# CompVis/behavior-driven-video-synthesis

Hardware: AMD Instinct MI355X
Metric: frames/sec VUnet 256x256 bs=16 fwd+bwd (higher is better)
Workload: dtype f32 (operands scaled by a power of two and split into 2 fp16 terms, 3 partial products on fp16 MFMA, fp32 accumulate; weight gradients and uncovered layers: 3 bf16 terms / 6 products, fp32-input MFMA, fp32 VALU); 1 GPU; Human3.6m shape_and_pose_net VunetAlter 256x256 per-GPU bs=16 fwd+bwd, VGG19 perceptual + KL loss, fused Adam, dropout 0.05, regressor side loop off, seeded-synthetic VGG19 weights, rasterised synthetic stickmen; global_batch=16, parallelism=dp1, conv_precision=h2, hip_streams=4, hip_graph=True, graph_settle_steps=7, rccl_world_size=1, dp_backend=none

## Files before the change

behavior_driven_video_synthesis_amd/csrc/common.h:

```cpp
#pragma once
#include <hip/hip_runtime.h>
#include <stdint.h>
#include <stdlib.h>

typedef float f32x16 __attribute__((ext_vector_type(16)));
typedef float f32x4 __attribute__((ext_vector_type(4)));

#include "../../include/vunet_hip.h"

enum { ACT_NONE = 0, ACT_ELU = 1, ACT_RELU = 2, ACT_SIGMOID = 3, ACT_LRELU = 4 };

__host__ __device__ __forceinline__ uint32_t vunet_hash_u32(uint32_t x) {
  x ^= x >> 16;
  x *= 0x7feb352dU;
  x ^= x >> 15;
  x *= 0x846ca68bU;
  x ^= x >> 16;
  return x;
}

__device__ __forceinline__ float elu_f(float x) { return x > 0.f ? x : (__expf(x) - 1.f); }
__device__ __forceinline__ float elu_grad_f(float x) { return x > 0.f ? 1.f : __expf(x); }
__device__ __forceinline__ float sigmoid_f(float x) { return 1.f / (1.f + expf(-x)); }
__device__ __forceinline__ float4 add4(float4 a, float4 b) { return make_float4(a.x + b.x, a.y + b.y, a.z + b.z, a.w + b.w); }

struct InAct {
  int act;
  uint32_t thresh;
  uint32_t seed;
  float keep_scale;
  float slope;
  const uint32_t* step;
};

#define VUNET_DROP_STEP_MUL 0x9E3779B1u

__device__ __forceinline__ uint32_t inact_seed(const InAct& a) {
  return a.step ? a.seed + (*a.step) * VUNET_DROP_STEP_MUL : a.seed;
}

__device__ __forceinline__ void inact_resolve(InAct& a) {
  a.seed = inact_seed(a);
  a.step = nullptr;
}

__device__ __forceinline__ float apply_in_act(const InAct& a, float v, uint32_t idx) {
  if (a.act == ACT_ELU) v = elu_f(v);
  else if (a.act == ACT_RELU) v = v > 0.f ? v : 0.f;
  else if (a.act == ACT_LRELU) v = v > 0.f ? v : v * a.slope;
  if (a.thresh) v = (vunet_hash_u32(idx + inact_seed(a)) >= a.thresh) ? v * a.keep_scale : 0.f;
  return v;
}

template <int FORM>
__device__ __forceinline__ float in_act_form(const InAct& a, float v, uint32_t idx) {
  if constexpr (FORM == 0) return v;
  else if constexpr (FORM == 1) return elu_f(v);
  else if constexpr (FORM == 2) {
    v = elu_f(v);
    return (vunet_hash_u32(idx + a.seed) >= a.thresh) ? v * a.keep_scale : 0.f;
  } else return apply_in_act(a, v, idx);
}
__device__ __forceinline__ int in_act_form_of(const InAct& a) {
  if (a.thresh) return a.act == ACT_ELU ? 2 : 3;
  return a.act == ACT_NONE ? 0 : (a.act == ACT_ELU ? 1 : 3);
}

__device__ __forceinline__ float in_act_grad(const InAct& a, float v, uint32_t idx) {
  float g = 1.f;
  if (a.act == ACT_ELU) g = elu_grad_f(v);
  else if (a.act == ACT_RELU) g = v > 0.f ? 1.f : 0.f;
  else if (a.act == ACT_LRELU) g = v > 0.f ? 1.f : a.slope;
  if (a.thresh) g = (vunet_hash_u32(idx + inact_seed(a)) >= a.thresh) ? g * a.keep_scale : 0.f;
  return g;
}

__device__ __forceinline__ float wave_sum(float v) {
#pragma unroll
  for (int o = 32; o > 0; o >>= 1) v += __shfl_xor(v, o, 64);
  return v;
}

__device__ __forceinline__ float wave_max(float v) {
#pragma unroll
  for (int o = 32; o > 0; o >>= 1) v = fmaxf(v, __shfl_xor(v, o, 64));
  return v;
}

__device__ __forceinline__ unsigned xcd_remap(unsigned bid, unsigned nblk) {
  const unsigned q = nblk >> 3, r = nblk & 7u, xcd = bid & 7u, idx = bid >> 3;
  const unsigned start = xcd < r ? xcd * (q + 1) : r * (q + 1) + (xcd - r) * q;
  return start + idx;
}

extern const uint32_t* g_vunet_drop_step;

static inline InAct make_inact(int act, float slope, float p, uint32_t seed) {
  InAct a;
  a.act = act;
  a.slope = slope;
  a.seed = seed;
  a.step = p > 0.f ? g_vunet_drop_step : nullptr;
  if (p > 0.f) {
    double t = (double)p * 4294967296.0;
    a.thresh = t >= 4294967295.0 ? 4294967295u : (uint32_t)t;
    if (a.thresh == 0) a.thresh = 1;
    a.keep_scale = 1.f / (1.f - p);
  } else {
    a.thresh = 0;
    a.keep_scale = 1.f;
  }
  return a;
}

#define VUNET_ENV_FLAG(fn, name)                              \
  static inline bool fn() {                                   \
    static const bool on = getenv(name) != nullptr;           \
    return on;                                                \
  }

extern int g_vunet_tune[16];

static inline int vunet_check_launch() {
  hipError_t e = hipGetLastError();
  return e == hipSuccess ? VUNET_OK : VUNET_ERR_LAUNCH;
}

#define VUNET_LAUNCH(...)          \
  do {                             \
    (void)hipGetLastError();       \
    hipLaunchKernelGGL(__VA_ARGS__); \
  } while (0)
```

behavior_driven_video_synthesis_amd/csrc/conv_h2_kernel.h:

```cpp
#pragma once
#include <type_traits>

#include "conv_common.h"

#include "split_h2.h"

__device__ __forceinline__ void h2_dma_wait() { asm volatile("s_waitcnt vmcnt(0)" ::: "memory"); }

union H2Unit {
  uint4 u;
  h2_f16x8 b;
};

#ifdef H2_TSTAMP
static __device__ unsigned long long h2_ts[8192 * 8];
#define H2_STAMP(k_)                                                                                              \
  do {                                                                                                            \
    if (threadIdx.x == 0 && blockIdx.x < 8192) h2_ts[blockIdx.x * 8 + (k_)] = __builtin_amdgcn_s_memrealtime();   \
  } while (0)
extern "C" int H2_TSTAMP(unsigned long long* out, int nblocks) {
  return hipMemcpyFromSymbol(out, HIP_SYMBOL(h2_ts), sizeof(unsigned long long) * 8 * (size_t)nblocks) == hipSuccess ? 0 : -1;
}
#else
#define H2_STAMP(k_)
#endif

template <int MT, int NT, int MODE, int PRO, int PHW = -1, int NWV = 4, int TW = 32>
__global__ __launch_bounds__(64 * NWV, (NWV == 8 || MT * NT >= 8) ? 1 : 2) void conv_h2_kernel(const GatherArgs a_in,
                                                                             const uint4* __restrict__ wx, int mtiles_pad,
                                                                             const float* __restrict__ amax) {
  GatherArgs a = a_in;
  H2_STAMP(0);
  inact_resolve(a.in1);
  inact_resolve(a.in2);
  inact_resolve(a.auxa);
  static_assert(PHW < 0 || MODE == 1, "parity phases exist for the data gradient only");
  constexpr bool ALLP = PHW == 4;
  static_assert(!ALLP || (NT == 1 && TW == 32 && NWV == 4 && PRO == 0), "fused parities: one dy row per wave");
  constexpr int NQ = ALLP ? 4 : NT;
  constexpr bool PIPE = TW == 16 && PHW < 0;
  constexpr int PH = (PHW >= 0 && !ALLP) ? (PHW >> 1) : 0, PW = (PHW >= 0 && !ALLP) ? (PHW & 1) : 0;
  constexpr int NKH = (PHW < 0 || ALLP) ? 3 : (PH ? 2 : 1);
  constexpr int NTHR = 64 * NWV;
  static_assert(TW == 32 || TW == 16, "tile width");
  constexpr int RPQ = 32 / TW;
  constexpr int TH = NWV * NT * RPQ, IH = TH + 2, CW = TW + 2, IW = TW == 32 ? CW : 32, PIX = IH * IW, MB = 32 * MT;
  constexpr int XU = 2 * IH * CW;
  constexpr int NX = (XU + NTHR - 1) / NTHR;
  constexpr int WU = H2_SLAB * MT;
  constexpr int GS = NWV == 8 ? NKH : 1;
  constexpr int WUS = WU * GS;
  extern __shared__ __attribute__((aligned(16))) uint4 smem4[];
  uint4* const xL = smem4;
  uint4* const wL = smem4 + 8 * PIX;

  const vunet_conv_desc& d = a.d;
  const int tid = threadIdx.x, lane = tid & 63, wave = tid >> 6;
  const int j = lane & 31, h = lane >> 5;
  const int jr = j / TW, jc = j % TW;
  const int H = d.Hs, W = d.Ws, HW = a.HsWs;

  const unsigned bid = xcd_remap(blockIdx.x, gridDim.x);
  const int mblocks = (d.M + MB - 1) / MB;
  const int mb = bid % mblocks;
  int t = bid / mblocks;
  const int tiles_w = W / TW, tiles_h = H / TH;
  const int tx = t % tiles_w;
  t /= tiles_w;
  const int ty = t % tiles_h;
  const int n = t / tiles_h;
  const int row0 = ty * TH, col0 = tx * TW, m0 = mb * MB;

  float sx, descale, descale2;

  unsigned rel[NX];
  int lds_x[NX];
  uint32_t vbits = 0;
#pragma unroll
  for (int i = 0; i < NX; ++i) {
    int u = tid + NTHR * i;
    if (u >= XU) u -= XU;
    const int c8 = u / (IH * CW);
    const int rem = u - c8 * (IH * CW);
    const int r = rem / CW, col = rem - r * CW;
    const int ih = row0 - 1 + r, iw = col0 - 1 + col;
    const bool ok = (unsigned)ih < (unsigned)H && (unsigned)iw < (unsigned)W;
    rel[i] = ok ? (unsigned)(8 * c8 * HW + ih * W + iw) : 0u;
    lds_x[i] = c8 * PIX + r * IW + col;
    vbits |= (ok ? 1u : 0u) << i;
  }

  f32x16 acc[MT][NQ], acx[MT][NQ];
#pragma unroll
  for (int mt = 0; mt < MT; ++mt)
#pragma unroll
    for (int q = 0; q < NQ; ++q)
#pragma unroll
      for (int r = 0; r < 16; ++r) acc[mt][q][r] = acx[mt][q][r] = 0.f;

  const int nch1 = d.C1 / 16, nch = nch1 + d.C2 / 16;
  float xv[NX][8];
  float mk[1][8];
  const int mt0 = (d.m_off + m0) >> 5;

  auto issue_x = [&](int ch, int i) {
    const bool second = ch >= nch1;
    const int cs = second ? (ch - nch1) * 16 : ch * 16;
    const int C = second ? d.C2 : d.C1;
    const float* __restrict__ xs = (second ? a.x2 : a.x1) + (size_t)(n * C + cs) * HW;
#pragma unroll
    for (int k = 0; k < 8; ++k)
      xv[i][k] = *reinterpret_cast<const float*>(reinterpret_cast<const char*>(xs) +
                                                 4u * (rel[i] + (((vbits >> i) & 1u) ? (unsigned)(k * HW) : 0u)));
  };
  auto issue_mask = [&](int ch, int i) {
    if constexpr (PRO == 4) {
      const float* __restrict__ ms = a.mask + (size_t)(n * d.C1 + ch * 16) * HW;
#pragma unroll
      for (int k = 0; k < 8; ++k)
        mk[0][k] = *reinterpret_cast<const float*>(reinterpret_cast<const char*>(ms) +
                                                   4u * (rel[i] + (((vbits >> i) & 1u) ? (unsigned)(k * HW) : 0u)));
    }
  };
  auto write_x = [&](int ch, int i) {
    const bool second = ch >= nch1;
    const int cs = second ? (ch - nch1) * 16 : ch * 16;
    const int C = second ? d.C2 : d.C1;
    InAct ia = a.in1;
    ia.seed = second ? a.in2.seed : a.in1.seed;
    const int gbase = (n * C + cs) * HW;
    const bool ok = (vbits >> i) & 1u;
    float v[8];
#pragma unroll
    for (int k = 0; k < 8; ++k) {
      float t_ = ok ? xv[i][k] : 0.f;
      if constexpr (PRO == 4) t_ = mk[0][k] > 0.f ? t_ : 0.f;
      else if constexpr (PRO != 0) t_ = prologue<PRO>(ia, t_, (uint32_t)gbase + rel[i] + (uint32_t)(k * HW));
      v[k] = t_ * sx;
    }
    uint4 ph, pl;
    h2_split2(v[0], v[1], ph.x, pl.x);
    h2_split2(v[2], v[3], ph.y, pl.y);
    h2_split2(v[4], v[5], ph.z, pl.z);
    h2_split2(v[6], v[7], ph.w, pl.w);
    uint4* const xb = xL + (ch & 1) * 4 * PIX;
    xb[lds_x[i]] = ph;
    xb[2 * PIX + lds_x[i]] = pl;
  };
  constexpr int WPS = WU / 64;
  constexpr int NWI = (GS * WPS + NWV - 1) / NWV;
  const int wave_u = __builtin_amdgcn_readfirstlane(wave);
  const uint32_t wL_addr = (uint32_t)(uintptr_t)(__attribute__((address_space(3))) void*)wL;
  auto slab_of = [&](int step) {
    if constexpr (PHW < 0 || ALLP) return step;
    else if constexpr (PH == 0) return step * 3 + 1;
    else return (step >> 1) * 3 + ((step & 1) ? 2 : 0);
  };
  auto issue_w = [&](int stage, int buf) {
#pragma unroll
    for (int i = 0; i < NWI; ++i) {
      int wi = wave_u + NWV * i;
      if (wi >= GS * WPS) wi -= GS * WPS;
      const int g = wi / WPS, r = wi - g * WPS;
      const char* wp = reinterpret_cast<const char*>(wx) + 16 +
                       ((size_t)slab_of(stage * GS + g) * mtiles_pad + mt0) * (H2_SLAB * 16);
      h2_dma16(wp + (size_t)(r * 64 + lane) * 16, wL_addr + (uint32_t)(buf * WUS + g * WU + r * 64) * 16u);
    }
  };

  issue_w(0, 0);
#pragma unroll
  for (int i = 0; i < NX; ++i) issue_x(0, i);
  {
    const float4 pm = h2_amax4(amax, a.amax2, tid & 255);
    float m_ = fmaxf(fmaxf(pm.x, pm.y), fmaxf(pm.z, pm.w));
    m_ = wave_max(m_);
    float* const redm = reinterpret_cast<float*>(smem4);
    if (lane == 0) redm[wave] = m_;
    __syncthreads();
    m_ = fmaxf(fmaxf(redm[0], redm[1]), fmaxf(redm[2], redm[3]));
    __syncthreads();
    if (a.in1.thresh) m_ *= a.in1.keep_scale;
    const int ex = h2_scale_exp(m_);
    const int ew = reinterpret_cast<const int*>(wx)[0];
    sx = h2_pow2(ex);
    h2_pow2_pair(-(ex + ew), descale, descale2);
  }
  H2_STAMP(1);

#pragma unroll
  for (int i = 0; i < NX; ++i) {
    issue_mask(0, i);
    write_x(0, i);
  }
  h2_dma_wait();
  __syncthreads();
  H2_STAMP(2);

  const uint4* const xB0 = xL + h * PIX + (wave * NT * RPQ + jr) * IW + jc;
  const uint4* const wA = wL + h * 32 + j;
  auto chunk = [&](int ch, auto last_c) {
    constexpr bool LAST = decltype(last_c)::value;
#pragma unroll
    for (int ki = 0; ki < NKH; ++ki) {
      const int kh = (PHW < 0 || ALLP) ? ki : (PH ? 2 * ki : 1);
      const int ph_t = ALLP ? ((kh + 1) & 1) : PH;
      const int phase = ch * NKH + ki;
      const int stage = phase / GS, g = phase - stage * GS;
      const int buf = stage & 1;
      const bool stage_begin = g == 0, stage_end = g == GS - 1;
      const bool more_w = !(LAST && ki == NKH - 1);
      const uint4* const xB = xB0 + (ch & 1) * 4 * PIX;
      if constexpr (!LAST) {
#pragma unroll
        for (int i = 0; i < NX; ++i)
          if (i * NKH / NX == ki) issue_x(ch + 1, i);
      }
      if (stage_begin && !(LAST && GS == NKH) && (GS == NKH || more_w)) issue_w(stage + 1, buf ^ 1);
      const int dr = PHW >= 0 ? (ph_t + 1 - kh) / 2 + 1 : (MODE == 0 ? kh : 2 - kh);
      if constexpr (PIPE) {
        H2Unit fa[2][2][MT], fb[2][2][NT];
        auto rd = [&](int kw, H2Unit (&av)[2][MT], H2Unit (&bv)[2][NT]) {
          const int dc = MODE == 0 ? kw : 2 - kw;
#pragma unroll
          for (int p = 0; p < 2; ++p) {
#pragma unroll
            for (int mt = 0; mt < MT; ++mt) av[p][mt].u = wA[buf * WUS + g * WU + ((mt * 3 + kw) * 2 + p) * 64];
#pragma unroll
            for (int q = 0; q < NT; ++q) bv[p][q].u = xB[p * 2 * PIX + (q * RPQ + dr) * IW + dc];
          }
        };
        rd(0, fa[0], fb[0]);
#pragma unroll
        for (int kw = 0; kw < 3; ++kw) {
          __builtin_amdgcn_sched_barrier(0);
          if (kw + 1 < 3) rd(kw + 1, fa[(kw + 1) & 1], fb[(kw + 1) & 1]);
          __builtin_amdgcn_sched_barrier(0);
#pragma unroll
          for (int mt = 0; mt < MT; ++mt)
#pragma unroll
            for (int q = 0; q < NT; ++q) {
              f32x16 cx = acx[mt][q];
              cx = __builtin_amdgcn_mfma_f32_32x32x16_f16(fa[kw & 1][1][mt].b, fb[kw & 1][0][q].b, cx, 0, 0, 0);
              cx = __builtin_amdgcn_mfma_f32_32x32x16_f16(fa[kw & 1][0][mt].b, fb[kw & 1][1][q].b, cx, 0, 0, 0);
              acx[mt][q] = cx;
              acc[mt][q] = __builtin_amdgcn_mfma_f32_32x32x16_f16(fa[kw & 1][0][mt].b, fb[kw & 1][0][q].b, acc[mt][q], 0, 0, 0);
            }
        }
      } else
#pragma unroll
      for (int kw = 0; kw < 3; ++kw) {
        if (PHW >= 0 && !ALLP && ((kw + PW) & 1) == 0) continue;
        const int pw_t = ALLP ? ((kw + 1) & 1) : PW;
        const int par = ph_t * 2 + pw_t;
        if constexpr (MT * NT < 8) __builtin_amdgcn_sched_barrier(0);
        const int dc = PHW >= 0 ? (pw_t + 1 - kw) / 2 + 1 : (MODE == 0 ? kw : 2 - kw);
        H2Unit av[2][MT], bv[2][NT];
#pragma unroll
        for (int p = 0; p < 2; ++p) {
#pragma unroll
          for (int mt = 0; mt < MT; ++mt) av[p][mt].u = wA[buf * WUS + g * WU + ((mt * 3 + kw) * 2 + p) * 64];
#pragma unroll
          for (int q = 0; q < NT; ++q) bv[p][q].u = xB[p * 2 * PIX + (q * RPQ + dr) * IW + dc];
        }
#pragma unroll
        for (int mt = 0; mt < MT; ++mt)
#pragma unroll
          for (int q = 0; q < NT; ++q) {
            const int qa = ALLP ? par : q;
            f32x16 cx = acx[mt][qa];
            cx = __builtin_amdgcn_mfma_f32_32x32x16_f16(av[1][mt].b, bv[0][q].b, cx, 0, 0, 0);
            cx = __builtin_amdgcn_mfma_f32_32x32x16_f16(av[0][mt].b, bv[1][q].b, cx, 0, 0, 0);
            acx[mt][qa] = cx;
            acc[mt][qa] = __builtin_amdgcn_mfma_f32_32x32x16_f16(av[0][mt].b, bv[0][q].b, acc[mt][qa], 0, 0, 0);
          }
      }
      __builtin_amdgcn_sched_barrier(0);
      if constexpr (!LAST) {
#pragma unroll
        for (int i = 0; i < NX; ++i)
          if (i * NKH / NX == ki) {
            issue_mask(ch + 1, i);
            write_x(ch + 1, i);
          }
      }
      if (stage_end && more_w) {
        h2_dma_wait();
        __syncthreads();
      }
    }
  };
  for (int ch = 0; ch + 1 < nch; ++ch) {
    chunk(ch, std::false_type{});
#ifdef H2_TSTAMP
    if (ch == 0) H2_STAMP(6);
#endif
  }
  chunk(nch - 1, std::true_type{});
  H2_STAMP(3);

  auto geo = [&](int q) {
    PixGeo g;
    g.n = n;
    const int orow = row0 + (wave * NT + q) * RPQ + jr, ocol = col0 + jc;
    g.oh = PHW >= 0 ? 2 * orow + PH : orow;
    g.ow = PHW >= 0 ? 2 * ocol + PW : ocol;
    g.valid = true;
    return g;
  };
  auto combined = [&](auto tc) {
    constexpr int t = decltype(tc)::value, q = t / MT, mt = t % MT;
    f32x16 c;
#pragma unroll
    for (int r = 0; r < 16; ++r) c[r] = (acc[mt][q][r] + acx[mt][q][r] * (1.f / 2048.f)) * descale * descale2;
    return c;
  };
  float ymax = 0.f;
  auto publish = [&]() {
    if (a.amax_out) {
      const float m_ = wave_max(ymax);
      if (lane == 0) atomicMax(reinterpret_cast<unsigned*>(a.amax_out) + ((blockIdx.x * 4u + wave) & 511u), __float_as_uint(m_));
    }
  };
  if constexpr (ALLP) {
    const int orow = row0 + wave + jr, ocol = col0 + jc;
#pragma unroll
    for (int mt = 0; mt < MT; ++mt)
#pragma unroll
      for (int ph = 0; ph < 2; ++ph) {
        f32x16 c0, c1;
#pragma unroll
        for (int r = 0; r < 16; ++r) {
          c0[r] = (acc[mt][2 * ph][r] + acx[mt][2 * ph][r] * (1.f / 2048.f)) * descale * descale2;
          c1[r] = (acc[mt][2 * ph + 1][r] + acx[mt][2 * ph + 1][r] * (1.f / 2048.f)) * descale * descale2;
        }
        ymax = fmaxf(ymax, store_tile_pair(a, n, 2 * orow + ph, 2 * ocol, m0 + 32 * mt, h, c0, c1));
      }
    publish();
    return;
  }
  if (PHW < 0 && a.wide) {
    const int k = lane & 3;
    TileSide4 side[2];
    auto tile = [&](auto tc, auto form_c) {
      constexpr int t = decltype(tc)::value, q = t / MT, mt = t % MT, FORM = decltype(form_c)::value;
      if constexpr (t == 0) load_tile_side4<MODE, FORM>(a, geo(0), m0, h, k, side[0]);
      if constexpr (t + 1 < MT * NT)
        load_tile_side4<MODE, FORM>(a, geo((t + 1) / MT), m0 + 32 * ((t + 1) % MT), h, k, side[(t + 1) & 1]);
      ymax = fmaxf(ymax, store_tile_side4<MODE, FORM>(a, geo(q), m0 + 32 * mt, h, k, combined(tc), side[t & 1]));
    };
    auto tiles = [&](auto form_c) {
      tile(std::integral_constant<int, 0>{}, form_c);
      if constexpr (MT * NT > 1) tile(std::integral_constant<int, 1>{}, form_c);
      if constexpr (MT * NT > 2) {
        tile(std::integral_constant<int, 2>{}, form_c);
        tile(std::integral_constant<int, 3>{}, form_c);
      }
      if constexpr (MT * NT > 4) {
        tile(std::integral_constant<int, 4>{}, form_c);
        tile(std::integral_constant<int, 5>{}, form_c);
        tile(std::integral_constant<int, 6>{}, form_c);
        tile(std::integral_constant<int, 7>{}, form_c);
      }
    };
    const int form = side4_form<MODE>(a);
    if (form == 1) tiles(std::integral_constant<int, 1>{});
    else if (MODE == 1 && form == 2) tiles(std::integral_constant<int, MODE == 1 ? 2 : 0>{});
    else if (MODE == 1 && form == 3) tiles(std::integral_constant<int, MODE == 1 ? 3 : 0>{});
    else tiles(std::integral_constant<int, 0>{});
    static_assert(MT * NT <= 8, "epilogue tiles are named at compile time");
    publish();
#ifdef H2_TSTAMP
    H2_STAMP(4);
    asm volatile("s_waitcnt vmcnt(0)" ::: "memory");
    H2_STAMP(5);
#endif
    return;
  }
  TileSide side[2];
  load_tile_side(a, geo(0), m0, h, side[0]);
  auto tile = [&](auto tc) {
    constexpr int t = decltype(tc)::value, q = t / MT, mt = t % MT;
    if constexpr (t + 1 < MT * NT) load_tile_side(a, geo((t + 1) / MT), m0 + 32 * ((t + 1) % MT), h, side[(t + 1) & 1]);
    ymax = fmaxf(ymax, store_tile_side(a, geo(q), m0 + 32 * mt, h, combined(tc), side[t & 1]));
  };
  tile(std::integral_constant<int, 0>{});
  if constexpr (MT * NT > 1) tile(std::integral_constant<int, 1>{});
  if constexpr (MT * NT > 2) {
    tile(std::integral_constant<int, 2>{});
    tile(std::integral_constant<int, 3>{});
  }
  if constexpr (MT * NT > 4) {
    tile(std::integral_constant<int, 4>{});
    tile(std::integral_constant<int, 5>{});
    tile(std::integral_constant<int, 6>{});
    tile(std::integral_constant<int, 7>{});
  }
  publish();
}

template <int MT, int NT, int MODE, int PRO, int PHW, int NWV, int TW = 32>
static int launch_h2_one(const GatherArgs& ga, const void* wx, int mtiles_pad, const float* amax, hipStream_t st) {
  constexpr int RPQ = 32 / TW;
  constexpr int PIX = (NWV * NT * RPQ + 2) * (TW == 32 ? 34 : 32);
  constexpr int NKH = (PHW < 0 || PHW == 4) ? 3 : ((PHW >> 1) ? 2 : 1);
  constexpr size_t lds = (size_t)(8 * PIX + 2 * H2_SLAB * MT * (NWV == 8 ? NKH : 1)) * 16;
  const vunet_conv_desc& d = ga.d;
  const int blocks = d.N * (d.Hs / (NWV * NT * RPQ)) * (d.Ws / TW) * ((d.M + 32 * MT - 1) / (32 * MT));
  auto kern = conv_h2_kernel<MT, NT, MODE, PRO, PHW, NWV, TW>;
  if (lds > 64 * 1024 &&
      hipFuncSetAttribute((const void*)kern, hipFuncAttributeMaxDynamicSharedMemorySize, (int)lds) != hipSuccess)
    return VUNET_ERR_LAUNCH;
  VUNET_LAUNCH(kern, dim3((unsigned)blocks), dim3(64 * NWV), lds, st, ga, (const uint4*)wx, mtiles_pad, amax);
  return vunet_check_launch();
}

template <int MT>
static int launch_h2_w16(const GatherArgs& ga, const void* wx, int mtiles_pad, const float* amax, int pro, hipStream_t st) {
  if (ga.d.mode == 1) {
    if (ga.d.stride != 1) return VUNET_ERR_UNSUPPORTED;
    if (pro == 4) return launch_h2_one<MT, 1, 1, 4, -1, 4, 16>(ga, wx, mtiles_pad, amax, st);
    if (pro == 0) return launch_h2_one<MT, 1, 1, 0, -1, 4, 16>(ga, wx, mtiles_pad, amax, st);
    return VUNET_ERR_UNSUPPORTED;
  }
  switch (pro) {
    case 0: return launch_h2_one<MT, 1, 0, 0, -1, 4, 16>(ga, wx, mtiles_pad, amax, st);
    case 1: return launch_h2_one<MT, 1, 0, 1, -1, 4, 16>(ga, wx, mtiles_pad, amax, st);
    case 2: return launch_h2_one<MT, 1, 0, 2, -1, 4, 16>(ga, wx, mtiles_pad, amax, st);
    default: return VUNET_ERR_UNSUPPORTED;
  }
}

template <int MT, int NT, int NWV = 4>
static int launch_h2(const GatherArgs& ga, const void* wx, int mtiles_pad, const float* amax, int pro, hipStream_t st) {
  if (ga.d.mode == 1 && ga.d.stride == 2) {
    if (pro != 0) return VUNET_ERR_UNSUPPORTED;
    int rc = launch_h2_one<MT, NT, 1, 0, 0, NWV>(ga, wx, mtiles_pad, amax, st);
    if (rc == VUNET_OK) rc = launch_h2_one<MT, NT, 1, 0, 1, NWV>(ga, wx, mtiles_pad, amax, st);
    if (rc == VUNET_OK) rc = launch_h2_one<MT, NT, 1, 0, 2, NWV>(ga, wx, mtiles_pad, amax, st);
    if (rc == VUNET_OK) rc = launch_h2_one<MT, NT, 1, 0, 3, NWV>(ga, wx, mtiles_pad, amax, st);
    return rc;
  }
  if (ga.d.mode == 1) {
    if (pro == 4) return launch_h2_one<MT, NT, 1, 4, -1, NWV>(ga, wx, mtiles_pad, amax, st);
    if (pro == 0) return launch_h2_one<MT, NT, 1, 0, -1, NWV>(ga, wx, mtiles_pad, amax, st);
    return VUNET_ERR_UNSUPPORTED;
  }
  switch (pro) {
    case 0: return launch_h2_one<MT, NT, 0, 0, -1, NWV>(ga, wx, mtiles_pad, amax, st);
    case 1: return launch_h2_one<MT, NT, 0, 1, -1, NWV>(ga, wx, mtiles_pad, amax, st);
    case 2: return launch_h2_one<MT, NT, 0, 2, -1, NWV>(ga, wx, mtiles_pad, amax, st);
    default: return VUNET_ERR_UNSUPPORTED;
  }
}
```

behavior_driven_video_synthesis_amd/csrc/conv_h2_mt2.hip:

```cpp
#include "conv_h2_kernel.h"

int vunet_conv_h2_launch_mt2(const GatherArgs& ga, const void* wx, int mtiles_pad, const float* amax, int pro, int NT,
                             hipStream_t st) {
  if (NT == 2) return launch_h2<2, 2>(ga, wx, mtiles_pad, amax, pro, st);
  return launch_h2<2, 1>(ga, wx, mtiles_pad, amax, pro, st);
}
```

behavior_driven_video_synthesis_amd/csrc/conv_h2_w16.hip:

```cpp
#include "conv_h2_kernel.h"

int vunet_conv_h2_launch_w16(const GatherArgs& ga, const void* wx, int mtiles_pad, const float* amax, int pro, int MT,
                             hipStream_t st) {
  return MT == 1 ? launch_h2_w16<1>(ga, wx, mtiles_pad, amax, pro, st) : launch_h2_w16<2>(ga, wx, mtiles_pad, amax, pro, st);
}
```

behavior_driven_video_synthesis_amd/csrc/conv_p2.hip:

```cpp
#include <stdio.h>

#include <type_traits>

#include "common.h"
#include "split_h2.h"

namespace {

constexpr int P2_META = 128, P2_AMAX0 = 16, P2_NSLOT = 64;

struct P2Args {
  const uint4* x;
  const int* xmeta;
  const uint4* w;
  const float* wk;
  const float* shift;
  const uint4* mask;
  uint4* y;
  int* ymeta;
  int N, C, H, W, M;
  int relu;
};

__device__ __forceinline__ void p2_dma(uint32_t voff, const void* sbase, uint32_t lds_addr) {
  uint32_t keep;
  asm volatile("s_mov_b32 %0, m0\n\ts_mov_b32 m0, %3\n\ts_nop 0\n\tglobal_load_lds_dwordx4 %1, %2\n\ts_mov_b32 m0, %0"
               : "=&s"(keep)
               : "v"(voff), "s"(sbase), "s"(lds_addr)
               : "memory");
}
template <int N>
__device__ __forceinline__ void p2_dma_wait() {
  static_assert(N == 0 || N == 1 || N == 2 || N == 4, "counts in use");
  if constexpr (N == 0) asm volatile("s_waitcnt vmcnt(0)" ::: "memory");
  else if constexpr (N == 1) asm volatile("s_waitcnt vmcnt(1)" ::: "memory");
  else if constexpr (N == 2) asm volatile("s_waitcnt vmcnt(2)" ::: "memory");
  else asm volatile("s_waitcnt vmcnt(4)" ::: "memory");
}
__device__ __forceinline__ const void* p2_uniform_ptr(const void* p) {
  const uint64_t v = (uint64_t)p;
  const uint32_t lo = __builtin_amdgcn_readfirstlane((uint32_t)v), hi = __builtin_amdgcn_readfirstlane((uint32_t)(v >> 32));
  return (const void*)(((uint64_t)hi << 32) | lo);
}

union P2Unit {
  uint4 u;
  h2_f16x8 b;
};

__device__ __forceinline__ float p2_meta_amax(const int* meta, int lane) {
  return wave_max(__int_as_float(meta[P2_AMAX0 + (lane & (P2_NSLOT - 1))]));
}

__device__ __forceinline__ void p2_swap16(uint32_t& a, uint32_t& b) {
  const auto r = __builtin_amdgcn_permlane16_swap(a, b, false, false);
  a = r[0];
  b = r[1];
}

__device__ __forceinline__ uint32_t p2_nonzero_halves(uint32_t t) {
  typedef unsigned short u16x2 __attribute__((ext_vector_type(2)));
  u16x2 v = __builtin_bit_cast(u16x2, t);
  const u16x2 one = {1, 1}, all = {0xFFFF, 0xFFFF};
  v = __builtin_elementwise_min(v, one) * all;
  return __builtin_bit_cast(uint32_t, v);
}

#define P2_TERMS 2
#include "conv_p2_kernel.h"
#undef P2_TERMS
#define P2_TERMS 1
#include "conv_p2_kernel.h"
#undef P2_TERMS

template <int CT, int TERMS>
int p2a_launch(const P2Args& a, hipStream_t st) {
  constexpr int XU = 4 * TERMS * 10 * (CT + 2), XS = (XU + 63) / 64 * 64, WU = 128 * 4 * TERMS;
  constexpr size_t lds = (size_t)(2 * XS + 2 * WU) * 16;
  const int blocks = a.N * (a.H / 8) * (a.W / CT) * (a.M / 128);
  void (*kern)(const P2Args);
  if constexpr (TERMS == 2) kern = conv_p2a_kernel<CT>;
  else kern = conv_p2a_kernel<CT, 1>;
  if (hipFuncSetAttribute((const void*)kern, hipFuncAttributeMaxDynamicSharedMemorySize, (int)lds) != hipSuccess) return VUNET_ERR_LAUNCH;
  VUNET_LAUNCH(kern, dim3((unsigned)blocks), dim3(512), lds, st, a);
  return vunet_check_launch();
}

template <int NW, int CT, int XBUF, int TERMS>
int p2_launch(const P2Args& a, hipStream_t st) {
  constexpr int XU = 4 * TERMS * 10 * (CT + 2), XS = (XU + 63) / 64 * 64, WU = 16 * NW * 4 * TERMS;
  constexpr size_t lds = (size_t)(XBUF * XS + 2 * WU) * 16;
  const int blocks = a.N * (a.H / 8) * (a.W / CT) * (a.M / (16 * NW));
  void (*kern)(const P2Args);
  if constexpr (TERMS == 2) kern = conv_p2_kernel<NW, CT, XBUF>;
  else kern = conv_p2_kernel<NW, CT, XBUF, 1>;
  if (lds > 64 * 1024 && hipFuncSetAttribute((const void*)kern, hipFuncAttributeMaxDynamicSharedMemorySize, (int)lds) != hipSuccess)
    return VUNET_ERR_LAUNCH;
  VUNET_LAUNCH(kern, dim3((unsigned)blocks), dim3(64 * NW), lds, st, a);
  return vunet_check_launch();
}

}

static bool p2_shape_ok(const vunet_p2_desc* d) {
  if (!d || d->N < 1 || d->C < 32 || d->C % 32 || d->M < 64 || d->M % 64 || d->H < 8 || d->H % 8) return false;
  if (!(d->W == 16 || (d->W >= 32 && d->W % 32 == 0))) return false;
  const double plane_bytes = (double)d->N * (d->C / 8) * (d->H + 2) * (d->W + 2) * 16.0;
  return plane_bytes * 2.0 < 4.0e9;
}

extern "C" int vunet_p2_conv_supported(const vunet_p2_desc* d) { return p2_shape_ok(d) ? 1 : 0; }

static int p2_form(const vunet_p2_desc* d) {
  const long px_tiles = (long)d->N * (d->H / 8) * (d->W / (d->W == 16 ? 16 : 32));
  const int force = g_vunet_tune[VUNET_TUNE_P2_FORM];
  const bool wide = d->M % 128 == 0 && (force == 2 || force == 3 || (force != 1 && px_tiles * (d->M / 128) >= 256));
  return wide ? 8 : 4;
}

static bool p2_one_term() { return g_vunet_tune[VUNET_TUNE_P2_TERMS] == 1; }

extern "C" int vunet_p2_conv(const vunet_p2_desc* d, const void* x, const int32_t* xmeta, const void* w_image, const float* wk,
                             const float* shift, const void* mask, void* y, int32_t* ymeta, void* stream) {
  if (!d || !x || !xmeta || !w_image || !wk || !y || !ymeta) return VUNET_ERR_ARG;
  if (!p2_shape_ok(d)) return VUNET_ERR_UNSUPPORTED;
  if (((uintptr_t)x | (uintptr_t)w_image | (uintptr_t)y | (uintptr_t)mask | (uintptr_t)shift) & 15) return VUNET_ERR_ARG;
  P2Args a;
  a.x = (const uint4*)x; a.xmeta = xmeta; a.w = (const uint4*)w_image; a.wk = wk; a.shift = shift; a.mask = (const uint4*)mask;
  a.y = (uint4*)y; a.ymeta = ymeta;
  a.N = d->N; a.C = d->C; a.H = d->H; a.W = d->W; a.M = d->M; a.relu = d->relu;
  hipStream_t st = (hipStream_t)stream;
  const int form = p2_form(d);
  if (!p2_one_term()) {
    const bool lockstep = g_vunet_tune[VUNET_TUNE_P2_FORM] == 3;
    if (d->W == 16) return form == 8 ? (lockstep ? p2_launch<8, 16, 2, 2>(a, st) : p2a_launch<16, 2>(a, st)) : p2_launch<4, 16, 1, 2>(a, st);
    return form == 8 ? (lockstep ? p2_launch<8, 32, 2, 2>(a, st) : p2a_launch<32, 2>(a, st)) : p2_launch<4, 32, 1, 2>(a, st);
  }
  if (d->W == 16) return form == 8 ? p2a_launch<16, 1>(a, st) : p2_launch<4, 16, 1, 1>(a, st);
  return form == 8 ? p2a_launch<32, 1>(a, st) : p2_launch<4, 32, 1, 1>(a, st);
}

extern "C" int vunet_p2_conv_variant(const vunet_p2_desc* d, char* name, int32_t len) {
  if (!d || !name || len < 32) return VUNET_ERR_ARG;
  if (!p2_shape_ok(d)) return VUNET_ERR_UNSUPPORTED;
  const int form = p2_form(d);
  if (p2_one_term()) {
    if (form == 8) snprintf(name, (size_t)len, "conv_p2a_kernel<%d, 1>", d->W == 16 ? 16 : 32);
    else snprintf(name, (size_t)len, "conv_p2_kernel<4, %d, 1, 1>", d->W == 16 ? 16 : 32);
    return VUNET_OK;
  }
  if (form == 8 && g_vunet_tune[VUNET_TUNE_P2_FORM] != 3) snprintf(name, (size_t)len, "conv_p2a_kernel<%d>", d->W == 16 ? 16 : 32);
  else snprintf(name, (size_t)len, "conv_p2_kernel<%d, %d, %d>", form, d->W == 16 ? 16 : 32, form == 8 ? 2 : 1);
  return VUNET_OK;
}

namespace {
__global__ __launch_bounds__(256) void p2_wstat_kernel(const float* __restrict__ w, int Cout, int Cin, int dgrad,
                                                       float* __restrict__ rows) {
  __shared__ float red[8];
  const int r = blockIdx.x;
  float s = 0.f, m = 0.f;
  const int K = dgrad ? Cout : Cin;
  for (int i = threadIdx.x; i < K * 9; i += 256) {
    const int k = i / 9, t = i - 9 * k;
    const float v = fabsf(dgrad ? w[((size_t)k * Cin + r) * 9 + t] : w[((size_t)r * Cin + k) * 9 + t]);
    s += v;
    m = fmaxf(m, v);
  }
  s = wave_sum(s);
  m = wave_max(m);
  if ((threadIdx.x & 63) == 0) {
    red[threadIdx.x >> 6] = s;
    red[4 + (threadIdx.x >> 6)] = m;
  }
  __syncthreads();
  if (threadIdx.x == 0) {
    rows[2 * r] = (red[0] + red[1]) + (red[2] + red[3]);
    rows[2 * r + 1] = fmaxf(fmaxf(red[4], red[5]), fmaxf(red[6], red[7]));
  }
}
__global__ __launch_bounds__(256) void p2_wk_kernel(const float* __restrict__ rows, int R, const float* __restrict__ shift,
                                                    int nshift, float* __restrict__ wk) {
  __shared__ float red[12];
  float s = 0.f, m = 0.f, b = 0.f;
  for (int i = threadIdx.x; i < R; i += 256) {
    s = fmaxf(s, rows[2 * i]);
    m = fmaxf(m, rows[2 * i + 1]);
  }
  for (int i = threadIdx.x; i < nshift; i += 256) b = fmaxf(b, fabsf(shift[i]));
  s = wave_max(s);
  m = wave_max(m);
  b = wave_max(b);
  if ((threadIdx.x & 63) == 0) {
    red[threadIdx.x >> 6] = s;
    red[4 + (threadIdx.x >> 6)] = m;
    red[8 + (threadIdx.x >> 6)] = b;
  }
  __syncthreads();
  if (threadIdx.x == 0) {
    const float mx = fmaxf(fmaxf(red[4], red[5]), fmaxf(red[6], red[7]));
    wk[0] = fmaxf(fmaxf(red[0], red[1]), fmaxf(red[2], red[3])) * (1.f + 1e-6f);
    wk[1] = fmaxf(fmaxf(red[8], red[9]), fmaxf(red[10], red[11]));
    wk[2] = (float)h2_scale_exp(mx);
    wk[3] = mx;
  }
}
__global__ __launch_bounds__(256) void p2_wpack_kernel(const float* __restrict__ w, int Cout, int Cin, int dgrad,
                                                       const float* __restrict__ wk, uint4* __restrict__ img) {
  const int R = dgrad ? Cin : Cout, K = dgrad ? Cout : Cin;
  const int MT = R / 16;
  const size_t units = (size_t)(K / 32) * 9 * MT * 2 * 64;
  const float sw = h2_pow2((int)wk[2]);
  for (size_t u = (size_t)blockIdx.x * 256 + threadIdx.x; u < units; u += (size_t)gridDim.x * 256) {
    size_t v = u;
    const int l = (int)(v & 63);
    v >>= 6;
    const int p = (int)(v & 1);
    v >>= 1;
    const int mt = (int)(v % MT);
    v /= MT;
    const int tap = (int)(v % 9);
    const int ch = (int)(v / 9);
    const int row = mt * 16 + (l & 15), k0 = ch * 32 + (l >> 4) * 8;
    const int kh = tap / 3, kw = tap - 3 * kh;
    float e[8];
#pragma unroll
    for (int j = 0; j < 8; ++j) {
      const int k = k0 + j;
      const float x = dgrad ? w[(((size_t)k * Cin + row) * 3 + (2 - kh)) * 3 + (2 - kw)] : w[(((size_t)row * Cin + k) * 3 + kh) * 3 + kw];
      e[j] = x * sw;
    }
    uint32_t h[4], lo[4];
#pragma unroll
    for (int j = 0; j < 4; ++j) h2_split2(e[2 * j], e[2 * j + 1], h[j], lo[j]);
    img[u] = p ? make_uint4(lo[0], lo[1], lo[2], lo[3]) : make_uint4(h[0], h[1], h[2], h[3]);
  }
}
}

extern "C" int vunet_p2_weight_image_bytes(int32_t Cout, int32_t Cin, int32_t dgrad) {
  const int R = dgrad ? Cin : Cout, K = dgrad ? Cout : Cin;
  if (R < 16 || R % 16 || K < 32 || K % 32 || (int64_t)R * K > (1 << 22)) return 0;
  return (K / 32) * 9 * (R / 16) * 2 * 64 * 16;
}

extern "C" int vunet_p2_pack_weights(const float* w, const float* shift, int32_t Cout, int32_t Cin, int32_t dgrad, void* image,
                                     float* wk, float* workspace, void* stream) {
  if (!w || !image || !wk || !workspace) return VUNET_ERR_ARG;
  if (vunet_p2_weight_image_bytes(Cout, Cin, dgrad) == 0) return VUNET_ERR_UNSUPPORTED;
  const int R = dgrad ? Cin : Cout;
  hipStream_t st = (hipStream_t)stream;
  VUNET_LAUNCH(p2_wstat_kernel, dim3((unsigned)R), dim3(256), 0, st, w, (int)Cout, (int)Cin, (int)dgrad, workspace);
  VUNET_LAUNCH(p2_wk_kernel, dim3(1), dim3(256), 0, st, (const float*)workspace, R, dgrad ? nullptr : shift,
               (dgrad || !shift) ? 0 : (int)Cout, wk);
  const size_t units = (size_t)vunet_p2_weight_image_bytes(Cout, Cin, dgrad) / 16;
  size_t nb = (units + 255) / 256;
  if (nb > 2048) nb = 2048;
  VUNET_LAUNCH(p2_wpack_kernel, dim3((unsigned)nb), dim3(256), 0, st, w, (int)Cout, (int)Cin, (int)dgrad, (const float*)wk,
               (uint4*)image);
  return vunet_check_launch();
}

extern "C" int vunet_p2_weight_bound(const float* w, const float* shift, int32_t Cout, int32_t Cin, float* wk, float* workspace,
                                     void* stream) {
  if (!w || !wk || !workspace || Cout < 1 || Cin < 1) return VUNET_ERR_ARG;
  hipStream_t st = (hipStream_t)stream;
  VUNET_LAUNCH(p2_wstat_kernel, dim3((unsigned)Cout), dim3(256), 0, st, w, (int)Cout, (int)Cin, 0, workspace);
  VUNET_LAUNCH(p2_wk_kernel, dim3(1), dim3(256), 0, st, (const float*)workspace, (int)Cout, shift, shift ? (int)Cout : 0, wk);
  return vunet_check_launch();
}

namespace {
__global__ __launch_bounds__(256) void p2_from_nchw_kernel(const float* __restrict__ x, const float* __restrict__ amax, int n_amax,
                                                           int relu, uint4* __restrict__ y, int* __restrict__ ymeta, int N, int C,
                                                           int H, int W) {
  __shared__ float red[4];
  float m = 0.f;
  for (int i = threadIdx.x; i < n_amax; i += 256) m = fmaxf(m, amax[i]);
  m = wave_max(m);
  if ((threadIdx.x & 63) == 0) red[threadIdx.x >> 6] = m;
  __syncthreads();
  m = fmaxf(fmaxf(red[0], red[1]), fmaxf(red[2], red[3]));
  const int e = h2_scale_exp(m);
  const float s = h2_pow2(e);
  if (blockIdx.x == 0 && threadIdx.x == 0) {
    ymeta[0] = e;
    ymeta[P2_AMAX0] = __float_as_int(m);
  }
  const int CB = C >> 3, Hp = H + 2, Wp = W + 2;
  const size_t HW = (size_t)H * W, total = (size_t)N * CB * HW, plane = (size_t)N * CB * Hp * Wp;
  for (size_t i = (size_t)blockIdx.x * 256 + threadIdx.x; i < total; i += (size_t)gridDim.x * 256) {
    const int xw = (int)(i % W);
    size_t t = i / W;
    const int yh = (int)(t % H);
    t /= H;
    const float* src = x + (t * 8) * HW + (size_t)yh * W + xw;
    float v[8];
#pragma unroll
    for (int j = 0; j < 8; ++j) {
      float f = src[j * HW];
      if (relu) f = f > 0.f ? f : 0.f;
      v[j] = f * s;
    }
    uint4 h, l;
    h2_split2(v[0], v[1], h.x, l.x);
    h2_split2(v[2], v[3], h.y, l.y);
    h2_split2(v[4], v[5], h.z, l.z);
    h2_split2(v[6], v[7], h.w, l.w);
    const size_t o = (t * Hp + (yh + 1)) * Wp + (xw + 1);
    y[o] = h;
    y[plane + o] = l;
  }
}
__device__ __forceinline__ void p2_unpack(const uint4& h, const uint4& l, float inv, float* v) {
  const uint32_t hs[4] = {h.x, h.y, h.z, h.w}, ls[4] = {l.x, l.y, l.z, l.w};
#pragma unroll
  for (int j = 0; j < 4; ++j) {
    const h2_f16x2 a = __builtin_bit_cast(h2_f16x2, hs[j]), b = __builtin_bit_cast(h2_f16x2, ls[j]);
    v[2 * j] = ((float)a[0] + (float)b[0] * (1.f / 2048.f)) * inv;
    v[2 * j + 1] = ((float)a[1] + (float)b[1] * (1.f / 2048.f)) * inv;
  }
}
__global__ __launch_bounds__(256) void p2_to_nchw_kernel(const uint4* __restrict__ x, const int* __restrict__ xmeta,
                                                         float* __restrict__ y, int N, int C, int H, int W) {
  const int CB = C >> 3, Hp = H + 2, Wp = W + 2;
  const float inv = h2_pow2(-xmeta[0]);
  const size_t HW = (size_t)H * W, total = (size_t)N * CB * HW, plane = (size_t)N * CB * Hp * Wp;
  for (size_t i = (size_t)blockIdx.x * 256 + threadIdx.x; i < total; i += (size_t)gridDim.x * 256) {
    const int xw = (int)(i % W);
    size_t t = i / W;
    const int yh = (int)(t % H);
    t /= H;
    const size_t o = (t * Hp + (yh + 1)) * Wp + (xw + 1);
    float v[8];
    p2_unpack(x[o], x[plane + o], inv, v);
    float* dst = y + (t * 8) * HW + (size_t)yh * W + xw;
#pragma unroll
    for (int j = 0; j < 8; ++j) dst[j * HW] = v[j];
  }
}
}

extern "C" int vunet_p2_from_nchw(const float* x, const float* amax, int32_t n_amax, int32_t relu, void* y, int32_t* ymeta,
                                  int32_t N, int32_t C, int32_t H, int32_t W, void* stream) {
  if (!x || !amax || n_amax < 1 || !y || !ymeta || C % 8 || N < 1) return VUNET_ERR_ARG;
  const size_t total = (size_t)N * (C / 8) * H * W;
  size_t nb = (total + 255) / 256;
  if (nb > 4096) nb = 4096;
  VUNET_LAUNCH(p2_from_nchw_kernel, dim3((unsigned)nb), dim3(256), 0, (hipStream_t)stream, x, amax, (int)n_amax, (int)relu, (uint4*)y,
               (int*)ymeta, (int)N, (int)C, (int)H, (int)W);
  return vunet_check_launch();
}

extern "C" int vunet_p2_to_nchw(const void* x, const int32_t* xmeta, float* y, int32_t N, int32_t C, int32_t H, int32_t W,
                                void* stream) {
  if (!x || !xmeta || !y || C % 8 || N < 1) return VUNET_ERR_ARG;
  const size_t total = (size_t)N * (C / 8) * H * W;
  size_t nb = (total + 255) / 256;
  if (nb > 4096) nb = 4096;
  VUNET_LAUNCH(p2_to_nchw_kernel, dim3((unsigned)nb), dim3(256), 0, (hipStream_t)stream, (const uint4*)x, (const int*)xmeta, y, (int)N,
               (int)C, (int)H, (int)W);
  return vunet_check_launch();
}
```

behavior_driven_video_synthesis_amd/csrc/conv_p2_kernel.h:

```cpp
#if P2_TERMS == 2
template <int NW, int CT, int XBUF>
#else
template <int NW, int CT, int XBUF, int ONE>
#endif
__global__ __launch_bounds__(64 * NW, NW == 8 ? 1 : 2) void conv_p2_kernel(const P2Args a) {
  constexpr int TERMS = P2_TERMS;
  static_assert(NW == 4 || NW == 8, "waves");
  static_assert(CT == 32 || CT == 16, "tile width");
  static_assert(TERMS == 1 || TERMS == 2, "terms per operand");
  constexpr int MW = 16 * NW;
  constexpr int RT = 8, IH = RT + 2, CW = CT + 2, XPIX = IH * CW, XU = 4 * TERMS * XPIX;
  constexpr int NXI = (XU + 63) / 64, XS = NXI * 64;
  constexpr int NXW = (NXI + NW - 1) / NW;
  constexpr int WU = MW * 4 * TERMS;
  constexpr int NWI = WU / 64 / NW;
  constexpr int WSRC = TERMS == 2 ? 1024 : 2048;
  constexpr int PTR = CT / 16, NPT = 2 * PTR;
  static_assert(XBUF == 1 || NXW <= 8, "the next chunk's pieces ride on the first taps");
  extern __shared__ __attribute__((aligned(16))) uint4 smem[];
  uint4* const xL = smem;
  uint4* const wL = smem + XBUF * XS;

  const int tid = threadIdx.x, lane = tid & 63;
  const int wave = __builtin_amdgcn_readfirstlane(tid >> 6);
// ... 117 lines not shown
          for (int q = 0; q < NPT; ++q)
            acx[mt][q] = __builtin_amdgcn_mfma_f32_16x16x32_f16(av[0][mt].b, bv[TERMS - 1][q].b, acx[mt][q], 0, 0, 0);
      }
#pragma unroll
      for (int mt = 0; mt < 4; ++mt)
#pragma unroll
        for (int q = 0; q < NPT; ++q)
          acc[mt][q] = __builtin_amdgcn_mfma_f32_16x16x32_f16(av[0][mt].b, bv[0][q].b, acc[mt][q], 0, 0, 0);
      __builtin_amdgcn_sched_barrier(0);
      if (more_w) {
        if (xpiece) p2_dma_wait<1>();
        else p2_dma_wait<0>();
        __syncthreads();
        if (XBUF == 1 && tap == 8) {
#pragma unroll
          for (int i = 0; i < NXW; ++i) issue_x(ch + 1, i);
          p2_dma_wait<0>();
          __syncthreads();
        }
      }
    }
  };
  for (int ch = 0; ch + 1 < nch; ++ch) chunk(ch, std::false_type{});
  chunk(nch - 1, std::true_type{});

  const bool relu = a.relu != 0;
  const size_t plane = (size_t)a.N * MB * Hp * Wp;
  float ymax = 0.f;
#pragma unroll
  for (int mt = 0; mt < 4; ++mt) {
    const int co = m0 + 64 * mg + 16 * mt + 4 * cg;
    float sh[4] = {0.f, 0.f, 0.f, 0.f};
    if (a.shift) {
      const float4 s4 = *reinterpret_cast<const float4*>(a.shift + co);
      sh[0] = s4.x; sh[1] = s4.y; sh[2] = s4.z; sh[3] = s4.w;
    }
#pragma unroll
    for (int qp = 0; qp < NPT; qp += 2) {
      uint32_t hh[2][2], ll[2][2];
#pragma unroll
      for (int s = 0; s < 2; ++s) {
        float v[4];
#pragma unroll
        for (int r = 0; r < 4; ++r) {
          float c;
          if constexpr (TERMS == 2) c = (acc[mt][qp + s][r] + acx[mt][qp + s][r] * (1.f / 2048.f)) * descale * descale2 + sh[r];
          else c = acc[mt][qp + s][r] * descale * descale2 + sh[r];
          c = (relu && !(c > 0.f)) ? 0.f : c;
          ymax = fmaxf(ymax, fabsf(c));
          v[r] = c * sy;
        }
        h2_split2(v[0], v[1], hh[s][0], ll[s][0]);
        h2_split2(v[2], v[3], hh[s][1], ll[s][1]);
      }
      p2_swap16(hh[0][0], hh[1][0]);
      p2_swap16(hh[0][1], hh[1][1]);
      p2_swap16(ll[0][0], ll[1][0]);
      p2_swap16(ll[0][1], ll[1][1]);
      uint4 uh = make_uint4(hh[0][0], hh[0][1], hh[1][0], hh[1][1]);
      uint4 ul = make_uint4(ll[0][0], ll[0][1], ll[1][0], ll[1][1]);
      const int q = qp + (cg & 1);
      const int orow = row0 + 2 * rg + q / PTR, ocol = col0 + (q % PTR) * 16 + px;
      const int cb = ((m0 + 64 * mg + 16 * mt) >> 3) + (cg >> 1);
      const size_t o = (((size_t)n * MB + cb) * Hp + (orow + 1)) * Wp + (ocol + 1);
      if (a.mask) {
        const uint4 mh = a.mask[o], ml = a.mask[plane + o];
        const uint32_t k0 = p2_nonzero_halves((mh.x | ml.x) & 0x7FFF7FFFu), k1 = p2_nonzero_halves((mh.y | ml.y) & 0x7FFF7FFFu);
        const uint32_t k2 = p2_nonzero_halves((mh.z | ml.z) & 0x7FFF7FFFu), k3 = p2_nonzero_halves((mh.w | ml.w) & 0x7FFF7FFFu);
        uh.x &= k0; uh.y &= k1; uh.z &= k2; uh.w &= k3;
        ul.x &= k0; ul.y &= k1; ul.z &= k2; ul.w &= k3;
      }
      a.y[o] = uh;
      a.y[plane + o] = ul;
    }
  }
  {
    const float m_ = wave_max(ymax);
    if (lane == 0)
      atomicMax(reinterpret_cast<unsigned*>(a.ymeta) + P2_AMAX0 + ((blockIdx.x * NW + wave) & (P2_NSLOT - 1)), __float_as_uint(m_));
  }
}

#if P2_TERMS == 2
template <int CT>
#else
template <int CT, int ONE>
#endif
__global__ __launch_bounds__(512, 1) void conv_p2a_kernel(const P2Args a) {
  constexpr int TERMS = P2_TERMS;
  static_assert(TERMS == 1 || TERMS == 2, "terms per operand");
  constexpr int NW = 8, MW = 128;
  constexpr int RT = 8, IH = RT + 2, CW = CT + 2, XPIX = IH * CW, XU = 4 * TERMS * XPIX;
  constexpr int NXI = (XU + 63) / 64, XS = NXI * 64;
  constexpr int NXG = (NXI + 3) / 4;
  constexpr int XPT = 2, NXT = (NXG + XPT - 1) / XPT;
  constexpr int WU = MW * 4 * TERMS;
  constexpr int WSRC = TERMS == 2 ? 1024 : 2048;
  constexpr int PTR = CT / 16, NPT = 2 * PTR;
  static_assert(NXT <= 8, "the next chunk's pieces must be visible before its first tap");
  extern __shared__ __attribute__((aligned(16))) uint4 smem[];
  uint4* const xL = smem;
  uint4* const wL = smem + 2 * XS;

  const int tid = threadIdx.x, lane = tid & 63;
  const int wave = __builtin_amdgcn_readfirstlane(tid >> 6);
  const int mg = wave >> 2, rg = wave & 3;
  const int px = lane & 15, cg = lane >> 4;
  const int Hp = a.H + 2, Wp = a.W + 2, CB = a.C >> 3, MB = a.M >> 3;

  const unsigned bid = xcd_remap(blockIdx.x, gridDim.x);
  const int mblocks = a.M / MW;
  const int mb = bid % mblocks;
  int t = bid / mblocks;
  const int tiles_w = a.W / CT, tiles_h = a.H / RT;
  const int tx = t % tiles_w;
  t /= tiles_w;
  const int ty = t % tiles_h;
  const int n = t / tiles_h;
  const int row0 = ty * RT, col0 = tx * CT, m0 = mb * MW;

  uint32_t xoff[NXG];
#pragma unroll
  for (int i = 0; i < NXG; ++i) {
    int j = rg + 4 * i;
    if (j >= NXI) j = NXI - 1;
    int u = 64 * j + lane;
    if (u >= XU) u = XU - 1;
    const int p = u / (4 * XPIX);
    int rem = u - p * 4 * XPIX;
    const int kq = rem / XPIX;
    rem -= kq * XPIX;
    const int r = rem / CW, c = rem - r * CW;
    xoff[i] = (uint32_t)((((size_t)p * a.N * CB + kq) * Hp + (row0 + r)) * Wp + col0 + c) * 16u;
  }
  const uint32_t xL_addr = (uint32_t)(uintptr_t)(__attribute__((address_space(3))) void*)xL;
  const uint32_t wL_addr = (uint32_t)(uintptr_t)(__attribute__((address_space(3))) void*)wL;
  const char* const xsrc0 = reinterpret_cast<const char*>(a.x) + (size_t)n * CB * Hp * Wp * 16;
  const size_t xchunk = (size_t)4 * Hp * Wp * 16;
  const char* const wsrc0 = reinterpret_cast<const char*>(a.w) + (size_t)mb * (MW / 16) * 128 * 16;
  const size_t wslab = (size_t)(a.M / 16) * 128 * 16;
  const uint32_t lane16 = (uint32_t)lane * 16u;

  auto issue_x = [&](int ch, int i) {
    int j = rg + 4 * i;
    if (j >= NXI) j = NXI - 1;
    if constexpr (TERMS == 1) j = __builtin_amdgcn_readfirstlane(j);
    p2_dma(xoff[i], p2_uniform_ptr(xsrc0 + (size_t)ch * xchunk), xL_addr + (uint32_t)((ch & 1) * XS + 64 * j) * 16u);
  };
  auto issue_w = [&](int g, int buf) {
    const char* src = wsrc0 + (size_t)g * wslab;
#pragma unroll
    for (int i = 0; i < 2 * TERMS; ++i) {
      const int part = rg * (2 * TERMS) + i;
      p2_dma(lane16, p2_uniform_ptr(src + (size_t)part * WSRC), wL_addr + (uint32_t)(buf * WU + part * 64) * 16u);
    }
  };

  if (mg == 0) issue_w(0, 0);
  else {
#pragma unroll
    for (int i = 0; i < NXG; ++i) issue_x(0, i);
  }
  float descale, descale2, sy;
  {
    const int ex = a.xmeta[0];
    const float amax_x = p2_meta_amax(a.xmeta, lane);
    const int ew = (int)a.wk[2];
    h2_pow2_pair(-(ex + ew), descale, descale2);
    const float bound = a.wk[0] * amax_x + a.wk[1];
    const int ey = h2_scale_exp(bound);
    sy = h2_pow2(ey);
    if (blockIdx.x == 0 && tid == 0) a.ymeta[0] = ey;
  }
  f32x4 acc[4][NPT], acx[4][NPT];
#pragma unroll
  for (int mt = 0; mt < 4; ++mt)
#pragma unroll
    for (int q = 0; q < NPT; ++q)
#pragma unroll
      for (int r = 0; r < 4; ++r) acc[mt][q][r] = acx[mt][q][r] = 0.f;
  p2_dma_wait<0>();
  __syncthreads();
  if (mg == 1) __builtin_amdgcn_s_barrier();

  const int nch = a.C >> 5;
  const uint4* const wA0 = wL + (mg * 4) * (64 * TERMS) + lane;
  const uint4* const xB0 = xL + cg * XPIX + px + (2 * rg) * CW;

  auto chunk = [&](int ch, auto last_c) {
    constexpr bool LAST = decltype(last_c)::value;
    const uint4* const xB = xB0 + (ch & 1) * XS;
    const int wpar = (ch * 9) & 1;
#pragma unroll
    for (int tap = 0; tap < 9; ++tap) {
      const int kh = tap / 3, kw = tap - 3 * kh;
      const int g = ch * 9 + tap;
      const int buf = wpar ^ (tap & 1);
      const bool more_w = !(LAST && tap == 8);
      if (mg == 0) {
        if (more_w) issue_w(g + 1, buf ^ 1);
      } else if (!LAST && tap < NXT) {
#pragma unroll
        for (int i = 0; i < XPT; ++i)
          if (tap * XPT + i < NXG) issue_x(ch + 1, tap * XPT + i);
      }
      const uint4* const wA = wA0 + buf * WU;
      P2Unit av[TERMS][4], bv[TERMS][NPT];
#pragma unroll
      for (int p = 0; p < TERMS; ++p) {
#pragma unroll
        for (int mt = 0; mt < 4; ++mt) av[p][mt].u = wA[(mt * TERMS + p) * 64];
#pragma unroll
        for (int q = 0; q < NPT; ++q) bv[p][q].u = xB[p * 4 * XPIX + (q / PTR + kh) * CW + (q % PTR) * 16 + kw];
      }
      asm volatile("s_waitcnt lgkmcnt(0)" ::: "memory");
      __builtin_amdgcn_sched_barrier(0);
      __builtin_amdgcn_s_barrier();
      __builtin_amdgcn_sched_barrier(0);
      __builtin_amdgcn_s_setprio(1);
      if constexpr (TERMS == 2) {
#pragma unroll
        for (int mt = 0; mt < 4; ++mt)
#pragma unroll
          for (int q = 0; q < NPT; ++q)
            acx[mt][q] = __builtin_amdgcn_mfma_f32_16x16x32_f16(av[TERMS - 1][mt].b, bv[0][q].b, acx[mt][q], 0, 0, 0);
#pragma unroll
        for (int mt = 0; mt < 4; ++mt)
#pragma unroll
          for (int q = 0; q < NPT; ++q)
            acx[mt][q] = __builtin_amdgcn_mfma_f32_16x16x32_f16(av[0][mt].b, bv[TERMS - 1][q].b, acx[mt][q], 0, 0, 0);
      }
#pragma unroll
      for (int mt = 0; mt < 4; ++mt)
#pragma unroll
        for (int q = 0; q < NPT; ++q)
          acc[mt][q] = __builtin_amdgcn_mfma_f32_16x16x32_f16(av[0][mt].b, bv[0][q].b, acc[mt][q], 0, 0, 0);
      __builtin_amdgcn_s_setprio(0);
      __builtin_amdgcn_sched_barrier(0);
      p2_dma_wait<0>();
      __builtin_amdgcn_s_barrier();
      __builtin_amdgcn_sched_barrier(0);
    }
  };
  for (int ch = 0; ch + 1 < nch; ++ch) chunk(ch, std::false_type{});
  chunk(nch - 1, std::true_type{});
  if (mg == 0) __builtin_amdgcn_s_barrier();

  const bool relu = a.relu != 0;
  const size_t plane = (size_t)a.N * MB * Hp * Wp;
  float ymax = 0.f;
#pragma unroll
  for (int mt = 0; mt < 4; ++mt) {
    const int co = m0 + 64 * mg + 16 * mt + 4 * cg;
    float sh[4] = {0.f, 0.f, 0.f, 0.f};
    if (a.shift) {
      const float4 s4 = *reinterpret_cast<const float4*>(a.shift + co);
      sh[0] = s4.x; sh[1] = s4.y; sh[2] = s4.z; sh[3] = s4.w;
    }
#pragma unroll
    for (int qp = 0; qp < NPT; qp += 2) {
      uint32_t hh[2][2], ll[2][2];
#pragma unroll
      for (int s = 0; s < 2; ++s) {
        float v[4];
#pragma unroll
        for (int r = 0; r < 4; ++r) {
          float c;
          if constexpr (TERMS == 2) c = (acc[mt][qp + s][r] + acx[mt][qp + s][r] * (1.f / 2048.f)) * descale * descale2 + sh[r];
          else c = acc[mt][qp + s][r] * descale * descale2 + sh[r];
          c = (relu && !(c > 0.f)) ? 0.f : c;
          ymax = fmaxf(ymax, fabsf(c));
          v[r] = c * sy;
        }
        h2_split2(v[0], v[1], hh[s][0], ll[s][0]);
        h2_split2(v[2], v[3], hh[s][1], ll[s][1]);
      }
      p2_swap16(hh[0][0], hh[1][0]);
      p2_swap16(hh[0][1], hh[1][1]);
      p2_swap16(ll[0][0], ll[1][0]);
      p2_swap16(ll[0][1], ll[1][1]);
      uint4 uh = make_uint4(hh[0][0], hh[0][1], hh[1][0], hh[1][1]);
      uint4 ul = make_uint4(ll[0][0], ll[0][1], ll[1][0], ll[1][1]);
      const int q = qp + (cg & 1);
      const int orow = row0 + 2 * rg + q / PTR, ocol = col0 + (q % PTR) * 16 + px;
      const int cb = ((m0 + 64 * mg + 16 * mt) >> 3) + (cg >> 1);
      const size_t o = (((size_t)n * MB + cb) * Hp + (orow + 1)) * Wp + (ocol + 1);
      if (a.mask) {
        const uint4 mh = a.mask[o], ml = a.mask[plane + o];
        const uint32_t k0 = p2_nonzero_halves((mh.x | ml.x) & 0x7FFF7FFFu), k1 = p2_nonzero_halves((mh.y | ml.y) & 0x7FFF7FFFu);
        const uint32_t k2 = p2_nonzero_halves((mh.z | ml.z) & 0x7FFF7FFFu), k3 = p2_nonzero_halves((mh.w | ml.w) & 0x7FFF7FFFu);
        uh.x &= k0; uh.y &= k1; uh.z &= k2; uh.w &= k3;
        ul.x &= k0; ul.y &= k1; ul.z &= k2; ul.w &= k3;
      }
      a.y[o] = uh;
      a.y[plane + o] = ul;
    }
  }
  {
    const float m_ = wave_max(ymax);
    if (lane == 0)
      atomicMax(reinterpret_cast<unsigned*>(a.ymeta) + P2_AMAX0 + ((blockIdx.x * NW + wave) & (P2_NSLOT - 1)), __float_as_uint(m_));
  }
}
```

behavior_driven_video_synthesis_amd/csrc/conv_route.h:

```cpp
#pragma once
#include "conv_common.h"

enum ConvFamily {
  CONV_UNSUPPORTED = 0,
  CONV_PHASE,
  CONV_THIN,
  CONV_1X1,
  CONV_TILED,
  CONV_GATHER,
  CONV_SPLITK,
  CONV_H2_S2,
  CONV_H2_SMALL,
  CONV_H2_W16,
  CONV_H2_PAR,
  CONV_H2,
  CONV_X6,
};

struct ConvRoute {
  int family;
  int pro;
  int MT, NT, TW;
  int form;
  bool publishes;
};

static inline bool conv_route_is_split(const ConvRoute& r) { return r.family >= CONV_H2_S2; }

ConvRoute conv_route(const vunet_conv_desc* d, int scheme, bool has_aux, bool has_res, bool has_mask, long min_blocks, bool query);
bool conv_route_tiled(const vunet_conv_desc* d, int pro, bool has_aux, ConvRoute* r);
int conv_route_gather_form(const vunet_conv_desc* d, long NP, int* MT, int* NT);
int conv_route_name(const ConvRoute& r, const vunet_conv_desc* d, char* name, int len);

int vunet_conv_thin_kind(const vunet_conv_desc* d, int pro, bool has_aux, bool has_res);
bool vunet_conv_thin_strips(const vunet_conv_desc* d);
int vunet_conv_thin_launch(const ConvRoute& r, const GatherArgs& ga, hipStream_t st);
bool vunet_conv_1x1_applicable(const vunet_conv_desc* d, int pro);
int vunet_conv_1x1_mt(const vunet_conv_desc* d);
int vunet_conv_1x1_launch(const ConvRoute& r, const GatherArgs& ga, hipStream_t st);
bool vunet_conv_tiled_applicable(const vunet_conv_desc* d);
int vunet_conv_tiled_pick(const vunet_conv_desc* d, int* MT, bool valu_heavy);
int vunet_conv_tiled_width(const vunet_conv_desc* d);
int vunet_conv_tiled_launch(const ConvRoute& r, const GatherArgs& ga, hipStream_t st);
int vunet_conv2d_gather_amax(const vunet_conv_desc* d, const float* x1, const float* x2, const float* wt, const float* shift,
                             const float* res, const float* aux, float* y, float* amax_out, void* stream,
                             const ConvRoute* route = nullptr);
bool vunet_conv_h2_s2_ok(const vunet_conv_desc* d, int pro);
int vunet_conv_h2_s2_mt(const vunet_conv_desc* d);
int vunet_conv_h2_s2_launch(const ConvRoute& r, const GatherArgs& ga, const void* wx, int mtiles_pad, const float* amax, hipStream_t st);
bool vunet_conv_h2_small_ok(const vunet_conv_desc* d, int pro);
bool vunet_conv_h2_small_wanted(const vunet_conv_desc* d, int pro);
int vunet_conv_h2_small_nr(const vunet_conv_desc* d);
int vunet_conv_h2_small_launch(const ConvRoute& r, const GatherArgs& ga, const void* wx, int mtiles_pad, const float* amax, hipStream_t st);
int vunet_conv_x6_launch_mt1(const GatherArgs& ga, const void* wx, int mtiles_pad, int pro, int NT, hipStream_t st);
int vunet_conv_x6_launch_mt2(const GatherArgs& ga, const void* wx, int mtiles_pad, int pro, int NT, hipStream_t st);
int vunet_conv_h2_launch_mt1(const GatherArgs& ga, const void* wx, int mtiles_pad, const float* amax, int pro, int NT, hipStream_t st);
int vunet_conv_h2_launch_mt2(const GatherArgs& ga, const void* wx, int mtiles_pad, const float* amax, int pro, int NT, hipStream_t st);
int vunet_conv_h2_launch_par(const GatherArgs& ga, const void* wx, int mtiles_pad, const float* amax, hipStream_t st);
int vunet_conv_h2_launch_w16(const GatherArgs& ga, const void* wx, int mtiles_pad, const float* amax, int pro, int MT, hipStream_t st);
```

behavior_driven_video_synthesis_amd/csrc/conv_x6.hip:

```cpp
#include "conv_route.h"

extern "C" int vunet_x6_mtiles(int32_t M);

static bool x6_enabled() {
  static const bool on = [] {
    const char* e = getenv("VUNET_CONV_PRECISION");
    return !(e && (e[0] == 'f' || e[0] == 'F'));
  }();
  return on;
}

static int prologue_code(const vunet_conv_desc* d, bool has_mask) {
  if (has_mask) return (d->in_act == ACT_NONE && d->drop_p <= 0.f) ? 4 : 3;
  if (d->in_act == ACT_NONE && d->drop_p <= 0.f) return 0;
  if (d->in_act == ACT_ELU && d->drop_p <= 0.f) return 1;
  if (d->in_act == ACT_ELU) return 2;
  return 3;
}

static bool h2_w16(const vunet_conv_desc* d) { return d->Ws % 32 != 0 && d->Ws % 16 == 0 && d->Hs % 8 == 0 && d->stride == 1; }

static bool x6_geometry_ok(const vunet_conv_desc* d, int pro, bool h2 = false) {
  if (d->KH != 3 || d->KW != 3 || d->pad != 1) return false;
  if (d->C1 <= 0 || d->C1 % 16 || d->C2 % 16 || d->Hs % 4) return false;
  if (d->Ws % 32 && !(h2 && h2_w16(d))) return false;
  if (d->M % 32 || d->m_off % 32) return false;
  if (d->stride == 2)
    return d->mode == 1 && pro == 0 && d->C2 == 0 && d->Ho == 2 * d->Hs && d->Wo == 2 * d->Ws;
  if (d->stride != 1 || d->Hs != d->Ho || d->Ws != d->Wo) return false;
  return d->mode == 0 ? (pro == 0 || pro == 1 || pro == 2) : (pro == 0 || pro == 4);
}

static long x6_blocks(const vunet_conv_desc* d, int MT, int NT) {
  if (d->Ws % 32) return NT == 1 ? (long)d->N * (d->Hs / 8) * (d->Ws / 16) * ((d->M + 32 * MT - 1) / (32 * MT)) : 0;
  if (d->Hs % (4 * NT)) return 0;
  return (long)d->N * (d->Hs / (4 * NT)) * (d->Ws / 32) * ((d->M + 32 * MT - 1) / (32 * MT));
}

static int x6_pick(const vunet_conv_desc* d, int* MT, long min_blocks, bool h2 = false) {
  *MT = d->M <= 32 ? 1 : 2;
  const int top = h2 ? (*MT == 1 ? 1 : 2) : (*MT == 1 ? 4 : 2);
  if (int NT = g_vunet_tune[VUNET_TUNE_SPLIT_FORCE_NT]) {
    if (NT > top) NT = (h2 && *MT == 1 && NT == 2) ? 2 : top;
    if ((NT == 1 || NT == 2 || NT == 4) && x6_blocks(d, *MT, NT) > 0) return NT;
  }
  for (int NT = top; NT >= 2; NT >>= 1)
    if (x6_blocks(d, *MT, NT) >= 512) return NT;
  return x6_blocks(d, *MT, 1) >= min_blocks ? 1 : 0;
}

VUNET_ENV_FLAG(env_no_tiled, "VUNET_NO_TILED")
VUNET_ENV_FLAG(env_no_phase, "VUNET_NO_PHASE")

static bool want_splitk(const vunet_conv_desc* d, long NP, int taps) {
  const long tiles = ((NP + 31) / 32) * ((d->M + 31) / 32);
  const int kpairs = ((d->C1 + 1) >> 1) + ((d->C2 + 1) >> 1);
  return (tiles <= 768 && kpairs >= 32) || (tiles <= 2048 && (long)kpairs * taps >= 288);
}

int conv_route_gather_form(const vunet_conv_desc* d, long NP, int* MT, int* NT) {
  *MT = *NT = 1;
  if (want_splitk(d, NP, d->KH * d->KW)) return CONV_SPLITK;
  if (d->M <= 32) *NT = 4;
  else *MT = *NT = 2;
  return CONV_GATHER;
}

bool conv_route_tiled(const vunet_conv_desc* d, int pro, bool has_aux, ConvRoute* r) {
  if (env_no_tiled() || !vunet_conv_tiled_applicable(d) ||
      !(d->mode == 0 ? pro != 4 : (pro == 0 || (pro == 4 && d->stride == 1))) || pro == 3)
    return false;
  if (vunet_conv_tiled_pick(d, &r->MT, true) <= 0) return false;
  r->family = CONV_TILED, r->pro = pro, r->form = 0;
  r->NT = vunet_conv_tiled_pick(d, &r->MT, (pro != 0 && pro != 4) || (d->mode == 1 && has_aux));
  r->TW = vunet_conv_tiled_width(d);
  r->publishes = !d->d2s;
  return true;
}

static ConvRoute gather_route(const vunet_conv_desc* d, bool has_aux, bool has_res) {
  ConvRoute r = {CONV_UNSUPPORTED, prologue_code(d, false), 1, 1, 32, 0, false};
  const long NP = (long)d->N * d->Ho * d->Wo;
  if (d->mode == 1 && d->stride > 1 && !env_no_phase()) {
    r.family = CONV_PHASE;
  } else if (const int thin = vunet_conv_thin_kind(d, r.pro, has_aux, has_res)) {
    r.family = CONV_THIN, r.form = thin;
    r.NT = vunet_conv_thin_strips(d) ? 1 : 0;
    r.publishes = thin == 2;
  } else if (vunet_conv_1x1_applicable(d, r.pro) && !want_splitk(d, NP, 1)) {
    r.family = CONV_1X1, r.MT = vunet_conv_1x1_mt(d);
    r.publishes = !d->d2s;
  } else if (!conv_route_tiled(d, r.pro, has_aux, &r)) {
    r.family = conv_route_gather_form(d, NP, &r.MT, &r.NT);
    r.form = (d->KH == 3 && d->KW == 3) ? 3 : ((d->KH == 1 && d->KW == 1) ? 1 : 0);
    r.publishes = r.family == CONV_SPLITK && !d->d2s;
  }
  return r;
}

static ConvRoute split_route(const vunet_conv_desc* d, bool h2, bool has_aux, bool has_res, bool has_mask, long min_blocks,
                             bool query) {
  ConvRoute r = {CONV_UNSUPPORTED, prologue_code(d, has_mask), 0, 0, 32, 0, h2};
  const int pro = r.pro;
  if (h2 && !has_mask && !has_aux && !has_res && !g_vunet_tune[VUNET_TUNE_S2_FWD_F32] && vunet_conv_h2_s2_ok(d, pro)) {
    r.family = CONV_H2_S2, r.MT = vunet_conv_h2_s2_mt(d);
    return r;
  }
  r.NT = x6_geometry_ok(d, pro, h2) ? x6_pick(d, &r.MT, min_blocks, h2) : 0;
  if (!query && g_vunet_tune[VUNET_TUNE_FORCE_SMALL] && h2 && !has_mask && vunet_conv_h2_small_ok(d, pro)) r.NT = 0;
  if (r.NT == 0) {
    if (!h2 || has_mask || !(min_blocks <= 1 ? vunet_conv_h2_small_ok(d, pro) : vunet_conv_h2_small_wanted(d, pro))) return r;
    r.family = CONV_H2_SMALL, r.form = vunet_conv_h2_small_nr(d);
  } else if (!h2) {
    r.family = CONV_X6;
  } else if (d->Ws % 32) {
    r.family = CONV_H2_W16, r.TW = 16;
  } else if (d->stride == 2 && !g_vunet_tune[VUNET_TUNE_PARITY_LAUNCHES]) {
    r.family = CONV_H2_PAR;
  } else {
    r.family = CONV_H2;
  }
  return r;
}

ConvRoute conv_route(const vunet_conv_desc* d, int scheme, bool has_aux, bool has_res, bool has_mask, long min_blocks, bool query) {
  if (scheme != 0 && x6_enabled()) {
    const int pro = prologue_code(d, has_mask);
    if (vunet_conv_thin_kind(d, pro == 4 ? 0 : pro, has_aux, has_res) == 0) {
      const ConvRoute r = split_route(d, scheme == 2, has_aux, has_res, has_mask, min_blocks, query);
      if (r.family != CONV_UNSUPPORTED) return r;
      if (!query && g_vunet_tune[VUNET_TUNE_FORCE_SMALL] &&
          split_route(d, scheme == 2, has_aux, has_res, has_mask, min_blocks, true).family != CONV_UNSUPPORTED)
        return r;
    }
  }
  return gather_route(d, has_aux, has_res);
}

int conv_route_name(const ConvRoute& r, const vunet_conv_desc* d, char* name, int len) {
  switch (r.family) {
    case CONV_PHASE: snprintf(name, len, "conv_gather_kernel<phase x%d>", d->stride * d->stride); break;
    case CONV_THIN:
      if (r.form == 1 && r.NT == 1) snprintf(name, len, "conv_thin_mv_kernel<%d, 4>", d->mode);
      else if (r.form == 1) snprintf(name, len, "conv_thin_m_kernel<%d>", d->mode);
      else if (r.NT == 1) snprintf(name, len, "conv_thin_kv_kernel<3, 4>");
      else snprintf(name, len, "conv_thin_k_kernel<%d, 3>", d->KH);
      break;
    case CONV_1X1: snprintf(name, len, "conv_1x1_kernel<%d, %d, %d>", r.MT, d->mode, d->mode == 1 ? 0 : r.pro); break;
    case CONV_TILED: {
      const int nt = r.TW == 16 ? 1 : r.NT;
      snprintf(name, len, "conv_tiled_kernel<%d, %d, %d, %d, %d, %d, %d>", r.MT, d->stride == 2 ? 1 : nt,
               (r.MT == 2 && nt == 4) ? 4 : 8, d->mode, d->mode == 1 ? (r.pro == 4 ? 4 : 0) : r.pro, r.TW, d->stride);
      break;
    }
    case CONV_GATHER: snprintf(name, len, "conv_gather_kernel<%d, %d, %d, %d>", r.MT, r.NT, r.pro, r.form); break;
    case CONV_SPLITK: snprintf(name, len, "conv_gather_splitk_kernel<16, %d, %d>", r.pro, r.form); break;
    case CONV_H2_S2: snprintf(name, len, "conv_h2_s2_kernel<%d>", r.MT); break;
    case CONV_H2_SMALL:
      if (r.form == 0) return VUNET_ERR_UNSUPPORTED;
      snprintf(name, len, "conv_h2_small_kernel<%d, %d>", r.pro, r.form); break;
    case CONV_H2_W16: snprintf(name, len, "conv_h2_kernel<%d, 1, %d, %d, -1, 4, 16>", r.MT, d->mode, r.pro); break;
    case CONV_H2_PAR: snprintf(name, len, "conv_h2_kernel<1, 1, 1, 0, 4, 4, 32>"); break;
    case CONV_H2:
      if (d->stride == 2) snprintf(name, len, "conv_h2_kernel<%d, %d, 1, 0, parity x4, 4, 32>", r.MT, r.NT);
      else snprintf(name, len, "conv_h2_kernel<%d, %d, %d, %d, -1, 4, 32>", r.MT, r.NT, d->mode, r.pro);
      break;
    case CONV_X6:
      if (d->stride == 2) snprintf(name, len, "conv_x6_kernel<%d, %d, 1, 0, parity x4>", r.MT, r.NT);
      else snprintf(name, len, "conv_x6_kernel<%d, %d, %d, %d, -1>", r.MT, r.NT, d->mode, r.pro);
      break;
    default: return VUNET_ERR_UNSUPPORTED;
  }
  return VUNET_OK;
}

static int split_launch(const ConvRoute& r, const vunet_conv_desc* d, const float* x1, const float* x2, const void* wx,
                        const float* shift, const float* res, const float* aux, const float* mask, float* y, const float* amax,
                        float* amax_out, void* stream, const float* amax2 = nullptr, const float* res2 = nullptr) {
  if (res2 && (d->mode != 1 || !amax)) return VUNET_ERR_UNSUPPORTED;
  if (r.family == CONV_UNSUPPORTED) return VUNET_ERR_UNSUPPORTED;
  GatherArgs ga;
  fill_gather_args(ga, d, x1, x2, nullptr, shift, res, aux, mask, y, d->stride == 1 && d->Wo % 4 == 0);
  ga.amax2 = amax2;
  if (r.publishes) ga.amax_out = amax_out;
  hipStream_t st = (hipStream_t)stream;
  const int mtp = vunet_x6_mtiles(d->Mpad);
  if (r.family == CONV_H2_S2) return vunet_conv_h2_s2_launch(r, ga, wx, mtp, amax, st);
  ga.res2 = res2;
  ga.wide = ga.wide && (reinterpret_cast<uintptr_t>(res2) & 15) == 0;
  switch (r.family) {
    case CONV_H2_SMALL: return vunet_conv_h2_small_launch(r, ga, wx, mtp, amax, st);
    case CONV_H2_W16: return vunet_conv_h2_launch_w16(ga, wx, mtp, amax, r.pro, r.MT, st);
    case CONV_H2_PAR: return vunet_conv_h2_launch_par(ga, wx, mtp, amax, st);
    case CONV_H2:
      return r.MT == 1 ? vunet_conv_h2_launch_mt1(ga, wx, mtp, amax, r.pro, r.NT, st)
                       : vunet_conv_h2_launch_mt2(ga, wx, mtp, amax, r.pro, r.NT, st);
    default:
      return r.MT == 1 ? vunet_conv_x6_launch_mt1(ga, wx, mtp, r.pro, r.NT, st)
                       : vunet_conv_x6_launch_mt2(ga, wx, mtp, r.pro, r.NT, st);
  }
}

extern "C" int vunet_conv2d_x6(const vunet_conv_desc* d, const float* x1, const float* x2, const void* wx,
                               const float* shift, const float* res, const float* aux, const float* mask, float* y,
                               const float* amax, float* amax_out, void* stream) {
  if (!d || !x1 || !wx || !y || (d->C2 > 0 && !x2) || d->Mpad % 32 != 0) return VUNET_ERR_ARG;
  if (mask && (d->mode != 1 || d->C2 != 0)) return VUNET_ERR_ARG;
  if (d->d2s && (d->M % 4 != 0 || d->mode != 0)) return VUNET_ERR_ARG;
  const ConvRoute r = split_route(d, amax != nullptr, aux != nullptr, res != nullptr, mask != nullptr, 1, false);
  return split_launch(r, d, x1, x2, wx, shift, res, aux, mask, y, amax, amax_out, stream);
}

extern "C" int vunet_conv2d_a2(const vunet_conv_desc* d, const float* x1, const float* x2, const float* wt, const void* wx,
                               const float* shift, const float* res, const float* res2, const float* aux, float* y,
                               const float* amax, const float* amax2, float* amax_out, void* stream) {
  if (!d) return VUNET_ERR_ARG;
  if (amax2 && (!amax || d->C2 <= 0)) return VUNET_ERR_ARG;
  if (res2 && (!res || d->mode != 1)) return VUNET_ERR_ARG;
  if (!wx) {
    if (res2) return VUNET_ERR_UNSUPPORTED;
    return vunet_conv2d_gather_amax(d, x1, x2, wt, shift, res, aux, y, amax_out, stream);
  }
  const ConvRoute r = conv_route(d, amax ? 2 : 1, aux != nullptr, res != nullptr, false, 128, false);
  if (conv_route_is_split(r) || r.family == CONV_UNSUPPORTED) {
    if (!x1 || !y || (d->C2 > 0 && !x2) || d->Mpad % 32 != 0) return VUNET_ERR_ARG;
    return split_launch(r, d, x1, x2, wx, shift, res, aux, nullptr, y, amax, amax_out, stream, amax2, res2);
  }
  if (res2) return VUNET_ERR_UNSUPPORTED;
  return vunet_conv2d_gather_amax(d, x1, x2, wt, shift, res, aux, y, amax_out, stream, &r);
}

extern "C" int vunet_conv2d(const vunet_conv_desc* d, const float* x1, const float* x2, const float* wt, const void* wx,
                            const float* shift, const float* res, const float* aux, float* y, const float* amax,
                            float* amax_out, void* stream) {
  return vunet_conv2d_a2(d, x1, x2, wt, wx, shift, res, nullptr, aux, y, amax, nullptr, amax_out, stream);
}

extern "C" int vunet_conv2d_dgrad_relu_x6(const vunet_conv_desc* d, const float* dy, const float* y, const void* wx,
                                          const float* res, float* dx, const float* amax, float* amax_out, void* stream) {
  if (!d || !dy || !y || !wx || !dx || d->mode != 1 || d->C2 != 0 || d->Mpad % 32 != 0) return VUNET_ERR_ARG;
  if (d->aux_act != ACT_NONE || d->aux_drop_p > 0.f) return VUNET_ERR_UNSUPPORTED;
  const ConvRoute r = conv_route(d, amax ? 2 : 1, false, res != nullptr, true, 128, false);
  if (!conv_route_is_split(r)) return VUNET_ERR_UNSUPPORTED;
  return split_launch(r, d, dy, nullptr, wx, nullptr, res, nullptr, y, dx, amax, amax_out, stream);
}

extern "C" int vunet_conv2d_x6_supported(const vunet_conv_desc* d, int32_t has_mask) {
  return d && x6_geometry_ok(d, prologue_code(d, has_mask != 0)) ? 1 : 0;
}

extern "C" int vunet_conv2d_wants_split(const vunet_conv_desc* d, int32_t has_aux, int32_t has_res, int32_t has_mask, int32_t split) {
  return d && conv_route_is_split(conv_route(d, split == 2 ? 2 : 1, has_aux != 0, has_res != 0, has_mask != 0, 128, true)) ? 1 : 0;
}

extern "C" int vunet_conv2d_publishes_amax(const vunet_conv_desc* d, int32_t has_aux, int32_t has_res, int32_t split) {
  if (!d) return 0;
  return conv_route(d, split == 0 ? 0 : (split == 2 ? 2 : 1), has_aux != 0, has_res != 0, false, 128, true).publishes ? 1 : 0;
}

extern "C" int vunet_conv2d_gather_variant(const vunet_conv_desc* d, int32_t has_aux, char* name, int32_t len) {
  if (!d || !name || len < 8) return VUNET_ERR_ARG;
  return conv_route_name(gather_route(d, has_aux != 0, false), d, name, len);
}

extern "C" int vunet_conv2d_variant(const vunet_conv_desc* d, int32_t has_aux, int32_t has_wx, int32_t has_mask,
                                    char* name, int32_t len) {
  if (!d || !name || len < 8) return VUNET_ERR_ARG;
  return conv_route_name(conv_route(d, has_wx == 2 ? 2 : (has_wx ? 1 : 0), has_aux != 0, false, has_mask != 0, 128, true), d,
                         name, len);
}
```

behavior_driven_video_synthesis_amd/ops.py:

```python
from __future__ import annotations

import contextlib
import ctypes
import os
from dataclasses import dataclass
from typing import Optional, Tuple

import torch

from . import _lib

ACT_NONE, ACT_ELU, ACT_RELU, ACT_SIGMOID, ACT_LRELU = 0, 1, 2, 3, 4
SEED2_OFFSET = 0x9E3779B9


class ConvDesc(ctypes.Structure):
    _fields_ = [("N", ctypes.c_int32), ("C1", ctypes.c_int32), ("C2", ctypes.c_int32), ("Hs", ctypes.c_int32),
                ("Ws", ctypes.c_int32), ("M", ctypes.c_int32), ("m_off", ctypes.c_int32), ("Mpad", ctypes.c_int32),
                ("Ho", ctypes.c_int32), ("Wo", ctypes.c_int32), ("KH", ctypes.c_int32), ("KW", ctypes.c_int32),
                ("stride", ctypes.c_int32), ("pad", ctypes.c_int32), ("mode", ctypes.c_int32),
                ("in_act", ctypes.c_int32), ("in_slope", ctypes.c_float), ("drop_p", ctypes.c_float),
                ("drop_seed", ctypes.c_uint32), ("out_act", ctypes.c_int32), ("d2s", ctypes.c_int32),
                ("aux_act", ctypes.c_int32), ("aux_slope", ctypes.c_float), ("aux_drop_p", ctypes.c_float),
                ("aux_drop_seed", ctypes.c_uint32)]


class WgradDesc(ctypes.Structure):
    _fields_ = [("N", ctypes.c_int32), ("C1", ctypes.c_int32), ("C2", ctypes.c_int32), ("Hs", ctypes.c_int32),
                ("Ws", ctypes.c_int32), ("Cout", ctypes.c_int32), ("Ho", ctypes.c_int32), ("Wo", ctypes.c_int32),
                ("KH", ctypes.c_int32), ("KW", ctypes.c_int32), ("stride", ctypes.c_int32), ("pad", ctypes.c_int32),
                ("in_act", ctypes.c_int32), ("in_slope", ctypes.c_float), ("drop_p", ctypes.c_float),
                ("drop_seed", ctypes.c_uint32), ("nsplit", ctypes.c_int32), ("flags", ctypes.c_int32)]


class WgradItem(ctypes.Structure):
    _fields_ = [("d", WgradDesc)] + [(n, ctypes.c_void_p) for n in ("x1", "x2", "dy", "slabs", "dshift", "amax_x", "amax_x2",
                                                                   "amax_dy")]


class WnDesc(ctypes.Structure):
    _fields_ = [("Cout", ctypes.c_int32), ("C1", ctypes.c_int32), ("C2", ctypes.c_int32), ("KH", ctypes.c_int32),
                ("KW", ctypes.c_int32), ("kind", ctypes.c_int32), ("split", ctypes.c_int32)]


class WnBwdItem(ctypes.Structure):
    _fields_ = ([(n, ctypes.c_void_p) for n in ("slabs", "dshift", "v", "g", "bias", "gamma", "invnorm", "dv", "dg", "dbias",
                                                "dgamma", "dbeta", "workspace")] +
                [("d", WnDesc), ("nsplit", ctypes.c_int32), ("accumulate", ctypes.c_int32)])


def _p(t: Optional[torch.Tensor]):
    return None if t is None else ctypes.c_void_p(t.data_ptr())


_raw_stream = getattr(torch._C, "_cuda_getCurrentRawStream", None)


def _stream():
    if _raw_stream is not None:
        return ctypes.c_void_p(_raw_stream(torch.cuda.current_device()))
    return ctypes.c_void_p(torch.cuda.current_stream().cuda_stream)


def _dev(*ts):
    for t in ts:
        if t is not None and not t.is_cuda:
            raise RuntimeError("vunet HIP path needs device tensors (hand-written gfx950 kernels; no CPU fallback)")
        if t is not None and t.dtype != torch.float32:
            raise RuntimeError(f"vunet HIP path computes in fp32, got {t.dtype}")


def _call(name: str, *args):
    rc = getattr(_lib.lib(), name)(*args)
    if rc != 0:
        raise RuntimeError(f"{name} failed with code {rc}")


def _c(t: Optional[torch.Tensor]) -> Optional[torch.Tensor]:
    return None if t is None else (t if t.is_contiguous() else t.contiguous())


def _r2(x: int) -> int:
    return (x + 1) // 2 * 2


def _r32(x: int) -> int:
    return (x + 31) // 32 * 32


_drop_state = {"base": None, "ctr": 0, "step": None, "host_step": 0}


def set_dropout_seed(seed: int):
    _drop_state["base"] = int(seed) & 0xFFFFFFFF
    _drop_state["ctr"] = 0


def set_dropout_host_step(step: int):
    _drop_state["host_step"] = int(step) & 0xFFFFFFFF


def reset_dropout_counter():
    if _drop_state["base"] is None:
        set_dropout_seed(torch.initial_seed())
    _drop_state["ctr"] = 0


def set_dropout_step(counter: Optional[torch.Tensor]):
    if counter is not None and not (counter.is_cuda and counter.dtype == torch.int32 and counter.numel() == 1):
        raise RuntimeError("dropout step counter: one int32 element on the GPU")
    _drop_state["step"] = counter
    _call("vunet_set_dropout_step", _p(counter))


def dropout_step_counter() -> Optional[torch.Tensor]:
    return _drop_state["step"]


def next_dropout_seed() -> int:
    if _drop_state["base"] is None:
        set_dropout_seed(torch.initial_seed())
    _drop_state["ctr"] += 1
    x = (_drop_state["base"] * 0x9E3779B1 + _drop_state["ctr"] * 0x85EBCA77) & 0xFFFFFFFF
    x ^= x >> 15
    return ((x * 0x2C1B3C6D) + _drop_state["host_step"] * 0x9E3779B1) & 0xFFFFFFFF


@dataclass
class ConvCfg:
    kind: int = 0
    k: int = 3
    stride: int = 1
    pad: int = 0
    in_act: int = ACT_NONE
    in_slope: float = 0.0
    drop_p: float = 0.0
    drop_seed: int = 0
    out_act: int = ACT_NONE
    d2s: bool = False
    res_is_x1: bool = False
    owner: object = None
    bf16: bool = False
    passthrough: bool = False


def conv_out_size(h: int, k: int, stride: int, pad: int) -> int:
    return (h + 2 * pad - k) // stride + 1


_SCHEMES = {"f32": 0, "x6": 1, "h2": 2}
_conv_precision = {"mode": os.environ.get("VUNET_CONV_SCHEME", "h2")}


def set_conv_precision(mode: str):
    if mode not in _SCHEMES:
        raise ValueError(f"unknown conv precision {mode!r} (h2 | x6 | f32)")
    _conv_precision["mode"] = mode


def conv_precision() -> str:
    return _conv_precision["mode"]


def _scheme() -> int:
    return _SCHEMES[_conv_precision["mode"]]


_wants_split_cache = {}
_TUNING_KEYS = {"split_force_nt": 0, "tiled_force_nt": 1, "force_small": 2, "blk_force_nt": 3, "parity_launches": 4, "blk_ws": 5, "wgrad_rowsplit": 6, "s2_fwd_f32": 7, "p2_form": 8,
                "p2_terms": 9}
_tuning_values = {}


def set_tuning(key: str, value: int):
    _call("vunet_set_tuning", _TUNING_KEYS[key], int(value))
    _tuning_values[key] = int(value)
    _wants_split_cache.clear()


def tuning(key: str) -> int:
    _TUNING_KEYS[key]
    return _tuning_values.get(key, 0)


def apply_env_tuning():
    spec = os.environ.get("VUNET_TUNING", "")
    for kv in filter(None, (t.strip() for t in spec.split(","))):
        k, _, v = kv.partition("=")
        set_tuning(k.strip(), int(v))


def absmax_partials(x1, x2=None):
    out = torch.empty(1024, device=x1.device, dtype=torch.float32)
    _call("vunet_absmax_partials", _p(x1), x1.numel(), _p(x2), 0 if x2 is None else x2.numel(), _p(out), _stream())
    return out


_amax_arena = {}


def _new_amax_out(dev):
    idx = dev.index if dev.index is not None else torch.cuda.current_device()
    key = (idx, _raw_stream(idx) if _raw_stream is not None else 0)
    a = _amax_arena.get(key)
    if a is None or a[1] >= a[0].shape[0]:
        a = _amax_arena[key] = [torch.zeros(128, 1024, device=dev, dtype=torch.float32), 0]
    a[1] += 1
    return a[0][a[1] - 1]


def _zero_scalar(dev, shape=(1,)):
    idx = dev.index if dev.index is not None else torch.cuda.current_device()
    key = (idx, _raw_stream(idx) if _raw_stream is not None else 0)
    z = _zero_rows.get(key)
    if z is None or z[1] + 16 > z[0].numel():
        z = _zero_rows[key] = [_new_amax_out(dev), 0]
    z[1] += 16
    return z[0][z[1] - 16:z[1] - 15].view(shape)


_zero_rows = {}
_amax_retired = []


def _reset_amax_arena():
    _amax_retired[:] = [list(_amax_arena.values())]
    _amax_arena.clear()
    _zero_rows.clear()


def _tag_amax(t, buf):
    t._vunet_amax = (buf, t._version)


def _tagged_amax(t):
    rec = getattr(t, "_vunet_amax", None)
    return rec[0] if rec is not None and rec[1] == t._version else None


def carry_amax_tag(src, dst):
    tag = _tagged_amax(src)
    if tag is not None:
        _tag_amax(dst, tag)
    if _is_relu_out(src):
        _tag_relu_out(dst)


_relu_premask = os.environ.get("VUNET_RELU_PREMASK", "1") != "0"


def enable_relu_premask(on: bool = True):
    global _relu_premask
    _relu_premask = bool(on)


def _tag_relu_out(t):
    t._vunet_relu_out = t._version


def _is_relu_out(t) -> bool:
    return t is not None and getattr(t, "_vunet_relu_out", None) == t._version


def _tag_masked(g, by):
    g._vunet_masked = (by.data_ptr(), g._version)


def _is_masked_by(g, y) -> bool:
    rec = getattr(g, "_vunet_masked", None)
    return rec is not None and y is not None and rec[0] == y.data_ptr() and rec[1] == g._version


def _amax_for(x1, x2=None):
    t1 = _tagged_amax(x1)
    if x2 is None:
        return t1 if t1 is not None else absmax_partials(x1)
    t2 = _tagged_amax(x2)
    if t1 is None and t2 is None:
        return absmax_partials(x1, x2)
    return (t1 if t1 is not None else absmax_partials(x1), t2 if t2 is not None else absmax_partials(x2))


def _amax_pair(amax):
    return amax if isinstance(amax, tuple) else (amax, None)


def _publishes_amax(desc, has_aux: bool, has_res: bool, has_wx: bool) -> bool:
    key = ("p", desc.N, desc.C1, desc.C2, desc.Hs, desc.Ws, desc.M, desc.m_off, desc.Mpad, desc.Ho, desc.Wo, desc.KH,
           desc.stride, desc.pad, desc.mode, desc.in_act, desc.drop_p > 0, desc.out_act, desc.d2s, desc.aux_act,
           desc.aux_drop_p > 0, has_aux, has_res, has_wx)
    r = _wants_split_cache.get(key)
    if r is None:
        r = _wants_split_cache[key] = _lib.lib().vunet_conv2d_publishes_amax(ctypes.byref(desc), int(has_aux),
                                                                             int(has_res), 2 if has_wx else 0) == 1
    return r


def _wgrad_wants_split(wd) -> bool:
    key = ("w", wd.N, wd.C1, wd.C2, wd.Hs, wd.Ws, wd.Cout, wd.Ho, wd.Wo, wd.KH, wd.stride, wd.pad, wd.flags & 1)
    r = _wants_split_cache.get(key)
    if r is None:
        r = _wants_split_cache[key] = _lib.lib().vunet_conv2d_wgrad_wants_split(ctypes.byref(wd)) == 1
    return r


def _wants_split(desc, has_aux: bool, has_res: bool, has_mask: bool = False) -> bool:
    key = (desc.N, desc.C1, desc.C2, desc.Hs, desc.Ws, desc.M, desc.m_off, desc.Mpad, desc.Ho, desc.Wo, desc.KH, desc.stride,
           desc.pad, desc.mode, desc.in_act, desc.drop_p > 0, desc.out_act, desc.d2s, desc.aux_act, desc.aux_drop_p > 0,
           has_aux, has_res, has_mask, _scheme())
    r = _wants_split_cache.get(key)
    if r is None:
        r = _wants_split_cache[key] = _lib.lib().vunet_conv2d_wants_split(ctypes.byref(desc), int(has_aux), int(has_res),
                                                                          int(has_mask), _scheme()) == 1
    return r


def x6_mtiles(m: int) -> int:
    return (((m + 31) // 32 + 1) + 1) & ~1


def x6_image_units(cout: int, c1: int, c2: int, k: int, dgrad: bool, split: int = 1) -> int:
    if k != 3:
        return 0
    slab, hdr = (384, 1) if split == 2 else (576, 0)
    if dgrad:
        return (cout // 16) * 3 * x6_mtiles(c1 + c2) * slab + hdr if cout % 16 == 0 else 0
    return ((c1 + c2) // 16) * 3 * x6_mtiles(cout) * slab + hdr if (c1 % 16 == 0 and c2 % 16 == 0) else 0


def _alloc_x6(cout, c1, c2, k, dgrad, dev):
    if _scheme() == 0:
        return None
    n = x6_image_units(cout, c1, c2, k, dgrad, _scheme())
    return torch.zeros(n * 4, device=dev, dtype=torch.int32) if n else None


def pack_weights(v, g, bias, gamma, beta, c1: int, c2: int, kind: int, need_dgrad: bool):
    cout, ctot, kh, kw = v.shape
    assert ctot == c1 + c2
    t = kh * kw
    dev = v.device
    wt_f = torch.empty(t * (_r2(c1) + _r2(c2)), _r32(cout), device=dev, dtype=torch.float32)
    wt_d = torch.empty(t * _r2(cout), _r32(ctot), device=dev, dtype=torch.float32) if need_dgrad else None
    wx_f = _alloc_x6(cout, c1, c2, kh, False, dev) if kh == kw else None
    wx_d = _alloc_x6(cout, c1, c2, kh, True, dev) if (need_dgrad and kh == kw) else None
    small = torch.empty(4, cout, device=dev, dtype=torch.float32)
    d = WnDesc(cout, c1, c2, kh, kw, kind, _scheme())
    _call("vunet_weightnorm_fwd", ctypes.byref(d), _p(v), _p(g), _p(bias), _p(gamma), _p(beta), _p(wt_f), _p(wt_d),
          _p(wx_f), _p(wx_d), _p(small[0]), _p(small[1]), _p(small[2]), _p(small[3]), _stream())
    return wt_f, wt_d, small[0], small[1], small[2], wx_f, wx_d


_prof = {"on": False, "recs": []}
_NO_TIMER = contextlib.nullcontext()


def profile_start():
    _prof["on"], _prof["recs"] = True, []


def profile_stop(detail: bool = False, by_kernel: bool = False):
    _prof["on"] = False
    if _prof["recs"]:
        torch.cuda.synchronize()
    fam = {}
    for name, flop, e0, e1 in _prof["recs"]:
        if by_kernel:
            name = name[-1]
        elif not detail:
            name = name[0]
        f = fam.setdefault(name, {"ms": 0.0, "flop": 0.0, "n": 0})
        f["ms"] += e0.elapsed_time(e1)
        f["flop"] += flop
        f["n"] += 1
    _prof["recs"] = []
    return fam


class _Timed:
    def __init__(self, name, flop):
        self.name, self.flop = name, flop

    def __enter__(self):
        if _prof["on"]:
            self.e0 = torch.cuda.Event(enable_timing=True)
            self.e1 = torch.cuda.Event(enable_timing=True)
            self.e0.record()

    def __exit__(self, *a):
        if _prof["on"]:
            self.e1.record()
            _prof["recs"].append((self.name, self.flop, self.e0, self.e1))


def _conv_gather(desc: ConvDesc, x1, x2, wt, shift, res, aux, y, wx=None, amax=None, res2=None):
    t = desc.KH * desc.KW
    scheme = _scheme() if wx is not None else 0
    amax_out = None
    if scheme == 2:
        if _wants_split(desc, aux is not None, res is not None):
            if amax is None:
                amax = _amax_for(x1, x2)
        else:
            wx = amax = None
    else:
        amax = None
    if _scheme() == 2 and _publishes_amax(desc, aux is not None, res is not None, wx is not None):
        amax_out = _new_amax_out(y.device)
    if desc.mode == 0:
        name, flop = "conv_gather_fwd", 2.0 * desc.N * desc.Ho * desc.Wo * desc.M * (desc.C1 + desc.C2) * t
    else:
        name, flop = "conv_gather_dgrad", 2.0 * desc.N * desc.Hs * desc.Ws * desc.C1 * desc.M * t
    kname = ""
    if _prof["on"]:
        buf = ctypes.create_string_buffer(96)
        _call("vunet_conv2d_variant", ctypes.byref(desc), 0 if aux is None else 1, 0 if wx is None else scheme, 0, buf, 96)
        kname = buf.value.decode()
    with (_Timed((name, desc.N, desc.C1, desc.C2, desc.Hs, desc.Ws, desc.M, desc.KH, desc.stride, desc.in_act, kname),
                flop) if _prof["on"] else _NO_TIMER):
        a1, a2 = _amax_pair(amax)
        rc = _lib.lib().vunet_conv2d_a2(ctypes.byref(desc), _p(x1), _p(x2), _p(wt), _p(wx), _p(shift), _p(res), _p(res2),
                                        _p(aux), _p(y), _p(a1), _p(a2), _p(amax_out), _stream())
        if rc == -3 and res2 is not None:
            _call("vunet_conv2d_a2", ctypes.byref(desc), _p(x1), _p(x2), _p(wt), _p(wx), _p(shift), _p(res), None, _p(aux),
                  _p(y), _p(a1), _p(a2), None, _stream())
            y.add_(res2)
            amax_out = None
        elif rc != 0:
            raise RuntimeError(f"vunet_conv2d_a2 failed with code {rc}")
    if amax_out is not None:
        _tag_amax(y, amax_out)
    return amax


def _plain_pack(w, need_dgrad):
    cout, cin = w.shape[0], w.shape[1]
    return pack_weights(w.contiguous(), None, None, None, None, cin, 0, 1, need_dgrad)


def _plain_desc(n, cin, hs, ws, m, ho, wo, k, stride, pad, mode, mpad):
    return ConvDesc(N=n, C1=cin, C2=0, Hs=hs, Ws=ws, M=m, m_off=0, Mpad=mpad, Ho=ho, Wo=wo, KH=k, KW=k,
                    stride=stride, pad=pad, mode=mode, in_act=ACT_NONE, in_slope=0.0, drop_p=0.0, drop_seed=0,
                    out_act=ACT_NONE, d2s=0, aux_act=ACT_NONE, aux_slope=0.0, aux_drop_p=0.0, aux_drop_seed=0)


class ConvPlainFwd(torch.autograd.Function):

    @staticmethod
    def forward(ctx, x, w, stride, pad):
        _dev(x, w)
        x, w = _c(x), _c(w)
        n, cin, hs, ws = x.shape
        cout, _, k, _ = w.shape
        ho, wo = conv_out_size(hs, k, stride, pad), conv_out_size(ws, k, stride, pad)
        pk = _plain_pack(w, False)
        wt_f = pk[0]
        y = torch.empty(n, cout, ho, wo, device=x.device, dtype=torch.float32)
        _conv_gather(_plain_desc(n, cin, hs, ws, cout, ho, wo, k, stride, pad, 0, wt_f.shape[1]), x, None, wt_f, None,
                     None, None, y, pk[5])
        ctx.save_for_backward(x, w)
        ctx.geo = (stride, pad)
        return y

    @staticmethod
    def backward(ctx, gy):
        x, w = ctx.saved_tensors
        stride, pad = ctx.geo
        gx = ConvPlainDgrad.apply(gy, w, x.shape[2], x.shape[3], stride, pad) if ctx.needs_input_grad[0] else None
        gw = ConvPlainWgrad.apply(x, gy, w.shape[2], stride, pad) if ctx.needs_input_grad[1] else None
        return gx, gw, None, None


class ConvPlainDgrad(torch.autograd.Function):

    @staticmethod
    def forward(ctx, dy, w, hs, ws, stride, pad):
        _dev(dy, w)
        dy, w = _c(dy), _c(w)
        n, cout, ho, wo = dy.shape
        cin, k = w.shape[1], w.shape[2]
        pk = _plain_pack(w, True)
        wt_d = pk[1]
        dx = torch.empty(n, cin, hs, ws, device=dy.device, dtype=torch.float32)
        _conv_gather(_plain_desc(n, cout, ho, wo, cin, hs, ws, k, stride, pad, 1, wt_d.shape[1]), dy, None, wt_d, None,
                     None, None, dx, pk[6])
        ctx.save_for_backward(dy, w)
        ctx.geo = (stride, pad)
        return dx

    @staticmethod
    def backward(ctx, gdx):
        dy, w = ctx.saved_tensors
# ... 1256 lines not shown
```

include/vunet_hip.h:

```cpp
#ifndef VUNET_HIP_H
#define VUNET_HIP_H
#include <stddef.h>
#include <stdint.h>

#ifdef __cplusplus
extern "C" {
#endif

#define VUNET_OK 0
#define VUNET_ERR_ARG (-1)
#define VUNET_ERR_LAUNCH (-2)
#define VUNET_ERR_UNSUPPORTED (-3)

#define VUNET_ACT_NONE 0
#define VUNET_ACT_ELU 1
#define VUNET_ACT_RELU 2
#define VUNET_ACT_SIGMOID 3
#define VUNET_ACT_LRELU 4

int vunet_abi_version(void);

typedef struct vunet_conv_desc {
  int32_t N;
  int32_t C1, C2;
  int32_t Hs, Ws;
  int32_t M;
  int32_t m_off;
  int32_t Mpad;
  int32_t Ho, Wo;
  int32_t KH, KW, stride, pad;
  int32_t mode;
  int32_t in_act;
  float in_slope;
  float drop_p;
  uint32_t drop_seed;
  int32_t out_act;
  int32_t d2s;
  int32_t aux_act;
  float aux_slope;
  float aux_drop_p;
  uint32_t aux_drop_seed;
} vunet_conv_desc;

int vunet_conv2d_gather(const vunet_conv_desc* d, const float* x1, const float* x2, const float* wt,
                        const float* shift, const float* res, const float* aux, float* y, void* stream);

int vunet_conv2d_dgrad_relu(const vunet_conv_desc* d, const float* dy, const float* y, const float* wt,
                            const float* res, float* dx, void* stream);

int vunet_conv2d_gather_variant(const vunet_conv_desc* d, int32_t has_aux, char* name, int32_t len);

int vunet_conv2d(const vunet_conv_desc* d, const float* x1, const float* x2, const float* wt, const void* wx,
                 const float* shift, const float* res, const float* aux, float* y, const float* amax, float* amax_out,
                 void* stream);
int vunet_conv2d_a2(const vunet_conv_desc* d, const float* x1, const float* x2, const float* wt, const void* wx,
                    const float* shift, const float* res, const float* res2, const float* aux, float* y, const float* amax,
                    const float* amax2, float* amax_out, void* stream);
int vunet_conv2d_x6(const vunet_conv_desc* d, const float* x1, const float* x2, const void* wx, const float* shift,
                    const float* res, const float* aux, const float* mask, float* y, const float* amax, float* amax_out,
                    void* stream);
int vunet_conv2d_x6_supported(const vunet_conv_desc* d, int32_t has_mask);
int vunet_conv2d_wants_split(const vunet_conv_desc* d, int32_t has_aux, int32_t has_res, int32_t has_mask, int32_t split);
int vunet_conv2d_dgrad_relu_x6(const vunet_conv_desc* d, const float* dy, const float* y, const void* wx,
                               const float* res, float* dx, const float* amax, float* amax_out, void* stream);
int vunet_conv2d_publishes_amax(const vunet_conv_desc* d, int32_t has_aux, int32_t has_res, int32_t split);
int vunet_absmax_partials(const float* x1, int64_t n1, const float* x2, int64_t n2, float* out, void* stream);
int vunet_conv2d_variant(const vunet_conv_desc* d, int32_t has_aux, int32_t has_wx, int32_t has_mask, char* name,
                         int32_t len);

int vunet_conv2d_bf16_supported(const vunet_conv_desc* d);
int vunet_pack_bf16(const float* wt_f, void* wb, int32_t C1, int32_t C2, int32_t Mpad, void* stream);
int vunet_conv2d_bf16(const vunet_conv_desc* d, const float* x1, const float* x2, const void* wb,
                      const float* shift, const float* res, float* y, void* stream);

int vunet_conv2d_blk(const vunet_conv_desc* d, const void* x1, const void* x2, const void* wb, const float* shift,
                     const void* res, void* y, int32_t y_fp32_nchw, void* stream);
int vunet_conv2d_blk_rnb_supported(const vunet_conv_desc* d);
int vunet_conv2d_blk_rnb(const vunet_conv_desc* d, const void* x, const void* skip, const void* wb_nin, const float* shift_nin,
                         int32_t Mpad_nin, const void* wb, const float* shift, const void* res, void* y, void* stream);
int vunet_conv2d_blk_tiled(const vunet_conv_desc* d);
int vunet_pack_bf16_taps(const float* wt_f, void* wb, int32_t C1, int32_t C2, int32_t Mpad, int32_t taps, void* stream);
int vunet_nchw_to_blk(const float* x, void* y, int32_t N, int32_t C, int32_t H, int32_t W, void* stream);
int vunet_blk_to_nchw(const void* x, float* y, int32_t N, int32_t C, int32_t H, int32_t W, void* stream);
int vunet_conv1x1_few_to_blk(const float* x, const float* wt_f, const float* shift, void* y, int32_t N, int32_t C,
                             int32_t H, int32_t W, int32_t M, int32_t Mpad, void* stream);

typedef struct vunet_wgrad_desc {
  int32_t N, C1, C2, Hs, Ws;
  int32_t Cout, Ho, Wo;
  int32_t KH, KW, stride, pad;
  int32_t in_act;
  float in_slope;
  float drop_p;
  uint32_t drop_seed;
  int32_t nsplit;
  int32_t flags;
} vunet_wgrad_desc;

int vunet_conv2d_wgrad(const vunet_wgrad_desc* d, const float* x1, const float* x2, const float* dy,
                       float* slabs, float* dshift, const float* amax_x, const float* amax_dy, void* stream);
int vunet_conv2d_wgrad_a2(const vunet_wgrad_desc* d, const float* x1, const float* x2, const float* dy,
                          float* slabs, float* dshift, const float* amax_x, const float* amax_x2, const float* amax_dy,
                          void* stream);
typedef struct vunet_wgrad_item {
  vunet_wgrad_desc d;
  const float* x1;
  const float* x2;
  const float* dy;
  float* slabs;
  float* dshift;
  const float* amax_x;
  const float* amax_x2;
  const float* amax_dy;
} vunet_wgrad_item;
int vunet_conv2d_wgrad_multi(const vunet_wgrad_item* items, int32_t n, void* stream);
int vunet_conv2d_wgrad_batchable(const vunet_wgrad_desc* d);
int vunet_conv2d_wgrad_wants_split(const vunet_wgrad_desc* d);
int vunet_conv2d_wgrad_variant(const vunet_wgrad_desc* d, char* name, int32_t len);
int vunet_conv2d_wgrad_nsplit(const vunet_wgrad_desc* d);

typedef struct vunet_wn_desc {
  int32_t Cout, C1, C2, KH, KW;
  int32_t kind;
  int32_t split;
} vunet_wn_desc;

int vunet_weightnorm_fwd(const vunet_wn_desc* d, const float* v, const float* g, const float* bias,
                         const float* gamma, const float* beta, float* wt_f, float* wt_d, void* wx_f, void* wx_d,
                         float* scale, float* shift, float* invnorm, float* wmax, void* stream);

typedef struct vunet_wn_item {
  const float *v, *g, *bias, *gamma, *beta;
  float *wt_f, *wt_d, *scale, *shift, *invnorm;
  void *wx_f, *wx_d;
  float* wmax;
  vunet_wn_desc d;
} vunet_wn_item;
int vunet_weightnorm_fwd_multi(const vunet_wn_item* items_dev, int32_t n_items, int32_t max_cout, void* stream);
int vunet_x6_image_bytes(const vunet_wn_desc* d, int32_t dgrad);
int vunet_x6_mtiles(int32_t M);

int vunet_weightnorm_bwd(const vunet_wn_desc* d, const float* slabs, const float* dshift, int32_t nsplit,
                         const float* v, const float* g, const float* bias, const float* gamma,
                         const float* invnorm, float* dv, float* dg, float* dbias, float* dgamma,
                         float* dbeta, float* workspace, int32_t accumulate, void* stream);

typedef struct vunet_wn_bwd_item {
  const float *slabs, *dshift, *v, *g, *bias, *gamma, *invnorm;
  float *dv, *dg, *dbias, *dgamma, *dbeta;
  float* workspace;
  vunet_wn_desc d;
  int32_t nsplit, accumulate;
} vunet_wn_bwd_item;
int vunet_weightnorm_bwd_multi(const vunet_wn_bwd_item* items_dev, int32_t n_items, int32_t max_cout,
                               int32_t max_reduce_blocks, void* stream);

int vunet_depth_to_space(const float* x, float* y, int32_t N, int32_t C, int32_t H, int32_t W, void* stream);
int vunet_space_to_depth(const float* x, float* y, int32_t N, int32_t C, int32_t H, int32_t W, void* stream);

int vunet_upsample_bilinear2x_fwd(const float* x, float* y, int64_t NC, int32_t H, int32_t W, void* stream);
int vunet_upsample_bilinear2x_bwd(const float* dy, float* dx, int64_t NC, int32_t H, int32_t W, void* stream);

int vunet_axpby(const float* x, const float* y_in, float* y, float a, float b, int64_t n, void* stream);
int vunet_act_bwd_from_out(const float* y, const float* dy, float* dx, int32_t act, float slope, int64_t n,
                           void* stream);
int vunet_act_fwd(const float* x, float* y, int32_t act, float slope, int64_t n, void* stream);

int vunet_reparam_fwd(const float* mu, const float* logstd, const float* eps, float* z, int64_t n, void* stream);
int vunet_reparam_bwd(const float* dz, const float* logstd, const float* eps, float* dmu, float* dlogstd,
                      int64_t n, void* stream);

int vunet_l1_mean_fwd(const float* a, const float* b, float* partial, float* out, float weight, int64_t n,
                      void* stream);
int vunet_l1_mean_bwd(const float* a, const float* b, const float* add, float* db, float gscale,
                      const float* gout, int64_t n, void* stream);
int vunet_l1_mean_bwd_amax(const float* a, const float* b, const float* add, float* db, float gscale,
                           const float* gout, int64_t n, float* amax_out, int32_t relu_mask, void* stream);

int vunet_kl_fwd(const float* mu, const float* logstd, float* partial, float* out, float weight, int32_t N, int64_t D,
                 void* stream);
int vunet_kl_bwd(const float* mu, const float* logstd, float* dmu, float* dlogstd, float gscale,
                 const float* gout, int64_t n, void* stream);
int vunet_sqdiff_fwd(const float* p, const float* q, float* partial, float* out, float weight, int32_t N, int64_t D,
                     void* stream);
int vunet_sqdiff_bwd(const float* p, const float* q, float* dp, float* dq, float gscale, const float* gout,
                     int64_t n, void* stream);

int vunet_vgg_preprocess(const float* x, float* y, int32_t N, int32_t H, int32_t W, void* stream);
int vunet_vgg_preprocess_bwd(const float* dy, const float* add, float* dx, int32_t N, int32_t H, int32_t W,
                             void* stream);
int vunet_maxpool2_fwd(const float* x, float* y, int32_t NC, int32_t H, int32_t W, void* stream);
int vunet_l1_pool_fwd(const float* a, const float* b, float* partial, float* out, float* y, float weight, int32_t NC,
                      int32_t H, int32_t W, void* stream);
int vunet_l1_pool_bwd(const float* a, const float* b, const float* dy_pool, float* db, float gscale, const float* gout,
                      int32_t NC, int32_t H, int32_t W, float* amax_out, int32_t relu_mask, void* stream);
int vunet_maxpool2_bwd_relu(const float* x, const float* y, const float* dy, float* dx, int32_t NC, int32_t H, int32_t W,
                            void* stream);
int vunet_maxpool2_bwd(const float* x, const float* y, const float* dy, float* dx, int32_t NC, int32_t H,
                       int32_t W, void* stream);

int vunet_instnorm_fwd(const float* x, float* y, float* stats, int32_t NC, int32_t HW, float eps, void* stream);
int vunet_instnorm_bwd(const float* y, const float* dy, const float* stats, float* dx, int32_t NC, int32_t HW,
                       void* stream);

int vunet_adam_step(float* param, const float* grad, float* exp_avg, float* exp_avg_sq, int64_t n, float lr,
                    float beta1, float beta2, float eps, float weight_decay, int32_t step, float grad_scale,
                    void* stream);

int vunet_adam_step_dev(float* param, const float* grad, float* exp_avg, float* exp_avg_sq, int64_t n,
                        const double* lr_dev, float beta1, float beta2, float eps, float weight_decay,
                        const int64_t* step_dev, float grad_scale, void* stream);

int vunet_set_dropout_step(const uint32_t* step_dev);

#define VUNET_TUNE_SPLIT_FORCE_NT 0
#define VUNET_TUNE_TILED_FORCE_NT 1
#define VUNET_TUNE_FORCE_SMALL 2
#define VUNET_TUNE_BLK_FORCE_NT 3
#define VUNET_TUNE_PARITY_LAUNCHES 4
#define VUNET_TUNE_BLK_WS 5
#define VUNET_TUNE_WGRAD_ROWSPLIT 6
#define VUNET_TUNE_S2_FWD_F32 7
#define VUNET_TUNE_P2_FORM 8
#define VUNET_TUNE_P2_TERMS 9
#define VUNET_TUNE_COUNT 10
int vunet_set_tuning(int32_t key, int32_t value);

int vunet_dropout_mask(float* mask, int64_t n, float p, uint32_t seed, void* stream);

int vunet_stickman_raster(const float* kps, int32_t B, int32_t J, const int32_t* body, int32_t n_body,
                          const int32_t* cmds, int32_t n_cmds, uint8_t* out_u8, float* out_f32, int32_t H, int32_t W,
                          void* stream);
int vunet_stickman_raster_thick(const float* kps, int32_t B, int32_t J, const int32_t* body, int32_t n_body,
                                const int32_t* cmds, int32_t n_cmds, uint8_t* out_u8, float* out_f32, int32_t H, int32_t W,
                                int32_t thickness, void* stream);
int vunet_u8_to_unit(const uint8_t* in, float* out, int64_t n, void* stream);

int vunet_ssim_partial(const float* x, const float* y, int32_t planes, int32_t H, int32_t W, float data_range,
                       const float* window11, float* partial, void* stream);

int vunet_dp_available(void);
int vunet_dp_unique_id(void* id128);
int vunet_dp_init(int32_t world, int32_t rank, const void* id128);
int vunet_dp_world(void);
int vunet_dp_allreduce_bucket(float* buf, int64_t n, int32_t average, void* stream);
int vunet_dp_finalize(void);

int vunet_crop_window(const float* x, float* y, int32_t planes, int32_t H, int32_t W, int32_t P, const int32_t* off,
                      void* stream);
int vunet_crop_window_bwd(const float* dy, float* dx, int32_t planes, int32_t H, int32_t W, int32_t P, const int32_t* off,
                          void* stream);

#define VUNET_LOSS_MAX_TERMS 8
int vunet_total_loss(const float* const* terms, int32_t n, const float* kl, const float* gamma, float gamma_const,
                     float ll_weight, int32_t use_kl, float* loss, float* ll, void* stream);
int vunet_total_loss_bwd(const float* g_loss, const float* g_ll, int32_t n, const float* gamma, float gamma_const,
                         float ll_weight, int32_t use_kl, float* d, void* stream);
int vunet_gamma_update(float* gamma, const float* imax, const float* avg_kl, float gamma_step, void* stream);

int vunet_unit_sample(const float* mu, const float* logstd, float* z, float* eps_out, int64_t n, uint32_t seed, void* stream);

int vunet_set_schedule(double* lr_dev, double lr, float* imax_dev, float imax, int32_t* step_dev, int32_t step, void* stream);

int vunet_sum_amax(const float* const* srcs, int32_t n, float* out, float* amax_out, int64_t numel, void* stream);

typedef struct vunet_p2_desc {
  int32_t N, C, H, W;
  int32_t M;
  int32_t relu;
} vunet_p2_desc;
int vunet_p2_conv_supported(const vunet_p2_desc* d);
int vunet_p2_conv_variant(const vunet_p2_desc* d, char* name, int32_t len);
int vunet_p2_conv(const vunet_p2_desc* d, const void* x, const int32_t* xmeta, const void* w_image, const float* wk,
                  const float* shift, const void* mask, void* y, int32_t* ymeta, void* stream);
int vunet_p2_weight_image_bytes(int32_t Cout, int32_t Cin, int32_t dgrad);
int vunet_p2_pack_weights(const float* w, const float* shift, int32_t Cout, int32_t Cin, int32_t dgrad, void* image, float* wk,
                          float* workspace, void* stream);
int vunet_p2_weight_bound(const float* w, const float* shift, int32_t Cout, int32_t Cin, float* wk, float* workspace, void* stream);
int vunet_p2_conv_first(const float* x, const float* amax_x, int32_t n_amax, const float* wt_f, int32_t Mpad, const float* shift,
                        const float* wk, void* y, int32_t* ymeta, int32_t N, int32_t H, int32_t W, int32_t M, void* stream);
int vunet_p2_from_nchw(const float* x, const float* amax, int32_t n_amax, int32_t relu, void* y, int32_t* ymeta, int32_t N,
                       int32_t C, int32_t H, int32_t W, void* stream);
int vunet_p2_to_nchw(const void* x, const int32_t* xmeta, float* y, int32_t N, int32_t C, int32_t H, int32_t W, void* stream);

int vunet_p2_l1_fwd(const void* t, const int32_t* tmeta, const void* p, const int32_t* pmeta, float* partial, float* out,
                    float weight, int32_t N, int32_t C, int32_t H, int32_t W, void* stream);
int vunet_p2_pool_fwd(const void* t, const int32_t* tmeta, const void* p, const int32_t* pmeta, float* partial, float* out,
                      float weight, void* y, int32_t* ymeta, int32_t N, int32_t C, int32_t H, int32_t W, void* stream);
int vunet_p2_l1_bwd(const void* t, const int32_t* tmeta, const void* p, const int32_t* pmeta, const void* add,
                    const int32_t* addmeta, void* g, int32_t* gmeta, float gscale, const float* gout, int32_t N, int32_t C,
                    int32_t H, int32_t W, void* stream);
int vunet_p2_pool_bwd(const void* t, const int32_t* tmeta, const void* p, const int32_t* pmeta, const void* dy,
                      const int32_t* dymeta, void* g, int32_t* gmeta, float gscale, const float* gout, int32_t N, int32_t C,
                      int32_t H, int32_t W, void* stream);

typedef struct vunet_seq_linear_desc {
  int32_t B, M, K, ldx, act0, act1, nets, shared_in, S;
} vunet_seq_linear_desc;
typedef struct vunet_seq_coupling_desc {
  int32_t B, C, c1, ld_in, ld_out, Mp, reverse, affine_on_src, S;
} vunet_seq_coupling_desc;
typedef struct vunet_seq_lstm_desc {
  int32_t B, H, ldx, hoff, n, ldraw;
  int64_t seq_stride;
} vunet_seq_lstm_desc;
int vunet_seq_linear(const vunet_seq_linear_desc* d, const float* w0, const float* w1, const float* x, const float* bias0,
                     const float* bias1, float* y, void* stream);
int vunet_seq_coupling(const vunet_seq_coupling_desc* d, const float* in, const float* st, const float* bias_s, const float* bias_t,
                       const int32_t* map, const float* scale, const float* loc, float* out, float* logdet, void* stream);
int vunet_seq_start(const float* x0, int64_t x0_stride, const float* h0, const float* c0, float* xraw, int32_t ldraw, float* xh,
                    int32_t ldx, int32_t hoff, float* c, int32_t B, int32_t n, int32_t H, void* stream);
int vunet_seq_lstm_gates(const vunet_seq_lstm_desc* d, const float* w_perm, const float* xh, const float* bias_perm, const float* c_in,
                         float* c_out, float* xh_next, float* h_out, const float* x_next, void* stream);
int vunet_seq_decoder_out(const vunet_seq_lstm_desc* d, float* xh, const float* w_out, const float* b_out, float* xraw, float* xs,
                          float* cs, void* stream);
int vunet_seq_lstm_bias(const float* b_ih, const float* b_hh, const float* fold, int32_t H, float* bias_perm, void* stream);
int vunet_seq_fold_input(const float* w_ih, const float* w_in, const float* b_in, int32_t M, int32_t n, float* w_fold,
                         float* bias_fold, void* stream);
int vunet_seq_bottleneck(const float* heads, int32_t Mp, const float* eps, float* mu, float* logstd, float* b_out, int32_t B,
                         int32_t H, void* stream);
int vunet_seq_pack_rows(const float* src, int32_t M, int32_t K, const float* row_scale, float* dst, int32_t ld_dst, int32_t col_off,
                        int32_t row_off, int32_t row_mul, void* stream);
int vunet_seq_pose_project(const float* x, int32_t n_use, const int32_t* dims_to_use, const double* mean, const double* stdv, int32_t D,
                           int32_t f32_math, const double* cam, float* kps, int32_t T, int32_t J, void* stream);
int vunet_seq_actnorm_init(const float* x, int32_t ld, int32_t B, int32_t C, float* loc, float* scale, void* stream);
int vunet_seq_normlinear_rows(const float* v, const float* g, const float* bias, const float* gamma, const float* beta, int32_t M,
                              int32_t K, float* row_scale, float* bias_eff, void* stream);

int vunet_seq_slerp(const float* b1, const float* b2, int64_t ld_in, int pairs, int h, const double* steps, int n_steps, float* out,
                    void* stream);

#ifdef __cplusplus
}
#endif
#endif
```

Measured before the change: 799.4 frames/s.

## Add intra-block K-split to h2 conv kernels for low-occupancy layers

Moves the h2 conv kernel body into a shared header instantiated with KS=1 and KS=2. The KS=2 variant splits the input-channel chunks between two wave groups, each with its own LDS staging area, so that convs with too few blocks to fill the device get more parallel work per block. A routing heuristic turns the split on for stride-1, NT=1 routes when the block count is at most the CU count, and an env override plus a query API are added. The cost is doubled LDS per block and an extra cross-group reduction of the accumulators.

```diff
diff --git a/behavior_driven_video_synthesis_amd/csrc/common.h b/behavior_driven_video_synthesis_amd/csrc/common.h
--- a/behavior_driven_video_synthesis_amd/csrc/common.h
+++ b/behavior_driven_video_synthesis_amd/csrc/common.h
@@ -120,6 +120,8 @@
   }
 
 extern int g_vunet_tune[16];
+extern int g_vunet_ksplit;
+int vunet_cu_count();
 
 static inline int vunet_check_launch() {
   hipError_t e = hipGetLastError();
diff --git a/behavior_driven_video_synthesis_amd/csrc/conv_h2_kernel.h b/behavior_driven_video_synthesis_amd/csrc/conv_h2_kernel.h
--- a/behavior_driven_video_synthesis_amd/csrc/conv_h2_kernel.h
+++ b/behavior_driven_video_synthesis_amd/csrc/conv_h2_kernel.h
@@ -25,408 +25,68 @@
 #define H2_STAMP(k_)
 #endif
 
-template <int MT, int NT, int MODE, int PRO, int PHW = -1, int NWV = 4, int TW = 32>
-__global__ __launch_bounds__(64 * NWV, (NWV == 8 || MT * NT >= 8) ? 1 : 2) void conv_h2_kernel(const GatherArgs a_in,
-                                                                             const uint4* __restrict__ wx, int mtiles_pad,
-                                                                             const float* __restrict__ amax) {
-  GatherArgs a = a_in;
-  H2_STAMP(0);
-  inact_resolve(a.in1);
-  inact_resolve(a.in2);
-  inact_resolve(a.auxa);
-  static_assert(PHW < 0 || MODE == 1, "parity phases exist for the data gradient only");
-  constexpr bool ALLP = PHW == 4;
-  static_assert(!ALLP || (NT == 1 && TW == 32 && NWV == 4 && PRO == 0), "fused parities: one dy row per wave");
-  constexpr int NQ = ALLP ? 4 : NT;
-  constexpr bool PIPE = TW == 16 && PHW < 0;
-  constexpr int PH = (PHW >= 0 && !ALLP) ? (PHW >> 1) : 0, PW = (PHW >= 0 && !ALLP) ? (PHW & 1) : 0;
-  constexpr int NKH = (PHW < 0 || ALLP) ? 3 : (PH ? 2 : 1);
-  constexpr int NTHR = 64 * NWV;
-  static_assert(TW == 32 || TW == 16, "tile width");
-  constexpr int RPQ = 32 / TW;
-  constexpr int TH = NWV * NT * RPQ, IH = TH + 2, CW = TW + 2, IW = TW == 32 ? CW : 32, PIX = IH * IW, MB = 32 * MT;
-  constexpr int XU = 2 * IH * CW;
-  constexpr int NX = (XU + NTHR - 1) / NTHR;
-  constexpr int WU = H2_SLAB * MT;
-  constexpr int GS = NWV == 8 ? NKH : 1;
-  constexpr int WUS = WU * GS;
-  extern __shared__ __attribute__((aligned(16))) uint4 smem4[];
-  uint4* const xL = smem4;
-  uint4* const wL = smem4 + 8 * PIX;
+#define H2_KS 1
+#include "conv_h2_kernel_body.h"
+#undef H2_KS
+#define H2_KS 2
+#include "conv_h2_kernel_body.h"
+#undef H2_KS
 
-  const vunet_conv_desc& d = a.d;
-  const int tid = threadIdx.x, lane = tid & 63, wave = tid >> 6;
-  const int j = lane & 31, h = lane >> 5;
-  const int jr = j / TW, jc = j % TW;
-  const int H = d.Hs, W = d.Ws, HW = a.HsWs;
-
-  const unsigned bid = xcd_remap(blockIdx.x, gridDim.x);
-  const int mblocks = (d.M + MB - 1) / MB;
-  const int mb = bid % mblocks;
-  int t = bid / mblocks;
-  const int tiles_w = W / TW, tiles_h = H / TH;
-  const int tx = t % tiles_w;
-  t /= tiles_w;
-  const int ty = t % tiles_h;
-  const int n = t / tiles_h;
-  const int row0 = ty * TH, col0 = tx * TW, m0 = mb * MB;
-
-  float sx, descale, descale2;
-
-  unsigned rel[NX];
-  int lds_x[NX];
-  uint32_t vbits = 0;
-#pragma unroll
-  for (int i = 0; i < NX; ++i) {
-    int u = tid + NTHR * i;
-    if (u >= XU) u -= XU;
-    const int c8 = u / (IH * CW);
-    const int rem = u - c8 * (IH * CW);
-    const int r = rem / CW, col = rem - r * CW;
-    const int ih = row0 - 1 + r, iw = col0 - 1 + col;
-    const bool ok = (unsigned)ih < (unsigned)H && (unsigned)iw < (unsigned)W;
-    rel[i] = ok ? (unsigned)(8 * c8 * HW + ih * W + iw) : 0u;
-    lds_x[i] = c8 * PIX + r * IW + col;
-    vbits |= (ok ? 1u : 0u) << i;
-  }
-
-  f32x16 acc[MT][NQ], acx[MT][NQ];
-#pragma unroll
-  for (int mt = 0; mt < MT; ++mt)
-#pragma unroll
-    for (int q = 0; q < NQ; ++q)
-#pragma unroll
-      for (int r = 0; r < 16; ++r) acc[mt][q][r] = acx[mt][q][r] = 0.f;
-
-  const int nch1 = d.C1 / 16, nch = nch1 + d.C2 / 16;
-  float xv[NX][8];
-  float mk[1][8];
-  const int mt0 = (d.m_off + m0) >> 5;
-
-  auto issue_x = [&](int ch, int i) {
-    const bool second = ch >= nch1;
-    const int cs = second ? (ch - nch1) * 16 : ch * 16;
-    const int C = second ? d.C2 : d.C1;
-    const float* __restrict__ xs = (second ? a.x2 : a.x1) + (size_t)(n * C + cs) * HW;
-#pragma unroll
-    for (int k = 0; k < 8; ++k)
-      xv[i][k] = *reinterpret_cast<const float*>(reinterpret_cast<const char*>(xs) +
-                                                 4u * (rel[i] + (((vbits >> i) & 1u) ? (unsigned)(k * HW) : 0u)));
-  };
-  auto issue_mask = [&](int ch, int i) {
-    if constexpr (PRO == 4) {
-      const float* __restrict__ ms = a.mask + (size_t)(n * d.C1 + ch * 16) * HW;
-#pragma unroll
-      for (int k = 0; k < 8; ++k)
-        mk[0][k] = *reinterpret_cast<const float*>(reinterpret_cast<const char*>(ms) +
-                                                   4u * (rel[i] + (((vbits >> i) & 1u) ? (unsigned)(k * HW) : 0u)));
-    }
-  };
-  auto write_x = [&](int ch, int i) {
-    const bool second = ch >= nch1;
-    const int cs = second ? (ch - nch1) * 16 : ch * 16;
-    const int C = second ? d.C2 : d.C1;
-    InAct ia = a.in1;
-    ia.seed = second ? a.in2.seed : a.in1.seed;
-    const int gbase = (n * C + cs) * HW;
-    const bool ok = (vbits >> i) & 1u;
-    float v[8];
-#pragma unroll
-    for (int k = 0; k < 8; ++k) {
-      float t_ = ok ? xv[i][k] : 0.f;
-      if constexpr (PRO == 4) t_ = mk[0][k] > 0.f ? t_ : 0.f;
-      else if constexpr (PRO != 0) t_ = prologue<PRO>(ia, t_, (uint32_t)gbase + rel[i] + (uint32_t)(k * HW));
-      v[k] = t_ * sx;
-    }
-    uint4 ph, pl;
-    h2_split2(v[0], v[1], ph.x, pl.x);
-    h2_split2(v[2], v[3], ph.y, pl.y);
-    h2_split2(v[4], v[5], ph.z, pl.z);
-    h2_split2(v[6], v[7], ph.w, pl.w);
-    uint4* const xb = xL + (ch & 1) * 4 * PIX;
-    xb[lds_x[i]] = ph;
-    xb[2 * PIX + lds_x[i]] = pl;
-  };
-  constexpr int WPS = WU / 64;
-  constexpr int NWI = (GS * WPS + NWV - 1) / NWV;
-  const int wave_u = __builtin_amdgcn_readfirstlane(wave);
-  const uint32_t wL_addr = (uint32_t)(uintptr_t)(__attribute__((address_space(3))) void*)wL;
-  auto slab_of = [&](int step) {
-    if constexpr (PHW < 0 || ALLP) return step;
-    else if constexpr (PH == 0) return step * 3 + 1;
-    else return (step >> 1) * 3 + ((step & 1) ? 2 : 0);
-  };
-  auto issue_w = [&](int stage, int buf) {
-#pragma unroll
-    for (int i = 0; i < NWI; ++i) {
-      int wi = wave_u + NWV * i;
-      if (wi >= GS * WPS) wi -= GS * WPS;
-      const int g = wi / WPS, r = wi - g * WPS;
-      const char* wp = reinterpret_cast<const char*>(wx) + 16 +
-                       ((size_t)slab_of(stage * GS + g) * mtiles_pad + mt0) * (H2_SLAB * 16);
-      h2_dma16(wp + (size_t)(r * 64 + lane) * 16, wL_addr + (uint32_t)(buf * WUS + g * WU + r * 64) * 16u);
-    }
-  };
-
-  issue_w(0, 0);
-#pragma unroll
-  for (int i = 0; i < NX; ++i) issue_x(0, i);
-  {
-    const float4 pm = h2_amax4(amax, a.amax2, tid & 255);
-    float m_ = fmaxf(fmaxf(pm.x, pm.y), fmaxf(pm.z, pm.w));
-    m_ = wave_max(m_);
-    float* const redm = reinterpret_cast<float*>(smem4);
-    if (lane == 0) redm[wave] = m_;
-    __syncthreads();
-    m_ = fmaxf(fmaxf(redm[0], redm[1]), fmaxf(redm[2], redm[3]));
-    __syncthreads();
-    if (a.in1.thresh) m_ *= a.in1.keep_scale;
-    const int ex = h2_scale_exp(m_);
-    const int ew = reinterpret_cast<const int*>(wx)[0];
-    sx = h2_pow2(ex);
-    h2_pow2_pair(-(ex + ew), descale, descale2);
-  }
-  H2_STAMP(1);
-
-#pragma unroll
-  for (int i = 0; i < NX; ++i) {
-    issue_mask(0, i);
-    write_x(0, i);
-  }
-  h2_dma_wait();
-  __syncthreads();
-  H2_STAMP(2);
-
-  const uint4* const xB0 = xL + h * PIX + (wave * NT * RPQ + jr) * IW + jc;
-  const uint4* const wA = wL + h * 32 + j;
-  auto chunk = [&](int ch, auto last_c) {
-    constexpr bool LAST = decltype(last_c)::value;
-#pragma unroll
-    for (int ki = 0; ki < NKH; ++ki) {
-      const int kh = (PHW < 0 || ALLP) ? ki : (PH ? 2 * ki : 1);
-      const int ph_t = ALLP ? ((kh + 1) & 1) : PH;
-      const int phase = ch * NKH + ki;
-      const int stage = phase / GS, g = phase - stage * GS;
-      const int buf = stage & 1;
-      const bool stage_begin = g == 0, stage_end = g == GS - 1;
-      const bool more_w = !(LAST && ki == NKH - 1);
-      const uint4* const xB = xB0 + (ch & 1) * 4 * PIX;
-      if constexpr (!LAST) {
-#pragma unroll
-        for (int i = 0; i < NX; ++i)
-          if (i * NKH / NX == ki) issue_x(ch + 1, i);
-      }
-      if (stage_begin && !(LAST && GS == NKH) && (GS == NKH || more_w)) issue_w(stage + 1, buf ^ 1);
-      const int dr = PHW >= 0 ? (ph_t + 1 - kh) / 2 + 1 : (MODE == 0 ? kh : 2 - kh);
-      if constexpr (PIPE) {
-        H2Unit fa[2][2][MT], fb[2][2][NT];
-        auto rd = [&](int kw, H2Unit (&av)[2][MT], H2Unit (&bv)[2][NT]) {
-          const int dc = MODE == 0 ? kw : 2 - kw;
-#pragma unroll
-          for (int p = 0; p < 2; ++p) {
-#pragma unroll
-            for (int mt = 0; mt < MT; ++mt) av[p][mt].u = wA[buf * WUS + g * WU + ((mt * 3 + kw) * 2 + p) * 64];
-#pragma unroll
-            for (int q = 0; q < NT; ++q) bv[p][q].u = xB[p * 2 * PIX + (q * RPQ + dr) * IW + dc];
-          }
-        };
-        rd(0, fa[0], fb[0]);
-#pragma unroll
-        for (int kw = 0; kw < 3; ++kw) {
-          __builtin_amdgcn_sched_barrier(0);
-          if (kw + 1 < 3) rd(kw + 1, fa[(kw + 1) & 1], fb[(kw + 1) & 1]);
-          __builtin_amdgcn_sched_barrier(0);
-#pragma unroll
-          for (int mt = 0; mt < MT; ++mt)
-#pragma unroll
-            for (int q = 0; q < NT; ++q) {
-              f32x16 cx = acx[mt][q];
-              cx = __builtin_amdgcn_mfma_f32_32x32x16_f16(fa[kw & 1][1][mt].b, fb[kw & 1][0][q].b, cx, 0, 0, 0);
-              cx = __builtin_amdgcn_mfma_f32_32x32x16_f16(fa[kw & 1][0][mt].b, fb[kw & 1][1][q].b, cx, 0, 0, 0);
-              acx[mt][q] = cx;
-              acc[mt][q] = __builtin_amdgcn_mfma_f32_32x32x16_f16(fa[kw & 1][0][mt].b, fb[kw & 1][0][q].b, acc[mt][q], 0, 0, 0);
-            }
-        }
-      } else
-#pragma unroll
-      for (int kw = 0; kw < 3; ++kw) {
-        if (PHW >= 0 && !ALLP && ((kw + PW) & 1) == 0) continue;
-        const int pw_t = ALLP ? ((kw + 1) & 1) : PW;
-        const int par = ph_t * 2 + pw_t;
-        if constexpr (MT * NT < 8) __builtin_amdgcn_sched_barrier(0);
-        const int dc = PHW >= 0 ? (pw_t + 1 - kw) / 2 + 1 : (MODE == 0 ? kw : 2 - kw);
-        H2Unit av[2][MT], bv[2][NT];
-#pragma unroll
-        for (int p = 0; p < 2; ++p) {
-#pragma unroll
-          for (int mt = 0; mt < MT; ++mt) av[p][mt].u = wA[buf * WUS + g * WU + ((mt * 3 + kw) * 2 + p) * 64];
-#pragma unroll
-          for (int q = 0; q < NT; ++q) bv[p][q].u = xB[p * 2 * PIX + (q * RPQ + dr) * IW + dc];
-        }
-#pragma unroll
-        for (int mt = 0; mt < MT; ++mt)
-#pragma unroll
-          for (int q = 0; q < NT; ++q) {
-            const int qa = ALLP ? par : q;
-            f32x16 cx = acx[mt][qa];
-            cx = __builtin_amdgcn_mfma_f32_32x32x16_f16(av[1][mt].b, bv[0][q].b, cx, 0, 0, 0);
-            cx = __builtin_amdgcn_mfma_f32_32x32x16_f16(av[0][mt].b, bv[1][q].b, cx, 0, 0, 0);
-            acx[mt][qa] = cx;
-            acc[mt][qa] = __builtin_amdgcn_mfma_f32_32x32x16_f16(av[0][mt].b, bv[0][q].b, acc[mt][qa], 0, 0, 0);
-          }
-      }
-      __builtin_amdgcn_sched_barrier(0);
-      if constexpr (!LAST) {
-#pragma unroll
-        for (int i = 0; i < NX; ++i)
-          if (i * NKH / NX == ki) {
-            issue_mask(ch + 1, i);
-            write_x(ch + 1, i);
-          }
-      }
-      if (stage_end && more_w) {
-        h2_dma_wait();
-        __syncthreads();
-      }
-    }
-  };
-  for (int ch = 0; ch + 1 < nch; ++ch) {
-    chunk(ch, std::false_type{});
-#ifdef H2_TSTAMP
-    if (ch == 0) H2_STAMP(6);
-#endif
-  }
-  chunk(nch - 1, std::true_type{});
-  H2_STAMP(3);
-
-  auto geo = [&](int q) {
-    PixGeo g;
-    g.n = n;
-    const int orow = row0 + (wave * NT + q) * RPQ + jr, ocol = col0 + jc;
-    g.oh = PHW >= 0 ? 2 * orow + PH : orow;
-    g.ow = PHW >= 0 ? 2 * ocol + PW : ocol;
-    g.valid = true;
-    return g;
-  };
-  auto combined = [&](auto tc) {
-    constexpr int t = decltype(tc)::value, q = t / MT, mt = t % MT;
-    f32x16 c;
-#pragma unroll
-    for (int r = 0; r < 16; ++r) c[r] = (acc[mt][q][r] + acx[mt][q][r] * (1.f / 2048.f)) * descale * descale2;
-    return c;
-  };
-  float ymax = 0.f;
-  auto publish = [&]() {
-    if (a.amax_out) {
-      const float m_ = wave_max(ymax);
-      if (lane == 0) atomicMax(reinterpret_cast<unsigned*>(a.amax_out) + ((blockIdx.x * 4u + wave) & 511u), __float_as_uint(m_));
-    }
-  };
-  if constexpr (ALLP) {
-    const int orow = row0 + wave + jr, ocol = col0 + jc;
-#pragma unroll
-    for (int mt = 0; mt < MT; ++mt)
-#pragma unroll
-      for (int ph = 0; ph < 2; ++ph) {
-        f32x16 c0, c1;
-#pragma unroll
-        for (int r = 0; r < 16; ++r) {
-          c0[r] = (acc[mt][2 * ph][r] + acx[mt][2 * ph][r] * (1.f / 2048.f)) * descale * descale2;
-          c1[r] = (acc[mt][2 * ph + 1][r] + acx[mt][2 * ph + 1][r] * (1.f / 2048.f)) * descale * descale2;
-        }
-        ymax = fmaxf(ymax, store_tile_pair(a, n, 2 * orow + ph, 2 * ocol, m0 + 32 * mt, h, c0, c1));
-      }
-    publish();
-    return;
-  }
-  if (PHW < 0 && a.wide) {
-    const int k = lane & 3;
-    TileSide4 side[2];
-    auto tile = [&](auto tc, auto form_c) {
-      constexpr int t = decltype(tc)::value, q = t / MT, mt = t % MT, FORM = decltype(form_c)::value;
-      if constexpr (t == 0) load_tile_side4<MODE, FORM>(a, geo(0), m0, h, k, side[0]);
-      if constexpr (t + 1 < MT * NT)
-        load_tile_side4<MODE, FORM>(a, geo((t + 1) / MT), m0 + 32 * ((t + 1) % MT), h, k, side[(t + 1) & 1]);
-      ymax = fmaxf(ymax, store_tile_side4<MODE, FORM>(a, geo(q), m0 + 32 * mt, h, k, combined(tc), side[t & 1]));
-    };
-    auto tiles = [&](auto form_c) {
-      tile(std::integral_constant<int, 0>{}, form_c);
-      if constexpr (MT * NT > 1) tile(std::integral_constant<int, 1>{}, form_c);
-      if constexpr (MT * NT > 2) {
-        tile(std::integral_constant<int, 2>{}, form_c);
-        tile(std::integral_constant<int, 3>{}, form_c);
-      }
-      if constexpr (MT * NT > 4) {
-        tile(std::integral_constant<int, 4>{}, form_c);
-        tile(std::integral_constant<int, 5>{}, form_c);
-        tile(std::integral_constant<int, 6>{}, form_c);
-        tile(std::integral_constant<int, 7>{}, form_c);
-      }
-    };
-    const int form = side4_form<MODE>(a);
-    if (form == 1) tiles(std::integral_constant<int, 1>{});
-    else if (MODE == 1 && form == 2) tiles(std::integral_constant<int, MODE == 1 ? 2 : 0>{});
-    else if (MODE == 1 && form == 3) tiles(std::integral_constant<int, MODE == 1 ? 3 : 0>{});
-    else tiles(std::integral_constant<int, 0>{});
-    static_assert(MT * NT <= 8, "epilogue tiles are named at compile time");
-    publish();
-#ifdef H2_TSTAMP
-    H2_STAMP(4);
-    asm volatile("s_waitcnt vmcnt(0)" ::: "memory");
-    H2_STAMP(5);
-#endif
-    return;
-  }
-  TileSide side[2];
-  load_tile_side(a, geo(0), m0, h, side[0]);
-  auto tile = [&](auto tc) {
-    constexpr int t = decltype(tc)::value, q = t / MT, mt = t % MT;
-    if constexpr (t + 1 < MT * NT) load_tile_side(a, geo((t + 1) / MT), m0 + 32 * ((t + 1) % MT), h, side[(t + 1) & 1]);
-    ymax = fmaxf(ymax, store_tile_side(a, geo(q), m0 + 32 * mt, h, combined(tc), side[t & 1]));
-  };
-  tile(std::integral_constant<int, 0>{});
-  if constexpr (MT * NT > 1) tile(std::integral_constant<int, 1>{});
-  if constexpr (MT * NT > 2) {
-    tile(std::integral_constant<int, 2>{});
-    tile(std::integral_constant<int, 3>{});
-  }
-  if constexpr (MT * NT > 4) {
-    tile(std::integral_constant<int, 4>{});
-    tile(std::integral_constant<int, 5>{});
-    tile(std::integral_constant<int, 6>{});
-    tile(std::integral_constant<int, 7>{});
-  }
-  publish();
-}
-
-template <int MT, int NT, int MODE, int PRO, int PHW, int NWV, int TW = 32>
+template <int MT, int NT, int MODE, int PRO, int PHW, int NWV, int TW = 32, int KS = 1>
 static int launch_h2_one(const GatherArgs& ga, const void* wx, int mtiles_pad, const float* amax, hipStream_t st) {
   constexpr int RPQ = 32 / TW;
   constexpr int PIX = (NWV * NT * RPQ + 2) * (TW == 32 ? 34 : 32);
   constexpr int NKH = (PHW < 0 || PHW == 4) ? 3 : ((PHW >> 1) ? 2 : 1);
-  constexpr size_t lds = (size_t)(8 * PIX + 2 * H2_SLAB * MT * (NWV == 8 ? NKH : 1)) * 16;
+  constexpr size_t lds = (size_t)KS * (8 * PIX + 2 * H2_SLAB * MT * (NWV == 8 ? NKH : 1)) * 16;
   const vunet_conv_desc& d = ga.d;
   const int blocks = d.N * (d.Hs / (NWV * NT * RPQ)) * (d.Ws / TW) * ((d.M + 32 * MT - 1) / (32 * MT));
-  auto kern = conv_h2_kernel<MT, NT, MODE, PRO, PHW, NWV, TW>;
-  if (lds > 64 * 1024 &&
-      hipFuncSetAttribute((const void*)kern, hipFuncAttributeMaxDynamicSharedMemorySize, (int)lds) != hipSuccess)
-    return VUNET_ERR_LAUNCH;
-  VUNET_LAUNCH(kern, dim3((unsigned)blocks), dim3(64 * NWV), lds, st, ga, (const uint4*)wx, mtiles_pad, amax);
-  return vunet_check_launch();
+  if constexpr (KS == 2) {
+    static_assert(lds <= 160 * 1024, "two staging areas in the CU's LDS");
+    if ((d.C1 / 16 + d.C2 / 16) % 2 != 0) return VUNET_ERR_ARG;
+    auto kern = conv_h2_ks2_kernel<MT, NT, MODE, PRO, TW>;
+    static const bool attr_ok =
+        hipFuncSetAttribute((const void*)kern, hipFuncAttributeMaxDynamicSharedMemorySize, (int)lds) == hipSuccess;
+    if (!attr_ok) return VUNET_ERR_LAUNCH;
+    VUNET_LAUNCH(kern, dim3((unsigned)blocks), dim3(512), lds, st, ga, (const uint4*)wx, mtiles_pad, amax);
+    return vunet_check_launch();
+  } else {
+    auto kern = conv_h2_kernel<MT, NT, MODE, PRO, PHW, NWV, TW>;
+    if (lds > 64 * 1024 &&
+        hipFuncSetAttribute((const void*)kern, hipFuncAttributeMaxDynamicSharedMemorySize, (int)lds) != hipSuccess)
+      return VUNET_ERR_LAUNCH;
+    VUNET_LAUNCH(kern, dim3((unsigned)blocks), dim3(64 * NWV), lds, st, ga, (const uint4*)wx, mtiles_pad, amax);
+    return vunet_check_launch();
+  }
 }
 
-template <int MT>
+template <int MT, int KS = 1>
 static int launch_h2_w16(const GatherArgs& ga, const void* wx, int mtiles_pad, const float* amax, int pro, hipStream_t st) {
   if (ga.d.mode == 1) {
     if (ga.d.stride != 1) return VUNET_ERR_UNSUPPORTED;
-    if (pro == 4) return launch_h2_one<MT, 1, 1, 4, -1, 4, 16>(ga, wx, mtiles_pad, amax, st);
-    if (pro == 0) return launch_h2_one<MT, 1, 1, 0, -1, 4, 16>(ga, wx, mtiles_pad, amax, st);
+    if (pro == 4) return launch_h2_one<MT, 1, 1, 4, -1, 4, 16, KS>(ga, wx, mtiles_pad, amax, st);
+    if (pro == 0) return launch_h2_one<MT, 1, 1, 0, -1, 4, 16, KS>(ga, wx, mtiles_pad, amax, st);
     return VUNET_ERR_UNSUPPORTED;
   }
   switch (pro) {
-    case 0: return launch_h2_one<MT, 1, 0, 0, -1, 4, 16>(ga, wx, mtiles_pad, amax, st);
-    case 1: return launch_h2_one<MT, 1, 0, 1, -1, 4, 16>(ga, wx, mtiles_pad, amax, st);
-    case 2: return launch_h2_one<MT, 1, 0, 2, -1, 4, 16>(ga, wx, mtiles_pad, amax, st);
+    case 0: return launch_h2_one<MT, 1, 0, 0, -1, 4, 16, KS>(ga, wx, mtiles_pad, amax, st);
+    case 1: return launch_h2_one<MT, 1, 0, 1, -1, 4, 16, KS>(ga, wx, mtiles_pad, amax, st);
+    case 2: return launch_h2_one<MT, 1, 0, 2, -1, 4, 16, KS>(ga, wx, mtiles_pad, amax, st);
+    default: return VUNET_ERR_UNSUPPORTED;
+  }
+}
+
+template <int MT, int NT>
+static int launch_h2_ks2(const GatherArgs& ga, const void* wx, int mtiles_pad, const float* amax, int pro, hipStream_t st) {
+  if (ga.d.stride != 1) return VUNET_ERR_UNSUPPORTED;
+  if (ga.d.mode == 1) {
+    if (pro == 4) return launch_h2_one<MT, NT, 1, 4, -1, 4, 32, 2>(ga, wx, mtiles_pad, amax, st);
+    if (pro == 0) return launch_h2_one<MT, NT, 1, 0, -1, 4, 32, 2>(ga, wx, mtiles_pad, amax, st);
+    return VUNET_ERR_UNSUPPORTED;
+  }
+  switch (pro) {
+    case 0: return launch_h2_one<MT, NT, 0, 0, -1, 4, 32, 2>(ga, wx, mtiles_pad, amax, st);
+    case 1: return launch_h2_one<MT, NT, 0, 1, -1, 4, 32, 2>(ga, wx, mtiles_pad, amax, st);
+    case 2: return launch_h2_one<MT, NT, 0, 2, -1, 4, 32, 2>(ga, wx, mtiles_pad, amax, st);
     default: return VUNET_ERR_UNSUPPORTED;
   }
 }
diff --git a/behavior_driven_video_synthesis_amd/csrc/conv_h2_kernel_body.h b/behavior_driven_video_synthesis_amd/csrc/conv_h2_kernel_body.h
--- /dev/null
+++ b/behavior_driven_video_synthesis_amd/csrc/conv_h2_kernel_body.h
@@ -0,0 +1,416 @@
+#if H2_KS == 1
+template <int MT, int NT, int MODE, int PRO, int PHW = -1, int NWV = 4, int TW = 32>
+__global__ __launch_bounds__(64 * NWV, (NWV == 8 || MT * NT >= 8) ? 1 : 2) void conv_h2_kernel(const GatherArgs a_in,
+                                                                             const uint4* __restrict__ wx, int mtiles_pad,
+                                                                             const float* __restrict__ amax) {
+#else
+template <int MT, int NT, int MODE, int PRO, int TW>
+__global__ __launch_bounds__(512, 1) void conv_h2_ks2_kernel(const GatherArgs a_in, const uint4* __restrict__ wx, int mtiles_pad,
+                                                             const float* __restrict__ amax) {
+  constexpr int PHW = -1, NWV = 4;
+#endif
+  constexpr int KS = H2_KS;
+  static_assert(KS == 1 || (KS == 2 && NWV == 4 && PHW < 0 && MT * NT < 8), "the K-split pair: two four-wave groups, stride 1");
+  GatherArgs a = a_in;
+  H2_STAMP(0);
+  inact_resolve(a.in1);
+  inact_resolve(a.in2);
+  inact_resolve(a.auxa);
+  static_assert(PHW < 0 || MODE == 1, "parity phases exist for the data gradient only");
+  constexpr bool ALLP = PHW == 4;
+  static_assert(!ALLP || (NT == 1 && TW == 32 && NWV == 4 && PRO == 0), "fused parities: one dy row per wave");
+  constexpr int NQ = ALLP ? 4 : NT;
+  constexpr bool PIPE = TW == 16 && PHW < 0;
+  constexpr int PH = (PHW >= 0 && !ALLP) ? (PHW >> 1) : 0, PW = (PHW >= 0 && !ALLP) ? (PHW & 1) : 0;
+  constexpr int NKH = (PHW < 0 || ALLP) ? 3 : (PH ? 2 : 1);
+  constexpr int NTHR = 64 * NWV;
+  static_assert(TW == 32 || TW == 16, "tile width");
+  constexpr int RPQ = 32 / TW;
+  constexpr int TH = NWV * NT * RPQ, IH = TH + 2, CW = TW + 2, IW = TW == 32 ? CW : 32, PIX = IH * IW, MB = 32 * MT;
+  constexpr int XU = 2 * IH * CW;
+  constexpr int NX = (XU + NTHR - 1) / NTHR;
+  constexpr int WU = H2_SLAB * MT;
+  constexpr int GS = NWV == 8 ? NKH : 1;
+  constexpr int WUS = WU * GS;
+  constexpr int GU = 8 * PIX + 2 * WUS;
+  extern __shared__ __attribute__((aligned(16))) uint4 smem4[];
+  const int grp = KS == 2 ? __builtin_amdgcn_readfirstlane((int)(threadIdx.x >> 8)) : 0;
+  uint4* const xL = smem4 + grp * GU;
+  uint4* const wL = xL + 8 * PIX;
+
+  const vunet_conv_desc& d = a.d;
+  const int tid = KS == 2 ? (int)(threadIdx.x & 255u) : (int)threadIdx.x, lane = tid & 63, wave = tid >> 6;
+  const int j = lane & 31, h = lane >> 5;
+  const int jr = j / TW, jc = j % TW;
+  const int H = d.Hs, W = d.Ws, HW = a.HsWs;
+
+  const unsigned bid = xcd_remap(blockIdx.x, gridDim.x);
+  const int mblocks = (d.M + MB - 1) / MB;
+  const int mb = bid % mblocks;
+  int t = bid / mblocks;
+  const int tiles_w = W / TW, tiles_h = H / TH;
+  const int tx = t % tiles_w;
+  t /= tiles_w;
+  const int ty = t % tiles_h;
+  const int n = t / tiles_h;
+  const int row0 = ty * TH, col0 = tx * TW, m0 = mb * MB;
+
+  float sx, descale, descale2;
+
+  unsigned rel[NX];
+  int lds_x[NX];
+  uint32_t vbits = 0;
+#pragma unroll
+  for (int i = 0; i < NX; ++i) {
+    int u = tid + NTHR * i;
+    if (u >= XU) u -= XU;
+    const int c8 = u / (IH * CW);
+    const int rem = u - c8 * (IH * CW);
+    const int r = rem / CW, col = rem - r * CW;
+    const int ih = row0 - 1 + r, iw = col0 - 1 + col;
+    const bool ok = (unsigned)ih < (unsigned)H && (unsigned)iw < (unsigned)W;
+    rel[i] = ok ? (unsigned)(8 * c8 * HW + ih * W + iw) : 0u;
+    lds_x[i] = c8 * PIX + r * IW + col;
+    vbits |= (ok ? 1u : 0u) << i;
+  }
+
+  f32x16 acc[MT][NQ], acx[MT][NQ];
+#pragma unroll
+  for (int mt = 0; mt < MT; ++mt)
+#pragma unroll
+    for (int q = 0; q < NQ; ++q)
+#pragma unroll
+      for (int r = 0; r < 16; ++r) acc[mt][q][r] = acx[mt][q][r] = 0.f;
+
+  const int nch1 = d.C1 / 16, nch = nch1 + d.C2 / 16;
+  const int nchg = KS == 2 ? (nch >> 1) : nch;
+  const int c0 = KS == 2 ? grp * nchg : 0;
+  float xv[NX][8];
+  float mk[1][8];
+  const int mt0 = (d.m_off + m0) >> 5;
+
+  auto issue_x = [&](int ch, int i) {
+    const bool second = ch >= nch1;
+    const int cs = second ? (ch - nch1) * 16 : ch * 16;
+    const int C = second ? d.C2 : d.C1;
+    const float* __restrict__ xs = (second ? a.x2 : a.x1) + (size_t)(n * C + cs) * HW;
+#pragma unroll
+    for (int k = 0; k < 8; ++k)
+      xv[i][k] = *reinterpret_cast<const float*>(reinterpret_cast<const char*>(xs) +
+                                                 4u * (rel[i] + (((vbits >> i) & 1u) ? (unsigned)(k * HW) : 0u)));
+  };
+  auto issue_mask = [&](int ch, int i) {
+    if constexpr (PRO == 4) {
+      const float* __restrict__ ms = a.mask + (size_t)(n * d.C1 + ch * 16) * HW;
+#pragma unroll
+      for (int k = 0; k < 8; ++k)
+        mk[0][k] = *reinterpret_cast<const float*>(reinterpret_cast<const char*>(ms) +
+                                                   4u * (rel[i] + (((vbits >> i) & 1u) ? (unsigned)(k * HW) : 0u)));
+    }
+  };
+  auto write_x = [&](int ch, int i) {
+    const bool second = ch >= nch1;
+    const int cs = second ? (ch - nch1) * 16 : ch * 16;
+    const int C = second ? d.C2 : d.C1;
+    InAct ia = a.in1;
+    ia.seed = second ? a.in2.seed : a.in1.seed;
+    const int gbase = (n * C + cs) * HW;
+    const bool ok = (vbits >> i) & 1u;
+    float v[8];
+#pragma unroll
+    for (int k = 0; k < 8; ++k) {
+      float t_ = ok ? xv[i][k] : 0.f;
+      if constexpr (PRO == 4) t_ = mk[0][k] > 0.f ? t_ : 0.f;
+      else if constexpr (PRO != 0) t_ = prologue<PRO>(ia, t_, (uint32_t)gbase + rel[i] + (uint32_t)(k * HW));
+      v[k] = t_ * sx;
+    }
+    uint4 ph, pl;
+    h2_split2(v[0], v[1], ph.x, pl.x);
+    h2_split2(v[2], v[3], ph.y, pl.y);
+    h2_split2(v[4], v[5], ph.z, pl.z);
+    h2_split2(v[6], v[7], ph.w, pl.w);
+    uint4* const xb = xL + ((ch - c0) & 1) * 4 * PIX;
+    xb[lds_x[i]] = ph;
+    xb[2 * PIX + lds_x[i]] = pl;
+  };
+  constexpr int WPS = WU / 64;
+  constexpr int NWI = (GS * WPS + NWV - 1) / NWV;
+  const int wave_u = __builtin_amdgcn_readfirstlane(wave);
+  const uint32_t wL_addr = (uint32_t)(uintptr_t)(__attribute__((address_space(3))) void*)wL;
+  auto slab_of = [&](int step) {
+    if constexpr (PHW < 0 || ALLP) return step;
+    else if constexpr (PH == 0) return step * 3 + 1;
+    else return (step >> 1) * 3 + ((step & 1) ? 2 : 0);
+  };
+  auto issue_w = [&](int stage, int buf) {
+#pragma unroll
+    for (int i = 0; i < NWI; ++i) {
+      int wi = wave_u + NWV * i;
+      if (wi >= GS * WPS) wi -= GS * WPS;
+      const int g = wi / WPS, r = wi - g * WPS;
+      const char* wp = reinterpret_cast<const char*>(wx) + 16 +
+                       ((size_t)slab_of(stage * GS + g) * mtiles_pad + mt0) * (H2_SLAB * 16);
+      h2_dma16(wp + (size_t)(r * 64 + lane) * 16, wL_addr + (uint32_t)(buf * WUS + g * WU + r * 64) * 16u);
+    }
+  };
+
+  issue_w(c0 * (NKH / GS), 0);
+#pragma unroll
+  for (int i = 0; i < NX; ++i) issue_x(c0, i);
+  {
+    const float4 pm = h2_amax4(amax, a.amax2, tid & 255);
+    float m_ = fmaxf(fmaxf(pm.x, pm.y), fmaxf(pm.z, pm.w));
+    m_ = wave_max(m_);
+    float* const redm = reinterpret_cast<float*>(xL);
+    if (lane == 0) redm[wave] = m_;
+    __syncthreads();
+    m_ = fmaxf(fmaxf(redm[0], redm[1]), fmaxf(redm[2], redm[3]));
+    __syncthreads();
+    if (a.in1.thresh) m_ *= a.in1.keep_scale;
+    const int ex = h2_scale_exp(m_);
+    const int ew = reinterpret_cast<const int*>(wx)[0];
+    sx = h2_pow2(ex);
+    h2_pow2_pair(-(ex + ew), descale, descale2);
+  }
+  H2_STAMP(1);
+
+#pragma unroll
+  for (int i = 0; i < NX; ++i) {
+    issue_mask(c0, i);
+    write_x(c0, i);
+  }
+  h2_dma_wait();
+  __syncthreads();
+  H2_STAMP(2);
+
+  const uint4* const xB0 = xL + h * PIX + (wave * NT * RPQ + jr) * IW + jc;
+  const uint4* const wA = wL + h * 32 + j;
+  auto chunk = [&](int ch, auto last_c) {
+    constexpr bool LAST = decltype(last_c)::value;
+#pragma unroll
+    for (int ki = 0; ki < NKH; ++ki) {
+      const int kh = (PHW < 0 || ALLP) ? ki : (PH ? 2 * ki : 1);
+      const int ph_t = ALLP ? ((kh + 1) & 1) : PH;
+      const int phase = ch * NKH + ki;
+      const int stage = phase / GS, g = phase - stage * GS;
+      const int buf = (((ch - c0) * NKH + ki) / GS) & 1;
+      const bool stage_begin = g == 0, stage_end = g == GS - 1;
+      const bool more_w = !(LAST && ki == NKH - 1);
+      const uint4* const xB = xB0 + ((ch - c0) & 1) * 4 * PIX;
+      if constexpr (!LAST) {
+#pragma unroll
+        for (int i = 0; i < NX; ++i)
+          if (i * NKH / NX == ki) issue_x(ch + 1, i);
+      }
+      if (stage_begin && !(LAST && GS == NKH) && (GS == NKH || more_w)) issue_w(stage + 1, buf ^ 1);
+      const int dr = PHW >= 0 ? (ph_t + 1 - kh) / 2 + 1 : (MODE == 0 ? kh : 2 - kh);
+      if constexpr (PIPE) {
+        H2Unit fa[2][2][MT], fb[2][2][NT];
+        auto rd = [&](int kw, H2Unit (&av)[2][MT], H2Unit (&bv)[2][NT]) {
+          const int dc = MODE == 0 ? kw : 2 - kw;
+#pragma unroll
+          for (int p = 0; p < 2; ++p) {
+#pragma unroll
+            for (int mt = 0; mt < MT; ++mt) av[p][mt].u = wA[buf * WUS + g * WU + ((mt * 3 + kw) * 2 + p) * 64];
+#pragma unroll
+            for (int q = 0; q < NT; ++q) bv[p][q].u = xB[p * 2 * PIX + (q * RPQ + dr) * IW + dc];
+          }
+        };
+        rd(0, fa[0], fb[0]);
+#pragma unroll
+        for (int kw = 0; kw < 3; ++kw) {
+          __builtin_amdgcn_sched_barrier(0);
+          if (kw + 1 < 3) rd(kw + 1, fa[(kw + 1) & 1], fb[(kw + 1) & 1]);
+          __builtin_amdgcn_sched_barrier(0);
+#pragma unroll
+          for (int mt = 0; mt < MT; ++mt)
+#pragma unroll
+            for (int q = 0; q < NT; ++q) {
+              f32x16 cx = acx[mt][q];
+              cx = __builtin_amdgcn_mfma_f32_32x32x16_f16(fa[kw & 1][1][mt].b, fb[kw & 1][0][q].b, cx, 0, 0, 0);
+              cx = __builtin_amdgcn_mfma_f32_32x32x16_f16(fa[kw & 1][0][mt].b, fb[kw & 1][1][q].b, cx, 0, 0, 0);
+              acx[mt][q] = cx;
+              acc[mt][q] = __builtin_amdgcn_mfma_f32_32x32x16_f16(fa[kw & 1][0][mt].b, fb[kw & 1][0][q].b, acc[mt][q], 0, 0, 0);
+            }
+        }
+      } else
+#pragma unroll
+      for (int kw = 0; kw < 3; ++kw) {
+        if (PHW >= 0 && !ALLP && ((kw + PW) & 1) == 0) continue;
+        const int pw_t = ALLP ? ((kw + 1) & 1) : PW;
+        const int par = ph_t * 2 + pw_t;
+        if constexpr (MT * NT < 8) __builtin_amdgcn_sched_barrier(0);
+        const int dc = PHW >= 0 ? (pw_t + 1 - kw) / 2 + 1 : (MODE == 0 ? kw : 2 - kw);
+        H2Unit av[2][MT], bv[2][NT];
+#pragma unroll
+        for (int p = 0; p < 2; ++p) {
+#pragma unroll
+          for (int mt = 0; mt < MT; ++mt) av[p][mt].u = wA[buf * WUS + g * WU + ((mt * 3 + kw) * 2 + p) * 64];
+#pragma unroll
+          for (int q = 0; q < NT; ++q) bv[p][q].u = xB[p * 2 * PIX + (q * RPQ + dr) * IW + dc];
+        }
+#pragma unroll
+        for (int mt = 0; mt < MT; ++mt)
+#pragma unroll
+          for (int q = 0; q < NT; ++q) {
+            const int qa = ALLP ? par : q;
+            f32x16 cx = acx[mt][qa];
+            cx = __builtin_amdgcn_mfma_f32_32x32x16_f16(av[1][mt].b, bv[0][q].b, cx, 0, 0, 0);
+            cx = __builtin_amdgcn_mfma_f32_32x32x16_f16(av[0][mt].b, bv[1][q].b, cx, 0, 0, 0);
+            acx[mt][qa] = cx;
+            acc[mt][qa] = __builtin_amdgcn_mfma_f32_32x32x16_f16(av[0][mt].b, bv[0][q].b, acc[mt][qa], 0, 0, 0);
+          }
+      }
+      __builtin_amdgcn_sched_barrier(0);
+      if constexpr (!LAST) {
+#pragma unroll
+        for (int i = 0; i < NX; ++i)
+          if (i * NKH / NX == ki) {
+            issue_mask(ch + 1, i);
+            write_x(ch + 1, i);
+          }
+      }
+      if (stage_end && more_w) {
+        h2_dma_wait();
+        __syncthreads();
+      }
+    }
+  };
+  for (int ch = c0; ch + 1 < c0 + nchg; ++ch) {
+    chunk(ch, std::false_type{});
+#ifdef H2_TSTAMP
+    if (ch == c0) H2_STAMP(6);
+#endif
+  }
+  chunk(c0 + nchg - 1, std::true_type{});
+  H2_STAMP(3);
+
+  if constexpr (KS == 2) {
+    static_assert(MT * NQ * 8 * 256 <= 2 * GU, "the fold fits the staging areas");
+    float4* const fL = reinterpret_cast<float4*>(smem4);
+    __syncthreads();
+    if (grp == 1) {
+#pragma unroll
+      for (int mt = 0; mt < MT; ++mt)
+#pragma unroll
+        for (int q = 0; q < NQ; ++q)
+#pragma unroll
+          for (int r = 0; r < 4; ++r) {
+            const f32x16 &c = acc[mt][q], &x = acx[mt][q];
+            fL[((mt * NQ + q) * 8 + r) * 256 + tid] = make_float4(c[4 * r], c[4 * r + 1], c[4 * r + 2], c[4 * r + 3]);
+            fL[((mt * NQ + q) * 8 + 4 + r) * 256 + tid] = make_float4(x[4 * r], x[4 * r + 1], x[4 * r + 2], x[4 * r + 3]);
+          }
+    }
+    __syncthreads();
+    if (grp == 1) return;
+#pragma unroll
+    for (int mt = 0; mt < MT; ++mt)
+#pragma unroll
+      for (int q = 0; q < NQ; ++q)
+#pragma unroll
+        for (int r = 0; r < 4; ++r) {
+          const float4 c = fL[((mt * NQ + q) * 8 + r) * 256 + tid], x = fL[((mt * NQ + q) * 8 + 4 + r) * 256 + tid];
+          acc[mt][q][4 * r] += c.x, acc[mt][q][4 * r + 1] += c.y, acc[mt][q][4 * r + 2] += c.z, acc[mt][q][4 * r + 3] += c.w;
+          acx[mt][q][4 * r] += x.x, acx[mt][q][4 * r + 1] += x.y, acx[mt][q][4 * r + 2] += x.z, acx[mt][q][4 * r + 3] += x.w;
+        }
+  }
+
+  auto geo = [&](int q) {
+    PixGeo g;
+    g.n = n;
+    const int orow = row0 + (wave * NT + q) * RPQ + jr, ocol = col0 + jc;
+    g.oh = PHW >= 0 ? 2 * orow + PH : orow;
+    g.ow = PHW >= 0 ? 2 * ocol + PW : ocol;
+    g.valid = true;
+    return g;
+  };
+  auto combined = [&](auto tc) {
+    constexpr int t = decltype(tc)::value, q = t / MT, mt = t % MT;
+    f32x16 c;
+#pragma unroll
+    for (int r = 0; r < 16; ++r) c[r] = (acc[mt][q][r] + acx[mt][q][r] * (1.f / 2048.f)) * descale * descale2;
+    return c;
+  };
+  float ymax = 0.f;
+  auto publish = [&]() {
+    if (a.amax_out) {
+      const float m_ = wave_max(ymax);
+      if (lane == 0) atomicMax(reinterpret_cast<unsigned*>(a.amax_out) + ((blockIdx.x * 4u + wave) & 511u), __float_as_uint(m_));
+    }
+  };
+  if constexpr (ALLP) {
+    const int orow = row0 + wave + jr, ocol = col0 + jc;
+#pragma unroll
+    for (int mt = 0; mt < MT; ++mt)
+#pragma unroll
+      for (int ph = 0; ph < 2; ++ph) {
+        f32x16 c0, c1;
+#pragma unroll
+        for (int r = 0; r < 16; ++r) {
+          c0[r] = (acc[mt][2 * ph][r] + acx[mt][2 * ph][r] * (1.f / 2048.f)) * descale * descale2;
+          c1[r] = (acc[mt][2 * ph + 1][r] + acx[mt][2 * ph + 1][r] * (1.f / 2048.f)) * descale * descale2;
+        }
+        ymax = fmaxf(ymax, store_tile_pair(a, n, 2 * orow + ph, 2 * ocol, m0 + 32 * mt, h, c0, c1));
+      }
+    publish();
+    return;
+  }
+  if (PHW < 0 && a.wide) {
+    const int k = lane & 3;
+    TileSide4 side[2];
+    auto tile = [&](auto tc, auto form_c) {
+      constexpr int t = decltype(tc)::value, q = t / MT, mt = t % MT, FORM = decltype(form_c)::value;
+      if constexpr (t == 0) load_tile_side4<MODE, FORM>(a, geo(0), m0, h, k, side[0]);
+      if constexpr (t + 1 < MT * NT)
+        load_tile_side4<MODE, FORM>(a, geo((t + 1) / MT), m0 + 32 * ((t + 1) % MT), h, k, side[(t + 1) & 1]);
+      ymax = fmaxf(ymax, store_tile_side4<MODE, FORM>(a, geo(q), m0 + 32 * mt, h, k, combined(tc), side[t & 1]));
+    };
+    auto tiles = [&](auto form_c) {
+      tile(std::integral_constant<int, 0>{}, form_c);
+      if constexpr (MT * NT > 1) tile(std::integral_constant<int, 1>{}, form_c);
+      if constexpr (MT * NT > 2) {
+        tile(std::integral_constant<int, 2>{}, form_c);
+        tile(std::integral_constant<int, 3>{}, form_c);
+      }
+      if constexpr (MT * NT > 4) {
+        tile(std::integral_constant<int, 4>{}, form_c);
+        tile(std::integral_constant<int, 5>{}, form_c);
+        tile(std::integral_constant<int, 6>{}, form_c);
+        tile(std::integral_constant<int, 7>{}, form_c);
+      }
+    };
+    const int form = side4_form<MODE>(a);
+    if (form == 1) tiles(std::integral_constant<int, 1>{});
+    else if (MODE == 1 && form == 2) tiles(std::integral_constant<int, MODE == 1 ? 2 : 0>{});
+    else if (MODE == 1 && form == 3) tiles(std::integral_constant<int, MODE == 1 ? 3 : 0>{});
+    else tiles(std::integral_constant<int, 0>{});
+    static_assert(MT * NT <= 8, "epilogue tiles are named at compile time");
+    publish();
+#ifdef H2_TSTAMP
+    H2_STAMP(4);
+    asm volatile("s_waitcnt vmcnt(0)" ::: "memory");
+    H2_STAMP(5);
+#endif
+    return;
+  }
+  TileSide side[2];
+  load_tile_side(a, geo(0), m0, h, side[0]);
+  auto tile = [&](auto tc) {
+    constexpr int t = decltype(tc)::value, q = t / MT, mt = t % MT;
+    if constexpr (t + 1 < MT * NT) load_tile_side(a, geo((t + 1) / MT), m0 + 32 * ((t + 1) % MT), h, side[(t + 1) & 1]);
+    ymax = fmaxf(ymax, store_tile_side(a, geo(q), m0 + 32 * mt, h, combined(tc), side[t & 1]));
+  };
+  tile(std::integral_constant<int, 0>{});
+  if constexpr (MT * NT > 1) tile(std::integral_constant<int, 1>{});
+  if constexpr (MT * NT > 2) {
+    tile(std::integral_constant<int, 2>{});
+    tile(std::integral_constant<int, 3>{});
+  }
+  if constexpr (MT * NT > 4) {
+    tile(std::integral_constant<int, 4>{});
+    tile(std::integral_constant<int, 5>{});
+    tile(std::integral_constant<int, 6>{});
+    tile(std::integral_constant<int, 7>{});
+  }
+  publish();
+}
diff --git a/behavior_driven_video_synthesis_amd/csrc/conv_h2_mt2.hip b/behavior_driven_video_synthesis_amd/csrc/conv_h2_mt2.hip
--- a/behavior_driven_video_synthesis_amd/csrc/conv_h2_mt2.hip
+++ b/behavior_driven_video_synthesis_amd/csrc/conv_h2_mt2.hip
@@ -1,7 +1,8 @@
 #include "conv_h2_kernel.h"
 
 int vunet_conv_h2_launch_mt2(const GatherArgs& ga, const void* wx, int mtiles_pad, const float* amax, int pro, int NT,
-                             hipStream_t st) {
+                             hipStream_t st, int ksplit) {
+  if (ksplit == 2) return NT == 1 ? launch_h2_ks2<2, 1>(ga, wx, mtiles_pad, amax, pro, st) : VUNET_ERR_UNSUPPORTED;
   if (NT == 2) return launch_h2<2, 2>(ga, wx, mtiles_pad, amax, pro, st);
   return launch_h2<2, 1>(ga, wx, mtiles_pad, amax, pro, st);
 }
diff --git a/behavior_driven_video_synthesis_amd/csrc/conv_h2_w16.hip b/behavior_driven_video_synthesis_amd/csrc/conv_h2_w16.hip
--- a/behavior_driven_video_synthesis_amd/csrc/conv_h2_w16.hip
+++ b/behavior_driven_video_synthesis_amd/csrc/conv_h2_w16.hip
@@ -1,6 +1,8 @@
 #include "conv_h2_kernel.h"
 
 int vunet_conv_h2_launch_w16(const GatherArgs& ga, const void* wx, int mtiles_pad, const float* amax, int pro, int MT,
-                             hipStream_t st) {
+                             hipStream_t st, int ksplit) {
+  if (ksplit == 2)
+    return MT == 1 ? launch_h2_w16<1, 2>(ga, wx, mtiles_pad, amax, pro, st) : launch_h2_w16<2, 2>(ga, wx, mtiles_pad, amax, pro, st);
   return MT == 1 ? launch_h2_w16<1>(ga, wx, mtiles_pad, amax, pro, st) : launch_h2_w16<2>(ga, wx, mtiles_pad, amax, pro, st);
 }
diff --git a/behavior_driven_video_synthesis_amd/csrc/conv_p2.hip b/behavior_driven_video_synthesis_amd/csrc/conv_p2.hip
--- a/behavior_driven_video_synthesis_amd/csrc/conv_p2.hip
+++ b/behavior_driven_video_synthesis_amd/csrc/conv_p2.hip
@@ -100,6 +100,20 @@
   return vunet_check_launch();
 }
 
+template <int CT>
+int p2k_launch(const P2Args& a, hipStream_t st) {
+  constexpr int XU = 4 * 2 * 10 * (CT + 2), XS = (XU + 63) / 64 * 64, WU = 64 * 4 * 2;
+  constexpr size_t lds = (size_t)2 * (XS + 2 * WU) * 16;
+  static_assert(lds <= 160 * 1024, "two staging areas in the CU's LDS");
+  if ((a.C >> 5) % 2 != 0) return VUNET_ERR_ARG;
+  const int blocks = a.N * (a.H / 8) * (a.W / CT) * (a.M / 64);
+  static const bool attr_ok =
+      hipFuncSetAttribute((const void*)conv_p2k_kernel<CT>, hipFuncAttributeMaxDynamicSharedMemorySize, (int)lds) == hipSuccess;
+  if (!attr_ok) return VUNET_ERR_LAUNCH;
+  VUNET_LAUNCH(conv_p2k_kernel<CT>, dim3((unsigned)blocks), dim3(512), lds, st, a);
+  return vunet_check_launch();
+}
+
 }
 
 static bool p2_shape_ok(const vunet_p2_desc* d) {
@@ -116,6 +130,13 @@
   const int force = g_vunet_tune[VUNET_TUNE_P2_FORM];
   const bool wide = d->M % 128 == 0 && (force == 2 || force == 3 || (force != 1 && px_tiles * (d->M / 128) >= 256));
   return wide ? 8 : 4;
+}
+
+static int p2_ksplit(const vunet_p2_desc* d, int form) {
+  if (form != 4 || g_vunet_tune[VUNET_TUNE_P2_TERMS] == 1 || g_vunet_ksplit == 1 || (d->C / 32) % 2 != 0) return 1;
+  if (g_vunet_ksplit == 2) return 2;
+  const long blocks = (long)d->N * (d->H / 8) * (d->W / (d->W == 16 ? 16 : 32)) * (d->M / 64);
+  return blocks <= vunet_cu_count() ? 2 : 1;
 }
 
 static bool p2_one_term() { return g_vunet_tune[VUNET_TUNE_P2_TERMS] == 1; }
@@ -133,6 +154,7 @@
   const int form = p2_form(d);
   if (!p2_one_term()) {
     const bool lockstep = g_vunet_tune[VUNET_TUNE_P2_FORM] == 3;
+    if (p2_ksplit(d, form) == 2) return d->W == 16 ? p2k_launch<16>(a, st) : p2k_launch<32>(a, st);
     if (d->W == 16) return form == 8 ? (lockstep ? p2_launch<8, 16, 2, 2>(a, st) : p2a_launch<16, 2>(a, st)) : p2_launch<4, 16, 1, 2>(a, st);
     return form == 8 ? (lockstep ? p2_launch<8, 32, 2, 2>(a, st) : p2a_launch<32, 2>(a, st)) : p2_launch<4, 32, 1, 2>(a, st);
   }
@@ -152,6 +174,11 @@
   if (form == 8 && g_vunet_tune[VUNET_TUNE_P2_FORM] != 3) snprintf(name, (size_t)len, "conv_p2a_kernel<%d>", d->W == 16 ? 16 : 32);
   else snprintf(name, (size_t)len, "conv_p2_kernel<%d, %d, %d>", form, d->W == 16 ? 16 : 32, form == 8 ? 2 : 1);
   return VUNET_OK;
+}
+
+extern "C" int vunet_p2_conv_ksplit(const vunet_p2_desc* d) {
+  if (!d || !p2_shape_ok(d)) return 1;
+  return p2_ksplit(d, p2_form(d));
 }
 
 namespace {
diff --git a/behavior_driven_video_synthesis_amd/csrc/conv_p2_kernel.h b/behavior_driven_video_synthesis_amd/csrc/conv_p2_kernel.h
--- a/behavior_driven_video_synthesis_amd/csrc/conv_p2_kernel.h
+++ b/behavior_driven_video_synthesis_amd/csrc/conv_p2_kernel.h
@@ -443,3 +443,241 @@
       atomicMax(reinterpret_cast<unsigned*>(a.ymeta) + P2_AMAX0 + ((blockIdx.x * NW + wave) & (P2_NSLOT - 1)), __float_as_uint(m_));
   }
 }
+
+#if P2_TERMS == 2
+template <int CT>
+__global__ __launch_bounds__(512, 1) void conv_p2k_kernel(const P2Args a) {
+  constexpr int TERMS = 2, NW = 4;
+  static_assert(CT == 32 || CT == 16, "tile width");
+  constexpr int MW = 16 * NW;
+  constexpr int RT = 8, IH = RT + 2, CW = CT + 2, XPIX = IH * CW, XU = 4 * TERMS * XPIX;
+  constexpr int NXI = (XU + 63) / 64, XS = NXI * 64;
+  constexpr int NXW = (NXI + NW - 1) / NW;
+  constexpr int WU = MW * 4 * TERMS;
+  constexpr int NWI = WU / 64 / NW;
+  constexpr int WSRC = 1024;
+  constexpr int PTR = CT / 16, NPT = 2 * PTR;
+  constexpr int GU = XS + 2 * WU;
+  extern __shared__ __attribute__((aligned(16))) uint4 smem[];
+  const int tid = threadIdx.x & 255, lane = tid & 63;
+  const int grp = __builtin_amdgcn_readfirstlane((int)(threadIdx.x >> 8));
+  const int wave = __builtin_amdgcn_readfirstlane(tid >> 6);
+  uint4* const xL = smem + grp * GU;
+  uint4* const wL = xL + XS;
+  const int rg = wave;
+  const int px = lane & 15, cg = lane >> 4;
+  const int Hp = a.H + 2, Wp = a.W + 2, CB = a.C >> 3, MB = a.M >> 3;
+
+  const unsigned bid = xcd_remap(blockIdx.x, gridDim.x);
+  const int mblocks = a.M / MW;
+  const int mb = bid % mblocks;
+  int t = bid / mblocks;
+  const int tiles_w = a.W / CT, tiles_h = a.H / RT;
+  const int tx = t % tiles_w;
+  t /= tiles_w;
+  const int ty = t % tiles_h;
+  const int n = t / tiles_h;
+  const int row0 = ty * RT, col0 = tx * CT, m0 = mb * MW;
+
+  uint32_t xoff[NXW];
+#pragma unroll
+  for (int i = 0; i < NXW; ++i) {
+    int j = wave + NW * i;
+    if (j >= NXI) j = NXI - 1;
+    int u = 64 * j + lane;
+    if (u >= XU) u = XU - 1;
+    const int p = u / (4 * XPIX);
+    int rem = u - p * 4 * XPIX;
+    const int kq = rem / XPIX;
+    rem -= kq * XPIX;
+    const int r = rem / CW, c = rem - r * CW;
+    xoff[i] = (uint32_t)((((size_t)p * a.N * CB + kq) * Hp + (row0 + r)) * Wp + col0 + c) * 16u;
+  }
+  const uint32_t xL_addr = (uint32_t)(uintptr_t)(__attribute__((address_space(3))) void*)xL;
+  const uint32_t wL_addr = (uint32_t)(uintptr_t)(__attribute__((address_space(3))) void*)wL;
+  const char* const xsrc0 = reinterpret_cast<const char*>(a.x) + (size_t)n * CB * Hp * Wp * 16;
+  const size_t xchunk = (size_t)4 * Hp * Wp * 16;
+  const char* const wsrc0 = reinterpret_cast<const char*>(a.w) + (size_t)mb * (MW / 16) * 128 * 16;
+  const size_t wslab = (size_t)(a.M / 16) * 128 * 16;
+  const uint32_t lane16 = (uint32_t)lane * 16u;
+
+  auto issue_x = [&](int ch, int i) {
+    int j = wave + NW * i;
+    if (j >= NXI) j = NXI - 1;
+    p2_dma(xoff[i], p2_uniform_ptr(xsrc0 + (size_t)ch * xchunk), xL_addr + (uint32_t)(64 * j) * 16u);
+  };
+  auto issue_w = [&](int g, int buf) {
+    const char* src = wsrc0 + (size_t)g * wslab;
+#pragma unroll
+    for (int i = 0; i < NWI; ++i) {
+      const int part = wave * NWI + i;
+      p2_dma(lane16, p2_uniform_ptr(src + (size_t)part * WSRC), wL_addr + (uint32_t)(buf * WU + part * 64) * 16u);
+    }
+  };
+
+  const int nchg = a.C >> 6;
+  const int c0 = grp * nchg;
+
+  issue_w(c0 * 9, 0);
+#pragma unroll
+  for (int i = 0; i < NXW; ++i) issue_x(c0, i);
+
+  float descale, descale2, sy;
+  {
+    const int ex = a.xmeta[0];
+    const float amax_x = p2_meta_amax(a.xmeta, lane);
+    const int ew = (int)a.wk[2];
+    h2_pow2_pair(-(ex + ew), descale, descale2);
+    const float bound = a.wk[0] * amax_x + a.wk[1];
+    const int ey = h2_scale_exp(bound);
+    sy = h2_pow2(ey);
+    if (blockIdx.x == 0 && threadIdx.x == 0) a.ymeta[0] = ey;
+  }
+
+  f32x4 acc[4][NPT], acx[4][NPT];
+#pragma unroll
+  for (int mt = 0; mt < 4; ++mt)
+#pragma unroll
+    for (int q = 0; q < NPT; ++q)
+#pragma unroll
+      for (int r = 0; r < 4; ++r) acc[mt][q][r] = acx[mt][q][r] = 0.f;
+
+  p2_dma_wait<0>();
+  __syncthreads();
+
+  const uint4* const wA0 = wL + lane;
+  const uint4* const xB = xL + cg * XPIX + px + (2 * rg) * CW;
+
+  auto chunk = [&](int ch, auto last_c) {
+    constexpr bool LAST = decltype(last_c)::value;
+    const int wpar = ((ch - c0) * 9) & 1;
+#pragma unroll
+    for (int tap = 0; tap < 9; ++tap) {
+      const int kh = tap / 3, kw = tap - 3 * kh;
+      const int g = ch * 9 + tap;
+      const int buf = wpar ^ (tap & 1);
+      const bool more_w = !(LAST && tap == 8);
+      if (more_w) issue_w(g + 1, buf ^ 1);
+      const uint4* const wA = wA0 + buf * WU;
+      P2Unit av[TERMS][4], bv[TERMS][NPT];
+#pragma unroll
+      for (int p = 0; p < TERMS; ++p) {
+#pragma unroll
+        for (int mt = 0; mt < 4; ++mt) av[p][mt].u = wA[(mt * TERMS + p) * 64];
+#pragma unroll
+        for (int q = 0; q < NPT; ++q) bv[p][q].u = xB[p * 4 * XPIX + (q / PTR + kh) * CW + (q % PTR) * 16 + kw];
+      }
+#pragma unroll
+      for (int mt = 0; mt < 4; ++mt)
+#pragma unroll
+        for (int q = 0; q < NPT; ++q)
+          acx[mt][q] = __builtin_amdgcn_mfma_f32_16x16x32_f16(av[1][mt].b, bv[0][q].b, acx[mt][q], 0, 0, 0);
+#pragma unroll
+      for (int mt = 0; mt < 4; ++mt)
+#pragma unroll
+        for (int q = 0; q < NPT; ++q)
+          acx[mt][q] = __builtin_amdgcn_mfma_f32_16x16x32_f16(av[0][mt].b, bv[1][q].b, acx[mt][q], 0, 0, 0);
+#pragma unroll
+      for (int mt = 0; mt < 4; ++mt)
+#pragma unroll
+        for (int q = 0; q < NPT; ++q)
+          acc[mt][q] = __builtin_amdgcn_mfma_f32_16x16x32_f16(av[0][mt].b, bv[0][q].b, acc[mt][q], 0, 0, 0);
+      __builtin_amdgcn_sched_barrier(0);
+      if (more_w) {
+        p2_dma_wait<0>();
+        __syncthreads();
+        if (tap == 8) {
+#pragma unroll
+          for (int i = 0; i < NXW; ++i) issue_x(ch + 1, i);
+          p2_dma_wait<0>();
+          __syncthreads();
+        }
+      }
+    }
+  };
+  for (int ch = c0; ch + 1 < c0 + nchg; ++ch) chunk(ch, std::false_type{});
+  chunk(c0 + nchg - 1, std::true_type{});
+
+  {
+    constexpr int NPC = NPT / 2;
+    static_assert(16 * 256 <= 2 * GU, "a piece fits the staging areas");
+    f32x4* const fL = reinterpret_cast<f32x4*>(smem);
+#pragma unroll
+    for (int pc = 0; pc < NPC; ++pc) {
+      __syncthreads();
+      if (grp == 1) {
+#pragma unroll
+        for (int i = 0; i < 8; ++i) {
+          const int mt = (pc * 8 + i) / NPT, q = (pc * 8 + i) % NPT;
+          fL[(2 * i) * 256 + tid] = acc[mt][q];
+          fL[(2 * i + 1) * 256 + tid] = acx[mt][q];
+        }
+      }
+      __syncthreads();
+      if (grp == 0) {
+#pragma unroll
+        for (int i = 0; i < 8; ++i) {
+          const int mt = (pc * 8 + i) / NPT, q = (pc * 8 + i) % NPT;
+          acc[mt][q] += fL[(2 * i) * 256 + tid];
+          acx[mt][q] += fL[(2 * i + 1) * 256 + tid];
+        }
+      }
+    }
+    if (grp == 1) return;
+  }
+
+  const bool relu = a.relu != 0;
+  const size_t plane = (size_t)a.N * MB * Hp * Wp;
+  float ymax = 0.f;
+#pragma unroll
+  for (int mt = 0; mt < 4; ++mt) {
+    const int co = m0 + 16 * mt + 4 * cg;
+    float sh[4] = {0.f, 0.f, 0.f, 0.f};
+    if (a.shift) {
+      const float4 s4 = *reinterpret_cast<const float4*>(a.shift + co);
+      sh[0] = s4.x; sh[1] = s4.y; sh[2] = s4.z; sh[3] = s4.w;
+    }
+#pragma unroll
+    for (int qp = 0; qp < NPT; qp += 2) {
+      uint32_t hh[2][2], ll[2][2];
+#pragma unroll
+      for (int s = 0; s < 2; ++s) {
+        float v[4];
+#pragma unroll
+        for (int r = 0; r < 4; ++r) {
+          float c = (acc[mt][qp + s][r] + acx[mt][qp + s][r] * (1.f / 2048.f)) * descale * descale2 + sh[r];
+          c = (relu && !(c > 0.f)) ? 0.f : c;
+          ymax = fmaxf(ymax, fabsf(c));
+          v[r] = c * sy;
+        }
+        h2_split2(v[0], v[1], hh[s][0], ll[s][0]);
+        h2_split2(v[2], v[3], hh[s][1], ll[s][1]);
+      }
+      p2_swap16(hh[0][0], hh[1][0]);
+      p2_swap16(hh[0][1], hh[1][1]);
+      p2_swap16(ll[0][0], ll[1][0]);
+      p2_swap16(ll[0][1], ll[1][1]);
+      uint4 uh = make_uint4(hh[0][0], hh[0][1], hh[1][0], hh[1][1]);
+      uint4 ul = make_uint4(ll[0][0], ll[0][1], ll[1][0], ll[1][1]);
+      const int q = qp + (cg & 1);
+      const int orow = row0 + 2 * rg + q / PTR, ocol = col0 + (q % PTR) * 16 + px;
+      const int cb = ((m0 + 16 * mt) >> 3) + (cg >> 1);
+      const size_t o = (((size_t)n * MB + cb) * Hp + (orow + 1)) * Wp + (ocol + 1);
+      if (a.mask) {
+        const uint4 mh = a.mask[o], ml = a.mask[plane + o];
+        const uint32_t k0 = p2_nonzero_halves((mh.x | ml.x) & 0x7FFF7FFFu), k1 = p2_nonzero_halves((mh.y | ml.y) & 0x7FFF7FFFu);
+        const uint32_t k2 = p2_nonzero_halves((mh.z | ml.z) & 0x7FFF7FFFu), k3 = p2_nonzero_halves((mh.w | ml.w) & 0x7FFF7FFFu);
+        uh.x &= k0; uh.y &= k1; uh.z &= k2; uh.w &= k3;
+        ul.x &= k0; ul.y &= k1; ul.z &= k2; ul.w &= k3;
+      }
+      a.y[o] = uh;
+      a.y[plane + o] = ul;
+    }
+  }
+  {
+    const float m_ = wave_max(ymax);
+    if (lane == 0)
+      atomicMax(reinterpret_cast<unsigned*>(a.ymeta) + P2_AMAX0 + ((blockIdx.x * NW + wave) & (P2_NSLOT - 1)), __float_as_uint(m_));
+  }
+}
+#endif
diff --git a/behavior_driven_video_synthesis_amd/csrc/conv_route.h b/behavior_driven_video_synthesis_amd/csrc/conv_route.h
--- a/behavior_driven_video_synthesis_amd/csrc/conv_route.h
+++ b/behavior_driven_video_synthesis_amd/csrc/conv_route.h
@@ -55,6 +55,8 @@
 int vunet_conv_x6_launch_mt1(const GatherArgs& ga, const void* wx, int mtiles_pad, int pro, int NT, hipStream_t st);
 int vunet_conv_x6_launch_mt2(const GatherArgs& ga, const void* wx, int mtiles_pad, int pro, int NT, hipStream_t st);
 int vunet_conv_h2_launch_mt1(const GatherArgs& ga, const void* wx, int mtiles_pad, const float* amax, int pro, int NT, hipStream_t st);
-int vunet_conv_h2_launch_mt2(const GatherArgs& ga, const void* wx, int mtiles_pad, const float* amax, int pro, int NT, hipStream_t st);
+int vunet_conv_h2_launch_mt2(const GatherArgs& ga, const void* wx, int mtiles_pad, const float* amax, int pro, int NT, hipStream_t st,
+                             int ksplit = 1);
 int vunet_conv_h2_launch_par(const GatherArgs& ga, const void* wx, int mtiles_pad, const float* amax, hipStream_t st);
-int vunet_conv_h2_launch_w16(const GatherArgs& ga, const void* wx, int mtiles_pad, const float* amax, int pro, int MT, hipStream_t st);
+int vunet_conv_h2_launch_w16(const GatherArgs& ga, const void* wx, int mtiles_pad, const float* amax, int pro, int MT, hipStream_t st,
+                             int ksplit = 1);
diff --git a/behavior_driven_video_synthesis_amd/csrc/conv_x6.hip b/behavior_driven_video_synthesis_amd/csrc/conv_x6.hip
--- a/behavior_driven_video_synthesis_amd/csrc/conv_x6.hip
+++ b/behavior_driven_video_synthesis_amd/csrc/conv_x6.hip
@@ -47,6 +47,29 @@
   for (int NT = top; NT >= 2; NT >>= 1)
     if (x6_blocks(d, *MT, NT) >= 512) return NT;
   return x6_blocks(d, *MT, 1) >= min_blocks ? 1 : 0;
+}
+
+int g_vunet_ksplit = 0;
+
+int vunet_cu_count() {
+  static const int n = [] {
+    int dev = 0, cus = 0;
+    if (hipGetDevice(&dev) != hipSuccess || hipDeviceGetAttribute(&cus, hipDeviceAttributeMultiprocessorCount, dev) != hipSuccess || cus <= 0) {
+      (void)hipGetLastError();
+      return 256;
+    }
+    return cus;
+  }();
+  return n;
+}
+
+static int conv_route_ksplit(const ConvRoute& r, const vunet_conv_desc* d) {
+  if (g_vunet_ksplit == 1 || d->stride != 1 || r.NT != 1) return 1;
+  if (!(r.family == CONV_H2_W16 || (r.family == CONV_H2 && r.MT == 2))) return 1;
+  const int nch = d->C1 / 16 + d->C2 / 16;
+  if (nch < 2 || nch % 2) return 1;
+  if (g_vunet_ksplit == 2) return 2;
+  return x6_blocks(d, r.MT, 1) <= vunet_cu_count() ? 2 : 1;
 }
 
 VUNET_ENV_FLAG(env_no_tiled, "VUNET_NO_TILED")
@@ -190,11 +213,11 @@
   ga.wide = ga.wide && (reinterpret_cast<uintptr_t>(res2) & 15) == 0;
   switch (r.family) {
     case CONV_H2_SMALL: return vunet_conv_h2_small_launch(r, ga, wx, mtp, amax, st);
-    case CONV_H2_W16: return vunet_conv_h2_launch_w16(ga, wx, mtp, amax, r.pro, r.MT, st);
+    case CONV_H2_W16: return vunet_conv_h2_launch_w16(ga, wx, mtp, amax, r.pro, r.MT, st, conv_route_ksplit(r, d));
     case CONV_H2_PAR: return vunet_conv_h2_launch_par(ga, wx, mtp, amax, st);
     case CONV_H2:
       return r.MT == 1 ? vunet_conv_h2_launch_mt1(ga, wx, mtp, amax, r.pro, r.NT, st)
-                       : vunet_conv_h2_launch_mt2(ga, wx, mtp, amax, r.pro, r.NT, st);
+                       : vunet_conv_h2_launch_mt2(ga, wx, mtp, amax, r.pro, r.NT, st, conv_route_ksplit(r, d));
     default:
       return r.MT == 1 ? vunet_conv_x6_launch_mt1(ga, wx, mtp, r.pro, r.NT, st)
                        : vunet_conv_x6_launch_mt2(ga, wx, mtp, r.pro, r.NT, st);
@@ -258,6 +281,19 @@
   return conv_route(d, split == 0 ? 0 : (split == 2 ? 2 : 1), has_aux != 0, has_res != 0, false, 128, true).publishes ? 1 : 0;
 }
 
+extern "C" int vunet_conv2d_ksplit(const vunet_conv_desc* d, int32_t has_aux, int32_t has_res, int32_t has_mask, int32_t x6_entry) {
+  if (!d) return 1;
+  const ConvRoute r = x6_entry ? split_route(d, true, has_aux != 0, has_res != 0, has_mask != 0, 1, true)
+                               : conv_route(d, 2, has_aux != 0, has_res != 0, has_mask != 0, 128, true);
+  return conv_route_ksplit(r, d);
+}
+
+extern "C" int vunet_set_ksplit(int32_t mode) {
+  if (mode < 0 || mode > 2) return VUNET_ERR_ARG;
+  g_vunet_ksplit = mode;
+  return VUNET_OK;
+}
+
 extern "C" int vunet_conv2d_gather_variant(const vunet_conv_desc* d, int32_t has_aux, char* name, int32_t len) {
   if (!d || !name || len < 8) return VUNET_ERR_ARG;
   return conv_route_name(gather_route(d, has_aux != 0, false), d, name, len);
diff --git a/behavior_driven_video_synthesis_amd/ops.py b/behavior_driven_video_synthesis_amd/ops.py
--- a/behavior_driven_video_synthesis_amd/ops.py
+++ b/behavior_driven_video_synthesis_amd/ops.py
@@ -183,11 +183,32 @@
     return _tuning_values.get(key, 0)
 
 
+_ksplit = {"mode": 0}
+
+
+def set_ksplit(mode: int) -> int:
+    prev = _ksplit["mode"]
+    _call("vunet_set_ksplit", int(mode))
+    _ksplit["mode"] = int(mode)
+    return prev
+
+
+def conv_ksplit(desc, has_aux=False, has_res=False, has_mask=False, x6_entry=False) -> int:
+    return int(_lib.lib().vunet_conv2d_ksplit(ctypes.byref(desc), int(has_aux), int(has_res), int(has_mask), int(x6_entry)))
+
+
+def p2_conv_ksplit(desc) -> int:
+    return int(_lib.lib().vunet_p2_conv_ksplit(ctypes.byref(desc)))
+
+
 def apply_env_tuning():
     spec = os.environ.get("VUNET_TUNING", "")
     for kv in filter(None, (t.strip() for t in spec.split(","))):
         k, _, v = kv.partition("=")
-        set_tuning(k.strip(), int(v))
+        if k.strip() == "ksplit":
+            set_ksplit(int(v))
+        else:
+            set_tuning(k.strip(), int(v))
 
 
 def absmax_partials(x1, x2=None):
diff --git a/include/vunet_hip.h b/include/vunet_hip.h
--- a/include/vunet_hip.h
+++ b/include/vunet_hip.h
@@ -67,6 +67,8 @@
 int vunet_absmax_partials(const float* x1, int64_t n1, const float* x2, int64_t n2, float* out, void* stream);
 int vunet_conv2d_variant(const vunet_conv_desc* d, int32_t has_aux, int32_t has_wx, int32_t has_mask, char* name,
                          int32_t len);
+int vunet_set_ksplit(int32_t mode);
+int vunet_conv2d_ksplit(const vunet_conv_desc* d, int32_t has_aux, int32_t has_res, int32_t has_mask, int32_t x6_entry);
 
 int vunet_conv2d_bf16_supported(const vunet_conv_desc* d);
 int vunet_pack_bf16(const float* wt_f, void* wb, int32_t C1, int32_t C2, int32_t Mpad, void* stream);
@@ -271,6 +273,7 @@
 } vunet_p2_desc;
 int vunet_p2_conv_supported(const vunet_p2_desc* d);
 int vunet_p2_conv_variant(const vunet_p2_desc* d, char* name, int32_t len);
+int vunet_p2_conv_ksplit(const vunet_p2_desc* d);
 int vunet_p2_conv(const vunet_p2_desc* d, const void* x, const int32_t* xmeta, const void* w_image, const float* wk,
                   const float* shift, const void* mask, void* y, int32_t* ymeta, void* stream);
 int vunet_p2_weight_image_bytes(int32_t Cout, int32_t Cin, int32_t dgrad);
```

Result: no change. 804.0 frames/s, median of 6 (+0.6%).
